# Meowuu7/equi-articulated-pose

Measured on AMD Instinct MI355X. Metric: point-clouds/sec (4096 pts, 60 anchors) fwd+bwd, higher is better.
Workload: dtype f32; 1 GPU; 8 x 4096-pt synthetic laptop clouds per GPU, 3-block inter backbone 1->64->128->512 (NN=64,K=24,A=60), forward+backward+Adam; clouds_per_gpu=8, points=4096, anchors=60

## Files before the change

equi-articulated-pose_amd/csrc/gemm_bf16x3.hip:

```cpp
#include "common.h"
#include "device_prims.h"
#include <algorithm>
#include <type_traits>

namespace {

constexpr int BK = 16, BN = 256;
constexpr unsigned PLANE_BYTES = 256 * BK * 2;
constexpr unsigned oper_bytes(int pl) { return (unsigned)pl * PLANE_BYTES; }
constexpr unsigned stage_bytes(int pl) { return 2 * oper_bytes(pl); }
constexpr size_t shmem_bytes(int pl) { return 3 * (size_t)stage_bytes(pl); }
constexpr int WAVES_N = 4;

struct Args {
    int M, N, K;
    const float *A; long long lda;
    const float *B; long long ldb, sB;
    float *C; long long ldc, sC;
    int tiles_m, tiles_n;
    const int *tbl; int na;
    int nr;
    const unsigned *Apre;
    long long sA; int slabs, kslab;
    const float *ep_scale, *ep_shift, *ep_res; float ep_slope; long long sRes;
    const unsigned *absA, *absB; float multB; int grpB; long long sAbsB;
};
constexpr int TAPS = 12;
constexpr unsigned TBL_BYTES = 64 * TAPS * 4;

__device__ __forceinline__ unsigned pk_bf16(float a, float b) {
    unsigned r;
    asm("v_cvt_pk_bf16_f32 %0, %1, %2" : "=v"(r) : "v"(a), "v"(b));
    return r;
}

struct Row16 { f32x4 q0, q1; u32x2 p0, p1; };

__device__ __forceinline__ void split_pair(float x0, float x1, unsigned &h, unsigned &m, unsigned &l) {
    h = pk_bf16(x0, x1);
    const float r0 = x0 - __uint_as_float(h << 16), r1 = x1 - __uint_as_float(h & 0xffff0000u);
    m = pk_bf16(r0, r1);
    const float s0 = r0 - __uint_as_float(m << 16), s1 = r1 - __uint_as_float(m & 0xffff0000u);
    l = pk_bf16(s0, s1);
}

__device__ __forceinline__ void split_pair_h(float x0, float x1, unsigned &h, unsigned &l) {
    const f16x2 hh = __builtin_convertvector((f32x2){x0, x1}, f16x2);
    const f16x2 ll = __builtin_convertvector((f32x2){x0 - (float)hh.x, x1 - (float)hh.y}, f16x2);
    h = __builtin_bit_cast(unsigned, hh);
    l = __builtin_bit_cast(unsigned, ll);
}

__device__ __forceinline__ void split_quad(const f32x4 &a, const f32x4 &b, u32x4 &h, u32x4 &m, u32x4 &l) {
    unsigned h0, h1, h2, h3, m0, m1, m2, m3, l0, l1, l2, l3;
    split_pair(a.x, a.y, h0, m0, l0);
    split_pair(a.z, a.w, h1, m1, l1);
    split_pair(b.x, b.y, h2, m2, l2);
    split_pair(b.z, b.w, h3, m3, l3);
    h = (u32x4){h0, h1, h2, h3};
    m = (u32x4){m0, m1, m2, m3};
    l = (u32x4){l0, l1, l2, l3};
}

template <int MI, int WN, int BMODE, bool APRE, int PL>
__device__ __forceinline__ void split_gemm_body(const Args &g) {
    constexpr unsigned OPER_BYTES = oper_bytes(PL), STAGE_BYTES = stage_bytes(PL);
    constexpr int NT = 128 * WN, NI = 8 / WN, WM = 8 / WN, BM = 32 * MI * WM, RG = NT / 4;
    constexpr int NPA = BM / RG, NPO = 256 / RG;
    static_assert(WN == 4 && NPO == 2 && (NPA == 1 || NPA == 2), "8 waves, 128-row staging groups");
    extern __shared__ __attribute__((aligned(16))) unsigned char smem[];

    int id = blockIdx.x, tm, tn;
    {
        const int groups = g.tiles_n / 8 * 8;
        const int xcd = id & 7, slot = id >> 3;
        const int panel = (slot / g.tiles_m) * 8 + xcd;
        if (panel < groups && id < groups * g.tiles_m) { tn = panel; tm = slot % g.tiles_m; }
        else { const int r = id - groups * g.tiles_m; tn = groups + r / g.tiles_m; tm = r % g.tiles_m; }
    }
    const int z = blockIdx.y;
    const int m0 = tm * BM, n0 = tn * BN;
    const int item = g.slabs > 1 ? z / g.slabs : z;
    const long long item_of_z = item;
    const long long kbeg = g.slabs > 1 ? (long long)(z - item * g.slabs) * g.kslab : 0;
    const float *A = g.A + item * g.sA + kbeg;
    const float *B = g.B + item * g.sB + (BMODE == 0 ? kbeg : BMODE == 1 ? kbeg * g.ldb : 0);
    long long zc = z;
    if constexpr (BMODE == 1) {
        if (g.slabs > 1) zc = (long long)(z - item * g.slabs) * (gridDim.y / g.slabs) + item;
    }
    float *C = g.C + zc * g.sC;

    const int t = threadIdx.x, lane = t & 63;
    const int wave = __builtin_amdgcn_readfirstlane(t >> 6);
    const int wm = wave / WN, wn = wave % WN;
    const int li = lane & 31, lh = lane >> 5;

    const int c4 = t & 3, rq = t >> 2;
    const int c4b = BMODE ? __builtin_amdgcn_readfirstlane(t >> 7) : c4, rqb = BMODE ? (t & 127) : rq;
    const float *baseA[NPA], *baseB[NPO];
#pragma unroll
    for (int u = 0; u < NPA; ++u) baseA[u] = A + (long long)min(m0 + RG * u, g.M - RG) * g.lda;
#pragma unroll
    for (int u = 0; u < NPO; ++u) baseB[u] = B + (long long)min(n0 + RG * u, g.N - RG) * g.ldb;
    const unsigned char *preA[NPA];
    constexpr int PRE_PIECE = PL == 3 ? 32 : 16;
    const long long pre_pitch = (long long)(g.K / 4) * PRE_PIECE;
#pragma unroll
    for (int u = 0; u < NPA; ++u)
        preA[u] = reinterpret_cast<const unsigned char *>(g.Apre) + (long long)min(m0 + RG * u, g.M - RG) * pre_pitch + (kbeg / 4) * PRE_PIECE;
    const unsigned offP = (unsigned)((long long)rq * pre_pitch + PRE_PIECE * c4);
    float sclA[2] = {1.0f, 1.0f}, sclB[2] = {1.0f, 1.0f};
    const unsigned *absBz = g.absB + item_of_z * g.sAbsB;
    if constexpr (PL == 2) {
#pragma unroll
        for (int u = 0; u < NPA; ++u) sclA[u] = pow2_scale(__uint_as_float(g.absA[min(m0 + RG * u, g.M - RG) + rq]));
#pragma unroll
        for (int u = 0; u < NPO; ++u) sclB[u] = pow2_scale(__uint_as_float(absBz[(min(n0 + RG * u, g.N - RG) + rqb) / g.grpB]) * g.multB);
    }
    const unsigned offA = (unsigned)((long long)rq * g.lda + 4 * c4) * 4u, offB = (unsigned)((long long)rq * g.ldb + 4 * c4) * 4u;
    unsigned colB[NPO], tapB[NPO];
#pragma unroll
    for (int u = 0; u < NPO; ++u) {
        const int n = min(n0 + RG * u, g.N - RG) + rqb;
        if constexpr (BMODE == 2) {
            const int per = g.na * g.nr, pt = n / per, an = (n - pt * per) / g.nr;
            colB[u] = (unsigned)(n - an * g.nr) * 4u;
            tapB[u] = (unsigned)an * (TAPS * 4u);
        } else {
            colB[u] = (unsigned)n * 4u; tapB[u] = 0;
        }
    }
    auto wr_of = [](int r, int c) { return (unsigned)r * 32u + ((16u * (unsigned)(c >> 1)) ^ ((((unsigned)r >> 2) ^ ((unsigned)r >> 3)) & 1u) * 16u) + 8u * (unsigned)(c & 1); };
    const unsigned wr_off = wr_of(rq, c4), wr_offB = wr_of(rqb, c4b);
    const unsigned char *tbl = smem + 3 * STAGE_BYTES;
    if constexpr (BMODE == 2) {
        for (int i = t; i < g.na * TAPS; i += NT) reinterpret_cast<int *>(smem + 3 * STAGE_BYTES)[i] = g.tbl[i] * 4 * g.nr;
        __syncthreads();
    }
    const int nk = (g.slabs > 1 ? g.kslab : g.K) / BK;

    Row16 ra0, rb0, ra1, rb1;
    auto ld = [&](const float *ubase, unsigned voff) __attribute__((always_inline)) {
        return *reinterpret_cast<const f32x4 *>(reinterpret_cast<const char *>(ubase) + voff);
    };
    auto ldw = [&](const float *ubase, unsigned voff) __attribute__((always_inline)) {
        return *reinterpret_cast<const float *>(reinterpret_cast<const char *>(ubase) + voff);
    };
    auto load_tile = [&](int kt, Row16 &a, Row16 &b) __attribute__((always_inline)) {
        const int ko = kt * BK;
        if constexpr (APRE) {
            const unsigned char *p0 = preA[0] + kt * (4 * PRE_PIECE) + offP;
            a.q0 = *reinterpret_cast<const f32x4 *>(p0);
            if constexpr (PL == 3) a.p0 = *reinterpret_cast<const u32x2 *>(p0 + 16);
            if constexpr (NPA == 2) {
                const unsigned char *p1 = preA[1] + kt * (4 * PRE_PIECE) + offP;
                a.q1 = *reinterpret_cast<const f32x4 *>(p1);
                if constexpr (PL == 3) a.p1 = *reinterpret_cast<const u32x2 *>(p1 + 16);
            }
        } else {
            a.q0 = ld(baseA[0] + ko, offA);
            if constexpr (NPA == 2) a.q1 = ld(baseA[1] + ko, offA);
        }
        if constexpr (BMODE == 0) {
            b.q0 = ld(baseB[0] + ko, offB); b.q1 = ld(baseB[1] + ko, offB);
        } else if constexpr (BMODE == 1) {
            const float *r0 = B + (long long)(ko + 4 * c4b) * g.ldb, *r1 = r0 + g.ldb, *r2 = r1 + g.ldb, *r3 = r2 + g.ldb;
            b.q0 = (f32x4){ldw(r0, colB[0]), ldw(r1, colB[0]), ldw(r2, colB[0]), ldw(r3, colB[0])};
            b.q1 = (f32x4){ldw(r0, colB[1]), ldw(r1, colB[1]), ldw(r2, colB[1]), ldw(r3, colB[1])};
        } else {
            const int k0 = ko + 4 * c4b, ch = k0 / TAPS, t0 = k0 - ch * TAPS;
            const float *r = B + (long long)ch * g.ldb;
            const u32x4 o0 = *reinterpret_cast<const u32x4 *>(tbl + tapB[0] + 4 * t0);
            const u32x4 o1 = *reinterpret_cast<const u32x4 *>(tbl + tapB[1] + 4 * t0);
            b.q0 = (f32x4){ldw(r, colB[0] + o0.x), ldw(r, colB[0] + o0.y), ldw(r, colB[0] + o0.z), ldw(r, colB[0] + o0.w)};
            b.q1 = (f32x4){ldw(r, colB[1] + o1.x), ldw(r, colB[1] + o1.y), ldw(r, colB[1] + o1.z), ldw(r, colB[1] + o1.w)};
        }
    };
    auto park_piece = [&](unsigned char *oper, int u, const f32x4 &q, unsigned wr, float scl) __attribute__((always_inline)) {
        unsigned h0, m0_, l0, h1, m1, l1;
        if constexpr (PL == 2) {
            split_pair_h(q.x * scl, q.y * scl, h0, l0);
            split_pair_h(q.z * scl, q.w * scl, h1, l1);
            unsigned char *row = oper + (unsigned)u * ((unsigned)RG * 32u) + wr;
            *reinterpret_cast<u32x2 *>(row) = (u32x2){h0, h1};
            *reinterpret_cast<u32x2 *>(row + PLANE_BYTES) = (u32x2){l0, l1};
            return;
        }
        split_pair(q.x, q.y, h0, m0_, l0);
        split_pair(q.z, q.w, h1, m1, l1);
        unsigned char *row = oper + (unsigned)u * ((unsigned)RG * 32u) + wr;
        *reinterpret_cast<u32x2 *>(row) = (u32x2){h0, h1};
        *reinterpret_cast<u32x2 *>(row + PLANE_BYTES) = (u32x2){m0_, m1};
        *reinterpret_cast<u32x2 *>(row + 2 * PLANE_BYTES) = (u32x2){l0, l1};
    };
    auto park_half = [&](unsigned char *oper, const Row16 &r, int half, int pieces, unsigned wr, float scl) __attribute__((always_inline)) {
        if (half < pieces) park_piece(oper, half, half ? r.q1 : r.q0, wr, scl);
    };
    auto park_half_a = [&](unsigned char *oper, const Row16 &r, int half, unsigned wr) __attribute__((always_inline)) {
// ... 68 lines not shown
            SB();
            product(al, bh);
            park_half(s2 + OPER_BYTES, sb, 1, NPO, wr_offB, sclB[1]);
            load_tile(min(kt + 4, nk - 1), sa, sb);
            SB();
            __syncthreads();
            return;
        }
        u32x4 bm[NI], am[MI], bh[NI], al[MI];
        frag(st, rdB, 1, bm);
        SB();
        if constexpr (decltype(first)::value) product0(ah, bl); else product(ah, bl);
        park_half_a(s2, sa, 0, wr_off);
        SB();
        frag(st, rdA, 1, am);
        SB();
        product(ah, bm);
        park_half_a(s2, sa, 1, wr_off);
        SB();
        frag(st, rdB, 0, bh);
        SB();
        product(am, bm);
        park_half(s2 + OPER_BYTES, sb, 0, NPO, wr_offB, sclB[0]);
        SB();
        frag(st, rdA, 2, al);
        SB();
        product(am, bh);
        park_half(s2 + OPER_BYTES, sb, 1, NPO, wr_offB, sclB[1]);
        SB();
        u32x4 ah2[MI];
        frag(s1, rdA, 0, ah2);
        SB();
        product(al, bh);
        load_tile(min(kt + 4, nk - 1), sa, sb);
        SB();
        frag(s1, rdB, 2, bl);
        SB();
        product(ah, bh);
        SB();
#undef SB
#pragma unroll
        for (int i = 0; i < MI; ++i) ah[i] = ah2[i];
        __syncthreads();
    };

    load_tile(0, ra0, rb0);
    load_tile(min(1, nk - 1), ra1, rb1);
    park_a(smem, ra0, wr_off);
    park(smem + OPER_BYTES, rb0, NPO, wr_offB);
    load_tile(min(2, nk - 1), ra0, rb0);
    park_a(smem + STAGE_BYTES, ra1, wr_off);
    park(smem + STAGE_BYTES + OPER_BYTES, rb1, NPO, wr_offB);
    load_tile(min(3, nk - 1), ra1, rb1);
    __syncthreads();
    frag(smem, rdA, 0, ah);
    frag(smem, rdB, PL - 1, bl);

    unsigned s0 = 0, s1 = STAGE_BYTES, s2 = 2 * STAGE_BYTES;
    tile(std::true_type{}, 0, smem + s0, smem + s1, smem + s2, ra0, rb0);
    int kt = 1;
    for (; kt + 1 < nk; kt += 2) {
        { const unsigned r = s0; s0 = s1; s1 = s2; s2 = r; }
        tile(std::false_type{}, kt, smem + s0, smem + s1, smem + s2, ra1, rb1);
        { const unsigned r = s0; s0 = s1; s1 = s2; s2 = r; }
        tile(std::false_type{}, kt + 1, smem + s0, smem + s1, smem + s2, ra0, rb0);
    }
    if (kt < nk) {
        { const unsigned r = s0; s0 = s1; s1 = s2; s2 = r; }
        tile(std::false_type{}, kt, smem + s0, smem + s1, smem + s2, ra1, rb1);
    }

#pragma unroll
    for (int i = 0; i < MI; ++i)
#pragma unroll
        for (int j = 0; j < NI; ++j) {
            const int col = n0 + 32 * NI * wn + 32 * j + li;
            float unsB = 1.0f;
            if constexpr (PL == 2) unsB = 1.0f / pow2_scale(__uint_as_float(absBz[min(col, g.N - 1) / g.grpB]) * g.multB);
#pragma unroll
            for (int r = 0; r < 16; ++r) {
                const int row = m0 + 32 * MI * wm + 32 * i + (r & 3) + 8 * (r >> 2) + 4 * lh;
                if (row < g.M && col < g.N) {
                    float v = acc[i][j][r];
                    if constexpr (PL == 2) v = (v * (1.0f / pow2_scale(__uint_as_float(g.absA[row])))) * unsB;
                    if (g.ep_scale != nullptr) {
                        v = fmaf(v, g.ep_scale[row], g.ep_shift[row]);
                        v = v >= 0.f ? v : v * g.ep_slope;
                        if (g.ep_res != nullptr) v += g.ep_res[(long long)z * g.sRes + (long long)row * g.ldc + col];
                    }
                    C[(long long)row * g.ldc + col] = v;
                }
            }
        }
}

template <int MI, int WN, int BMODE, bool APRE>
__global__ __launch_bounds__(128 * WN, WN / 2) void gemm_bf16x3_kernel(Args g) { split_gemm_body<MI, WN, BMODE, APRE, 3>(g); }

template <int MI, int WN, int BMODE, bool APRE>
__global__ __launch_bounds__(128 * WN, WN / 2) void gemm_f16x2_kernel(Args g) { split_gemm_body<MI, WN, BMODE, APRE, 2>(g); }

}

namespace {

__global__ __launch_bounds__(256) void presplit_kernel(int M, int K4, const float *__restrict__ A, long long lda, u32x4 *__restrict__ out) {
    const long long i = (long long)blockIdx.x * 256 + threadIdx.x;
    if (i >= (long long)M * K4) return;
    const int row = (int)(i / K4), c = (int)(i - (long long)row * K4);
    const f32x4 q = *reinterpret_cast<const f32x4 *>(A + row * lda + 4 * c);
    unsigned h0, m0, l0, h1, m1, l1;
    split_pair(q.x, q.y, h0, m0, l0);
    split_pair(q.z, q.w, h1, m1, l1);
    out[2 * i] = (u32x4){h0, h1, m0, m1};
    out[2 * i + 1] = (u32x4){l0, l1, 0u, 0u};
}

__global__ __launch_bounds__(256) void presplit_h_kernel(int M, int K4, const float *__restrict__ A, long long lda, const unsigned *__restrict__ absA,
                                                         u32x4 *__restrict__ out) {
    const long long i = (long long)blockIdx.x * 256 + threadIdx.x;
    if (i >= (long long)M * K4) return;
    const int row = (int)(i / K4), c = (int)(i - (long long)row * K4);
    const float scl = pow2_scale(__uint_as_float(absA[row]));
    const f32x4 q = *reinterpret_cast<const f32x4 *>(A + row * lda + 4 * c);
    unsigned h0, l0, h1, l1;
    split_pair_h(q.x * scl, q.y * scl, h0, l0);
    split_pair_h(q.z * scl, q.w * scl, h1, l1);
    out[i] = (u32x4){h0, h1, l0, l1};
}

__device__ __forceinline__ unsigned absbits4(const f32x4 &q) {
    return max(max(__float_as_uint(q.x) & 0x7fffffffu, __float_as_uint(q.y) & 0x7fffffffu), max(__float_as_uint(q.z) & 0x7fffffffu, __float_as_uint(q.w) & 0x7fffffffu));
}
__global__ __launch_bounds__(256) void absmax_rows_kernel(long long rows_total, int rows, int cols4, const float *__restrict__ x, long long ld,
                                                          long long stride, unsigned *__restrict__ out) {
    const long long r = (long long)blockIdx.x * 4 + (threadIdx.x >> 6);
    if (r >= rows_total) return;
    const long long item = r / rows;
    const f32x4 *row = reinterpret_cast<const f32x4 *>(x + item * stride + (r - item * rows) * ld);
    unsigned m = 0u;
    for (int c = threadIdx.x & 63; c < cols4; c += 64) m = max(m, absbits4(row[c]));
#pragma unroll
    for (int o = 32; o > 0; o >>= 1) m = max(m, (unsigned)__shfl_xor((int)m, o));
    if ((threadIdx.x & 63) == 0) out[r] = m;
}
__global__ __launch_bounds__(256) void absmax_colgroups_kernel(int rows, int cols4, int grp4, int row_slices, const float *__restrict__ x, long long ld,
                                                               long long stride, unsigned *__restrict__ out) {
    const int c = blockIdx.x * 256 + threadIdx.x;
    if (c >= cols4) return;
    const int item = blockIdx.z, sl = blockIdx.y;
    const int r0 = (int)((long long)rows * sl / row_slices), r1 = (int)((long long)rows * (sl + 1) / row_slices);
    const float *p = x + item * stride + 4 * (long long)c;
    unsigned m = 0u;
    for (int r = r0; r < r1; ++r) m = max(m, absbits4(*reinterpret_cast<const f32x4 *>(p + r * ld)));
    if (m != 0u) atomicMax(out + (long long)item * (cols4 / grp4) + c / grp4, m);
}
__global__ __launch_bounds__(256) void grouped_bound_kernel(long long total, int p, int nn, int n_sup, const unsigned *__restrict__ point_max,
                                                            const int32_t *__restrict__ idx, unsigned *__restrict__ out) {
    const long long i = (long long)blockIdx.x * 256 + threadIdx.x;
    if (i >= total) return;
    const unsigned *pm = point_max + (i / p) * n_sup;
    const int32_t *id = idx + i * nn;
    float s = 0.f;
    for (int n = 0; n < nn; ++n) {
        const int q = id[n];
        if ((unsigned)q < (unsigned)n_sup) s += __uint_as_float(pm[q]);
    }
// ... 247 lines not shown

void intra2d_args(Args &g, int o, int c, int p, int na, int nr, int nt, const float *W, const float *feats, const int32_t *intra_idx, float *out) {
    const long long pa = (long long)p * na * nr;
    g.M = o; g.N = (int)pa; g.K = c * nt;
    g.A = W; g.lda = (long long)c * nt;
    g.B = feats; g.ldb = pa; g.sB = (long long)c * pa;
    g.C = out; g.ldc = pa; g.sC = (long long)o * pa;
    g.tbl = intra_idx; g.na = na; g.nr = nr;
}

}

extern "C" int eap_so3_intra_conv2d_bf16x3_f32(int b, int o, int c, int p, int na, int nr, int nt, const float *W, const float *feats,
                                               const int32_t *intra_idx, float *out, eap_stream_t stream) {
    if (b <= 0 || o <= 0 || p <= 0 || na <= 0) return 0;
    if (int e = intra2d_refusal(b, o, c, p, na, nr, nt, W, "so3_intra_conv2d_bf16x3_f32")) return e;
    Args g{};
    intra2d_args(g, o, c, p, na, nr, nt, W, feats, intra_idx, out);
    return launch_split<2>(g, b, eap::S(stream), "so3_intra_conv2d_bf16x3_f32");
}

extern "C" int eap_so3_intra_conv2d_f16x2_f32(int b, int o, int c, int p, int na, int nr, int nt, const float *W, const float *feats,
                                              const int32_t *intra_idx, float *out, const int32_t *abs_w, const int32_t *abs_f, eap_stream_t stream) {
    if (b <= 0 || o <= 0 || p <= 0 || na <= 0) return 0;
    if (int e = intra2d_refusal(b, o, c, p, na, nr, nt, W, "so3_intra_conv2d_f16x2_f32")) return e;
    if (!abs_w || !abs_f) return eap::bad_arg("so3_intra_conv2d_f16x2_f32: the operand magnitudes are required (eap_absmax_rows_f32 / _colgroups_f32)");
    Args g{};
    intra2d_args(g, o, c, p, na, nr, nt, W, feats, intra_idx, out);
    g.absA = reinterpret_cast<const unsigned *>(abs_w); g.absB = reinterpret_cast<const unsigned *>(abs_f); g.multB = 1.0f;
    g.grpB = na * nr; g.sAbsB = p;
    return launch_split<2, 2>(g, b, eap::S(stream), "so3_intra_conv2d_f16x2_f32");
}

namespace {

__global__ __launch_bounds__(256) void split_reduce_kernel(long long mn4, int parts, const f32x4 *__restrict__ ws, float *__restrict__ C, int N, long long ldc) {
    const long long i = (long long)blockIdx.x * 256 + threadIdx.x;
    if (i >= mn4) return;
    f32x4 acc = ws[i];
    for (int z = 1; z < parts; ++z) acc += ws[(long long)z * mn4 + i];
    const long long e = i * 4, row = e / N, col = e - row * N;
    *reinterpret_cast<f32x4 *>(C + row * ldc + col) = acc;
}

inline int reduce_slabs(int M, int N, int K, int batch) {
    const int tiles = ((M % 256) == 0 ? M / 256 : M / 128) * ((N + BN - 1) / BN);
    int s = 1;
    while (s < 64 && (long long)tiles * batch * s < 512 && (K / BK) % (2 * s) == 0 && K / (2 * s) >= 64 * BK) s *= 2;
    return s;
}

}

extern "C" int eap_gemm_bf16x3_reduce_f32_supported(int M, int N, int K, const float *A, int64_t lda, int64_t strideA, const float *B,
                                                    int64_t ldb, int64_t strideB, int64_t ldc) {
    if (!tile_dims_ok(M, N, K)) return 0;
    if ((long long)32 * WAVES_N * lda * 4 >= (1ll << 32) || (long long)32 * WAVES_N * ldb * 4 >= (1ll << 32)) return 0;
    if ((lda & 3) || (ldb & 3) || (strideA & 3) || (strideB & 3) || (ldc & 3)) return 0;
    if ((reinterpret_cast<uintptr_t>(A) & 15) || (reinterpret_cast<uintptr_t>(B) & 15)) return 0;
    return 1;
}

extern "C" int64_t eap_gemm_bf16x3_reduce_workspace(int M, int N, int K, int batch) {
    if (M <= 0 || N <= 0 || K <= 0 || batch <= 0) return 0;
    return (int64_t)M * N * batch * reduce_slabs(M, N, K, batch);
}

extern "C" int eap_gemm_bf16x3_reduce_f32(int M, int N, int K, const float *A, int64_t lda, int64_t strideA, const float *B, int64_t ldb,
                                          int64_t strideB, float *C, int64_t ldc, int batch, float *workspace, eap_stream_t stream) {
    if (M <= 0 || N <= 0 || batch <= 0) return 0;
    if (!eap_gemm_bf16x3_reduce_f32_supported(M, N, K, A, lda, strideA, B, ldb, strideB, ldc) || (reinterpret_cast<uintptr_t>(C) & 15) ||
        (reinterpret_cast<uintptr_t>(workspace) & 15))
        return eap::bad_arg("gemm_bf16x3_reduce_f32: unsupported operands (ask eap_gemm_bf16x3_reduce_f32_supported)");
    const int slabs = reduce_slabs(M, N, K, batch);
    Args g{};
    g.M = M; g.N = N; g.K = K;
    g.A = A; g.lda = lda; g.sA = strideA;
    g.B = B; g.ldb = ldb; g.sB = strideB;
    g.C = workspace; g.ldc = N; g.sC = (long long)M * N;
    g.slabs = slabs; g.kslab = K / slabs;
    if (int e = launch_split<0>(g, (long long)batch * slabs, eap::S(stream), "gemm_bf16x3_reduce_f32")) return e;
    const long long mn4 = (long long)M * N / 4;
    return eap::run_kernel("gemm_bf16x3_reduce_f32 (sum of the partials)", split_reduce_kernel, eap::cdiv(mn4, 256), 1, 1, dim3(256), 0, eap::S(stream), mn4,
                           batch * slabs, reinterpret_cast<const f32x4 *>(workspace), C, N, (long long)ldc);
}

namespace {

int device_cus() {
    static std::atomic<int> seen[64] = {};
    int dev = 0;
    if (hipGetDevice(&dev) != hipSuccess) { (void)hipGetLastError(); return 256; }
    const bool slot = dev >= 0 && dev < 64;
    int n = slot ? seen[dev].load(std::memory_order_relaxed) : 0;
    if (n > 0) return n;
    if (hipDeviceGetAttribute(&n, hipDeviceAttributeMultiprocessorCount, dev) != hipSuccess || n <= 0) { (void)hipGetLastError(); n = 256; }
    if (slot) seen[dev].store(n, std::memory_order_relaxed);
    return n;
}

constexpr int SPLITK_MIN_TILES = 16;
constexpr int SPLITK_MAX_SLABS = 64;

inline bool splitk_slabs_ok(int K, int slabs) {
    return slabs >= 1 && slabs <= SPLITK_MAX_SLABS && (K / BK) % slabs == 0 && (slabs == 1 || K / BK / slabs >= SPLITK_MIN_TILES);
}

}

extern "C" int eap_gemm_f16x2_splitk_slabs(int M, int N, int K, int batch, int cus) {
    if (M != 128 || N <= 0 || batch <= 0 || K < 64 * BK || (K % BK) != 0) return 1;
    if (cus <= 0) cus = device_cus();
    const long long tiles = (long long)((N + BN - 1) / BN) * batch;
    const long long want = (4ll * cus + tiles - 1) / tiles;
    int best = 1;
    for (int s = 1; s <= SPLITK_MAX_SLABS; ++s) {
        if (!splitk_slabs_ok(K, s)) continue;
        best = s;
        if (s >= want) break;
    }
    const long long kt = K / BK;
    const long long one = ((tiles + cus - 1) / cus) * kt, cut = ((tiles * best + cus - 1) / cus) * (kt / best);
    return 4 * cut <= 3 * one ? best : 1;
}

extern "C" int64_t eap_gemm_f16x2_splitk_workspace(int M, int N, int batch, int slabs) {
    if (M <= 0 || N <= 0 || batch <= 0 || slabs <= 1) return 0;
    return (int64_t)M * N * batch * slabs;
}

extern "C" int eap_gemm_f16x2_splitk_f32(int M, int N, int K, const float *A, int64_t lda, const float *B, int64_t ldb, int64_t strideB,
                                         float *C, int64_t ldc, int64_t strideC, int batch, const int32_t *abs_a, const int32_t *abs_b, int grp_b,
                                         float mult_b, int slabs, float *workspace, int64_t workspace_floats, eap_stream_t stream) {
    if (M <= 0 || N <= 0 || batch <= 0) return eap::bad_arg("gemm_f16x2_splitk_f32: M, N and batch must be positive");
    if (!A || !B || !C) return eap::bad_arg("gemm_f16x2_splitk_f32: A, B and C are required");
    if (!abs_a || !abs_b || !(mult_b > 0.f) || grp_b <= 0 || (N % grp_b) != 0)
        return eap::bad_arg("gemm_f16x2_splitk_f32: the operand magnitudes are required (eap_absmax_rows_f32 / _colgroups_f32), column groups dividing N");
    if (M != 128 || !eap_gemm_bf16x3_nn_f32_supported(M, N, K, A, lda, B, ldb, strideB))
        return eap::bad_arg("gemm_f16x2_splitk_f32: one 128-row tile of operands eap_gemm_bf16x3_nn_f32_supported takes");
    if (slabs == 0) slabs = eap_gemm_f16x2_splitk_slabs(M, N, K, batch, 0);
    if (!splitk_slabs_ok(K, slabs))
        return eap::bad_arg("gemm_f16x2_splitk_f32: the slab count must divide the K / 16 k-tiles into slabs of at least 16 (at most 64 slabs)");
    if ((long long)batch * slabs > 65535) return eap::bad_arg("gemm_f16x2_splitk_f32: batch x slabs exceeds 65535");
    Args g{};
    g.M = M; g.N = N; g.K = K;
    g.A = A; g.lda = lda;
    g.B = B; g.ldb = ldb; g.sB = strideB;
    g.C = C; g.ldc = ldc; g.sC = strideC;
    g.absA = reinterpret_cast<const unsigned *>(abs_a); g.absB = reinterpret_cast<const unsigned *>(abs_b); g.multB = mult_b;
    g.grpB = grp_b; g.sAbsB = N / grp_b;
    if (slabs == 1) return launch_split<1, 2>(g, batch, eap::S(stream), "gemm_f16x2_splitk_f32");
    if (strideC != (int64_t)M * ldc || (ldc & 3) || ldc < N || !eap::aligned16(C, workspace))
        return eap::bad_arg("gemm_f16x2_splitk_f32: more than one slab needs strideC = M ldc, ldc a multiple of 4, C and the workspace 16-byte aligned");
    if (!workspace || workspace_floats < eap_gemm_f16x2_splitk_workspace(M, N, batch, slabs))
        return eap::bad_arg("gemm_f16x2_splitk_f32: the workspace is too small (ask eap_gemm_f16x2_splitk_workspace)");
    g.C = workspace; g.ldc = N; g.sC = (long long)M * N;
    g.slabs = slabs; g.kslab = K / slabs;
    if (int e = launch_split<1, 2>(g, (long long)batch * slabs, eap::S(stream), "gemm_f16x2_splitk_f32")) return e;
    const long long mn4 = (long long)batch * M * N / 4;
    return eap::run_kernel("gemm_f16x2_splitk_f32 (sum of the slabs)", split_reduce_kernel, eap::cdiv(mn4, 256), 1, 1, dim3(256), 0, eap::S(stream), mn4, slabs,
                           reinterpret_cast<const f32x4 *>(workspace), C, N, (long long)ldc);
}
```

equi-articulated-pose_amd/csrc/narrow_conv.hip:

```cpp
#include "common.h"
#include "device_prims.h"
#include <type_traits>

namespace {

constexpr int NT = 256, WAVES = 4;
constexpr int TILE = 128;
constexpr int SEGC = 2048;

__device__ __forceinline__ int drow(int r, int h) { return (r & 3) + 8 * (r >> 2) + 4 * h; }

template <int KS2>
__device__ __forceinline__ void load_x(f32x4 (&xa)[KS2], const float *__restrict__ xb, long n, long col0, unsigned voff, bool ok, int ck, int h) {
#pragma unroll
    for (int s = 0; s < KS2; ++s)
        xa[s] = (ok && 2 * s + h < ck) ? ld_off<f32x4>(xb + (size_t)(2 * s) * n + col0, voff) : (f32x4){0.f, 0.f, 0.f, 0.f};
}

template <int KS2>
__device__ __forceinline__ void load_w(float (&wf)[KS2], const float *__restrict__ W, int orow, int ck, int h) {
#pragma unroll
    for (int s = 0; s < KS2; ++s) wf[s] = (2 * s + h < ck) ? W[(size_t)orow * ck + 2 * s + h] : 0.f;
}

// ... 57 lines not shown
                                                                 const float *__restrict__ x, float *__restrict__ pivot,
                                                                 float *__restrict__ psum, float *__restrict__ psq) {
    __shared__ __attribute__((aligned(16))) float s_piv[64];
    __shared__ float s_red[WAVES][2][32];
    const Pos w(ct, n);
    const int t = threadIdx.x, o0 = blockIdx.y * ct * 32, h = w.h;
    if (t < 32 * ct) {
        float p = 0.f;
        for (int k = 0; k < ck; ++k) p = fmaf(W[(size_t)(o0 + t) * ck + k], x[(size_t)k * n], p);
        s_piv[t] = p;
        if (w.seg == 0 && w.bi == 0) pivot[o0 + t] = p;
    }
    __syncthreads();
    float wf[KS2];
    load_w<KS2>(wf, W, w.ch0 + w.li, ck, h);
    f32x4 pv[4];
#pragma unroll
    for (int g = 0; g < 4; ++g) pv[g] = *reinterpret_cast<const f32x4 *>(&s_piv[w.ch0 - o0 + 8 * g + 4 * h]);
    float sa[16], qa[16];
#pragma unroll
    for (int r = 0; r < 16; ++r) sa[r] = qa[r] = 0.f;
    const float *xb = x + (size_t)w.bi * ck * n;
#pragma unroll 1
    for (long col0 = w.beg + (long)w.cw * TILE; col0 < w.end; col0 += (long)w.ncw * TILE) {
        const long col = col0 + 4 * w.li;
        const bool ok = col < n;
        f32x4 xa[KS2];
        load_x<KS2>(xa, xb, n, col0, w.xoff, ok, ck, h);
        f32x16 d[4];
        conv_tile<KS2, false>(d, xa, wf);
        if (ok) {
#pragma unroll
            for (int r = 0; r < 16; ++r)
#pragma unroll
                for (int c = 0; c < 4; ++c) {
                    const float dd = d[c][r] - pv[r >> 2][r & 3];
                    sa[r] += dd;
                    qa[r] = fmaf(dd, dd, qa[r]);
                }
        }
    }
    block_sums(sa, qa, s_red, ct, o0, w.bi, gridDim.z, nseg, w.seg, psum, psq);
}

template <int KS2>
__global__ __launch_bounds__(NT) void narrow_conv_bnact_fwd_kernel(int ct, int o, int ck, long n, float slope, const float *__restrict__ W,
                                                                     const float *__restrict__ x, const float *__restrict__ scale,
                                                                     const float *__restrict__ shift, float *__restrict__ y) {
    const Pos w(ct, n);
    const int h = w.h;
    float wf[KS2];
    load_w<KS2>(wf, W, w.ch0 + w.li, ck, h);
    f32x4 sc[4], sh[4];
#pragma unroll
    for (int g = 0; g < 4; ++g) {
        sc[g] = *reinterpret_cast<const f32x4 *>(scale + w.ch0 + 8 * g + 4 * h);
        sh[g] = *reinterpret_cast<const f32x4 *>(shift + w.ch0 + 8 * g + 4 * h);
    }
    const float *xb = x + (size_t)w.bi * ck * n;
    float *yb = y + ((size_t)w.bi * o + w.ch0) * n;
    const unsigned roff = 4u * (4u * h * (unsigned)n + 4u * w.li);
#pragma unroll 1
    for (long col0 = w.beg + (long)w.cw * TILE; col0 < w.end; col0 += (long)w.ncw * TILE) {
        const long col = col0 + 4 * w.li;
        const bool ok = col < n;
        f32x4 xa[KS2];
        load_x<KS2>(xa, xb, n, col0, w.xoff, ok, ck, h);
        f32x16 d[4];
        conv_tile<KS2, false>(d, xa, wf);
        if (ok) {
#pragma unroll
            for (int r = 0; r < 16; ++r) {
                const float a = sc[r >> 2][r & 3], b = sh[r >> 2][r & 3];
                f32x4 v;
                v.x = fmaf(d[0][r], a, b); v.y = fmaf(d[1][r], a, b); v.z = fmaf(d[2][r], a, b); v.w = fmaf(d[3][r], a, b);
                v.x = v.x > 0.f ? v.x : v.x * slope; v.y = v.y > 0.f ? v.y : v.y * slope;
                v.z = v.z > 0.f ? v.z : v.z * slope; v.w = v.w > 0.f ? v.w : v.w * slope;
                st_off<f32x4>(yb + (size_t)(8 * (r >> 2)) * n + col0, roff + 4u * (unsigned)(r & 3) * (unsigned)n, v);
            }
        }
    }
}

template <int KS2>
__global__ __launch_bounds__(NT) void narrow_conv_bwd_reduce_kernel(int ct, int o, int ck, long n, int nseg, float slope,
                                                                      const float *__restrict__ gy, const float *__restrict__ x,
                                                                      const float *__restrict__ W, const float *__restrict__ scale,
                                                                      const float *__restrict__ shift, const float *__restrict__ mean,
                                                                      const float *__restrict__ invstd, float *__restrict__ pg,
                                                                      float *__restrict__ pgx) {
    __shared__ __attribute__((aligned(16))) float s_sc[64], s_sh[64], s_mu[64], s_is[64];
    __shared__ float s_red[WAVES][2][32];
    const Pos w(ct, n);
    const int t = threadIdx.x, o0 = blockIdx.y * ct * 32, h = w.h;
    if (t < 32 * ct) { s_sc[t] = scale[o0 + t]; s_sh[t] = shift[o0 + t]; s_mu[t] = mean[o0 + t]; s_is[t] = invstd[o0 + t]; }
    __syncthreads();
    float wf[KS2];
    load_w<KS2>(wf, W, w.ch0 + w.li, ck, h);
    float sa[16], qa[16];
#pragma unroll
    for (int r = 0; r < 16; ++r) sa[r] = qa[r] = 0.f;
    const float *xb = x + (size_t)w.bi * ck * n;
    const float *gb = gy + ((size_t)w.bi * o + w.ch0) * n;
    const unsigned roff = 4u * (4u * h * (unsigned)n + 4u * w.li);
    const int lc = w.ch0 - o0;
#pragma unroll 1
    for (long col0 = w.beg + (long)w.cw * TILE; col0 < w.end; col0 += (long)w.ncw * TILE) {
        const long col = col0 + 4 * w.li;
        const bool ok = col < n;
        f32x4 xa[KS2];
        load_x<KS2>(xa, xb, n, col0, w.xoff, ok, ck, h);
        f32x16 d[4];
        conv_tile<KS2, false>(d, xa, wf);
        if (ok) {
#pragma unroll
            for (int g = 0; g < 4; ++g) {
                f32x4 gv[4];
#pragma unroll
                for (int q = 0; q < 4; ++q) gv[q] = ld_off<f32x4>(gb + (size_t)(8 * g) * n + col0, roff + 4u * q * (unsigned)n);
                const f32x4 sc = *reinterpret_cast<const f32x4 *>(&s_sc[lc + 8 * g + 4 * h]), sh = *reinterpret_cast<const f32x4 *>(&s_sh[lc + 8 * g + 4 * h]);
                const f32x4 mu = *reinterpret_cast<const f32x4 *>(&s_mu[lc + 8 * g + 4 * h]), is = *reinterpret_cast<const f32x4 *>(&s_is[lc + 8 * g + 4 * h]);
#pragma unroll
                for (int q = 0; q < 4; ++q)
#pragma unroll
                    for (int c = 0; c < 4; ++c) {
                        const float yv = d[c][4 * g + q];
                        const float pre = fmaf(yv, sc[q], sh[q]);
                        const float gg = pre > 0.f ? gv[q][c] : gv[q][c] * slope;
                        sa[4 * g + q] += gg;
                        qa[4 * g + q] = fmaf(gg, (yv - mu[q]) * is[q], qa[4 * g + q]);
                    }
            }
        }
    }
    block_sums(sa, qa, s_red, ct, o0, w.bi, gridDim.z, nseg, w.seg, pg, pgx);
}

template <int KS2>
__global__ __launch_bounds__(NT) void narrow_conv_bwd_dw_kernel(int ct, int o, int ck, long n, int nseg, float slope,
                                                                  const float *__restrict__ gy, const float *__restrict__ x,
                                                                  const float *__restrict__ W, const float *__restrict__ scale,
                                                                  const float *__restrict__ shift, const float *__restrict__ mean,
                                                                  const float *__restrict__ invstd, const float *__restrict__ k2,
                                                                  const float *__restrict__ k3, float *__restrict__ partial) {
    __shared__ float s_part[WAVES][16][64];
    const Pos w(ct, n);
    const int h = w.h, li = w.li, wave = threadIdx.x >> 6;
    const int ch = w.ch0 + li;
    float wf[KS2];
    load_w<KS2>(wf, W, ch, ck, h);
    const float sc = scale[ch], sh = shift[ch], mu = mean[ch], is = invstd[ch], c2 = k2[ch], c3 = k3[ch];
    const float *gb = gy + ((size_t)w.bi * o + w.ch0) * n;
    const unsigned goff = 4u * ((unsigned)li * (unsigned)n + 16u * h), koff = 4u * ((unsigned)min(li, ck - 1) * (unsigned)n + 16u * h);
    f32x16 dw;
#pragma unroll
    for (int r = 0; r < 16; ++r) dw[r] = 0.f;
    const float *xb = x + (size_t)w.bi * ck * n;
    const f32x4 zero4 = {0.f, 0.f, 0.f, 0.f};
#pragma unroll 1
    for (long col0 = w.beg + (long)w.cw * TILE; col0 < w.end; col0 += (long)w.ncw * TILE) {
        const long col = col0 + 4 * li;
        f32x4 xa[KS2];
        load_x<KS2>(xa, xb, n, col0, w.xoff, col < n, ck, h);
        f32x16 d[4];
        conv_tile<KS2, true>(d, xa, wf);
#pragma unroll
        for (int g = 0; g < 4; ++g) {
            f32x4 gv[4], xv[4];
#pragma unroll
            for (int q = 0; q < 4; ++q) {
                const long cq = col0 + 4 * (8 * g + 4 * h + q);
                const bool in = cq < n;
                gv[q] = in ? ld_off<f32x4>(gb + col0 + 4 * (8 * g + q), goff) : zero4;
                xv[q] = (in && li < ck) ? ld_off<f32x4>(xb + col0 + 4 * (8 * g + q), koff) : zero4;
            }
#pragma unroll
            for (int q = 0; q < 4; ++q)
#pragma unroll
                for (int c = 0; c < 4; ++c) {
                    const float yv = d[c][4 * g + q];
                    const float pre = fmaf(yv, sc, sh);
                    const float gg = pre > 0.f ? gv[q][c] : gv[q][c] * slope;
                    const float gx = fmaf(gg, sc, -c2) - ((yv - mu) * is) * c3;
                    dw = __builtin_amdgcn_mfma_f32_32x32x2f32(gx, xv[q][c], dw, 0, 0, 0);
                }
        }
    }
#pragma unroll
    for (int r = 0; r < 16; ++r) s_part[wave][r][w.lane] = dw[r];
    __syncthreads();
    if (wave < ct) {
        float *slab = partial + ((size_t)w.bi * nseg + w.seg) * o * ck;
#pragma unroll
        for (int r = 0; r < 16; ++r) {
            float v = 0.f;
            for (int u = wave; u < WAVES; u += ct) v += s_part[u][r][w.lane];
            if (li < ck) slab[(size_t)(w.ch0 + drow(r, h)) * ck + li] = v;
        }
    }
}

__global__ __launch_bounds__(256) void narrow_conv_dw_sum_kernel(int mn, int slabs, const float *__restrict__ partial, float *__restrict__ dW) {
    const int e = blockIdx.x * 4 + (threadIdx.x >> 6), lane = threadIdx.x & 63;
    if (e >= mn) return;
    float s = 0.f;
    for (int z = lane; z < slabs; z += 64) s += partial[(size_t)z * mn + e];
#pragma unroll
    for (int d = 32; d > 0; d >>= 1) s += __shfl_xor(s, d);
    if (lane == 0) dW[e] = s;
}

inline int nseg_of(long n) { return (int)((n + SEGC - 1) / SEGC); }

inline bool misaligned(const void *p) { return (reinterpret_cast<uintptr_t>(p) & 15) != 0; }

inline int refuse(const char *who, int o, int ck, long n, const void *p0, const void *p1, const void *p2 = nullptr) {
    char buf[200];
    const char *why = nullptr;
    if (ck < 1 || ck > 32) why = "1 to 32 contraction indices (C*K)";
    else if (o < 32 || o % 32 != 0) why = "a multiple of 32 output channels";
    else if (n < 0 || (n & 3) != 0 || n >= (1l << 25)) why = "a row length (P*A) that is a multiple of 4 below 2^25";
    else if (misaligned(p0) || misaligned(p1) || misaligned(p2)) why = "16-byte aligned tensors";
    if (!why) return 0;
    snprintf(buf, sizeof(buf), "%s: takes %s", who, why);
    return eap::bad_arg(buf);
}

inline int tiles_per_block(int o) { return o % 64 == 0 ? 2 : 1; }

template <typename F>
int by_depth(int ck, F &&f) {
    return ck <= 24 ? f(std::integral_constant<int, 12>{}) : f(std::integral_constant<int, 16>{});
}

}

extern "C" int eap_narrow_conv_segments(int64_t n) { return n > 0 ? nseg_of((long)n) : 0; }

extern "C" int eap_narrow_conv_stats_f32(int b, int o, int ck, int64_t n, const float *W, const float *x, float *pivot, float *psum,
                                         float *psq, eap_stream_t stream) {
    if (int e = refuse("narrow_conv_stats", o, ck, (long)n, x, nullptr)) return e;
    if (b <= 0 || n <= 0) return 0;
    const int nseg = nseg_of((long)n), ct = tiles_per_block(o);
    return by_depth(ck, [&](auto ks2) {
        return eap::run_kernel("narrow_conv_stats", narrow_conv_stats_kernel<decltype(ks2)::value>, nseg, o / (32 * ct), b, dim3(NT), 0, eap::S(stream), ct,
                               ck, (long)n, nseg, W, x, pivot, psum, psq);
    });
}

extern "C" int eap_narrow_conv_bnact_fwd_f32(int b, int o, int ck, int64_t n, float slope, const float *W, const float *x, const float *scale,
                                             const float *shift, float *y, eap_stream_t stream) {
    if (int e = refuse("narrow_conv_bnact_fwd", o, ck, (long)n, x, y, scale)) return e;
    if (misaligned(shift)) return eap::bad_arg("narrow_conv_bnact_fwd: takes 16-byte aligned tensors");
    if (b <= 0 || n <= 0) return 0;
    const int ct = tiles_per_block(o);
    return by_depth(ck, [&](auto ks2) {
        return eap::run_kernel("narrow_conv_bnact_fwd", narrow_conv_bnact_fwd_kernel<decltype(ks2)::value>, nseg_of((long)n), o / (32 * ct), b, dim3(NT), 0,
                               eap::S(stream), ct, o, ck, (long)n, slope, W, x, scale, shift, y);
    });
}

extern "C" int eap_narrow_conv_bwd_reduce_f32(int b, int o, int ck, int64_t n, float slope, const float *gy, const float *x, const float *W,
                                              const float *scale, const float *shift, const float *mean, const float *invstd, float *pg,
                                              float *pgx, eap_stream_t stream) {
    if (int e = refuse("narrow_conv_bwd_reduce", o, ck, (long)n, x, gy)) return e;
    if (b <= 0 || n <= 0) return 0;
    const int nseg = nseg_of((long)n), ct = tiles_per_block(o);
    return by_depth(ck, [&](auto ks2) {
        return eap::run_kernel("narrow_conv_bwd_reduce", narrow_conv_bwd_reduce_kernel<decltype(ks2)::value>, nseg, o / (32 * ct), b, dim3(NT), 0, eap::S(stream),
                               ct, o, ck, (long)n, nseg, slope, gy, x, W, scale, shift, mean, invstd, pg, pgx);
    });
}

extern "C" int eap_narrow_conv_bwd_dw_f32(int b, int o, int ck, int64_t n, float slope, const float *gy, const float *x, const float *W,
                                          const float *scale, const float *shift, const float *mean, const float *invstd, const float *k2,
                                          const float *k3, float *partial, float *dW, eap_stream_t stream) {
    if (int e = refuse("narrow_conv_bwd_dw", o, ck, (long)n, x, gy)) return e;
    if (b <= 0 || n <= 0) return 0;
    const int nseg = nseg_of((long)n), ct = tiles_per_block(o);
    hipStream_t s = eap::S(stream);
    int e = by_depth(ck, [&](auto ks2) {
        return eap::run_kernel("narrow_conv_bwd_dw", narrow_conv_bwd_dw_kernel<decltype(ks2)::value>, nseg, o / (32 * ct), b, dim3(NT), 0, s, ct, o, ck, (long)n,
                               nseg, slope, gy, x, W, scale, shift, mean, invstd, k2, k3, partial);
    });
    if (e) return e;
    const int mn = o * ck;
    return eap::run_kernel("narrow_conv_bwd_dw (sum)", narrow_conv_dw_sum_kernel, eap::cdiv(mn, 4), 1, 1, dim3(256), 0, s, mn, b * nseg, partial, dW);
}
```

equi-articulated-pose_amd/csrc/norm_fold.hip:

```cpp
#include <math.h>
#include <string.h>

#include "common.h"

namespace {

constexpr int WAVE = 64;

__device__ __forceinline__ double wave_sum(double v) {
#pragma unroll
    for (int m = WAVE / 2; m >= 1; m >>= 1) v += __shfl_xor(v, m, WAVE);
    return v;
}

__device__ __forceinline__ void two_row_sums(const float *__restrict__ a, const float *__restrict__ q, int parts, int lane, double &sa, double &sq) {
    sa = 0.0, sq = 0.0;
    for (int i = lane; i < parts; i += WAVE) {
        sa += (double)a[i];
        sq += (double)q[i];
    }
    sa = wave_sum(sa);
    sq = wave_sum(sq);
}

// ... 15 lines not shown
    double var = s2 / count - m * m;
    var = var < 0.0 ? 0.0 : var;
    if (running_mean != nullptr) {
        const float keep = (float)(1.0 - momentum), alpha = (float)momentum;
        running_mean[ch] = fmaf(alpha, (float)mu, running_mean[ch] * keep);
        running_var[ch] = fmaf(alpha, (float)(var * (count / (count - 1.0))), running_var[ch] * keep);
    }
    const double g = (double)gamma[ch];
    const double is = rsqrt(var + eps);
    const double scale64 = g * is;
    scale[ch] = (float)scale64;
    shift[ch] = (float)((double)beta[ch] - mu * scale64);
    mean[ch] = mu;
    invstd[ch] = is;
    beta_copy[ch] = beta[ch];
    inv_gamma[ch] = g == 0.0 ? 0.f : (float)(1.0 / g);
}

__global__ __launch_bounds__(WAVE) void norm_fold_bwd_kernel(int o, int parts, int b, int na, double count, const float *__restrict__ pg,
                                                             const float *__restrict__ pgx, const float *__restrict__ k1v,
                                                             const float *__restrict__ beta, const float *__restrict__ inv_gamma,
                                                             const float *__restrict__ gmax, const float *__restrict__ xmax,
                                                             float *__restrict__ dgamma, float *__restrict__ dbeta, float *__restrict__ k2v,
                                                             float *__restrict__ k3v, float *__restrict__ coef, float *__restrict__ bound) {
    const int ch = blockIdx.x, lane = threadIdx.x;
    double tg, tgx;
    two_row_sums(pg + (long)ch * parts, pgx + (long)ch * parts, parts, lane, tg, tgx);
    const float k1 = k1v[ch];
    const float k2 = (float)((double)k1 * tg / count), k3 = (float)((double)k1 * tgx / count);
    if (lane == 0) {
        dgamma[ch] = (float)tgx;
        dbeta[ch] = (float)tg;
        k2v[ch] = k2;
        k3v[ch] = k3;
        if (coef != nullptr) {
            coef[ch] = k1, coef[o + ch] = k2, coef[2 * o + ch] = k3;
            coef[3 * o + ch] = beta[ch], coef[4 * o + ch] = inv_gamma[ch];
        }
    }
    if (bound == nullptr) return;
    const float a1 = fabsf(k1), a2 = fabsf(k2), a3 = fabsf(k3);
    for (int cloud = 0; cloud < b; ++cloud) {
        const long row = ((long)cloud * o + ch) * na;
        for (int a = lane; a < na; a += WAVE) bound[row + a] = (a1 * gmax[row + a] + a2) + a3 * xmax[row + a];
    }
}

__global__ __launch_bounds__(256) void norm_fold_colmax_kernel(int o, int na, const float *__restrict__ bound, float *__restrict__ colmax) {
    __shared__ float red[256];
    const int t = threadIdx.x, a = blockIdx.x * 16 + (t & 15), grp = t >> 4, cloud = blockIdx.y;
    float m = 0.f;
    if (a < na) {
        const float *src = bound + (long)cloud * o * na + a;
        for (int ch = grp; ch < o; ch += 16) m = nan_max(m, src[(long)ch * na]);
    }
    red[t] = m;
    __syncthreads();
    if (grp == 0 && a < na) {
        for (int g = 1; g < 16; ++g) m = nan_max(m, red[g * 16 + t]);
        colmax[(long)cloud * na + a] = m;
    }
}

__global__ __launch_bounds__(256) void dense_zbound_kernel(int b, int na, int rp, int p, int ldw, long cnt_stride, const float *__restrict__ colmax,
                                                           const int32_t *__restrict__ cnt, const int32_t *__restrict__ n_rows,
                                                           float *__restrict__ words) {
    const int w = blockIdx.x * blockDim.x + threadIdx.x, cloud = blockIdx.y;
    if (w >= ldw) return;
    float v = 0.f;
    if (w < na * rp / 4) {
        const int a = 4 * w / rp, r0 = 4 * w - a * rp, live = n_rows[cloud];
        const float m = colmax[(long)cloud * na + a];
#pragma unroll
        for (int j = 0; j < 4; ++j) {
            int c = r0 + j < live ? cnt[cloud * cnt_stride + r0 + j] : 0;
            c = c < 0 ? 0 : (c > p ? p : c);
            const float t = m * (float)c;
            v = j == 0 ? t : nan_max(v, t);
        }
    }
    words[(long)cloud * ldw + w] = v;
}

__global__ __launch_bounds__(256) void dense_gbound_parts_kernel(int bc, int c, int rp, int na, int ks, const float *__restrict__ W3,
                                                                 const float *__restrict__ fc4, float *__restrict__ fpart, float *__restrict__ wsum) {
    __shared__ float red[256];
    const int t = threadIdx.x, nt = blockDim.x;
    if ((int)blockIdx.x < bc) {
        const float *src = fc4 + (long)blockIdx.x * rp * na;
        const int len = rp * na;
        float m = 0.f, m1 = 0.f, m2 = 0.f, m3 = 0.f;
        int e = t;
        for (; e + 3 * nt < len; e += 4 * nt) {
            const float v0 = src[e], v1 = src[e + nt], v2 = src[e + 2 * nt], v3 = src[e + 3 * nt];
            m = nan_max(m, fabsf(v0)), m1 = nan_max(m1, fabsf(v1)), m2 = nan_max(m2, fabsf(v2)), m3 = nan_max(m3, fabsf(v3));
        }
        for (; e < len; e += nt) m = nan_max(m, fabsf(src[e]));
        m = nan_max(nan_max(m, m1), nan_max(m2, m3));
        red[t] = m;
        __syncthreads();
        if (t < na) {
            for (int g = 1; g < nt / na; ++g) m = nan_max(m, red[t + g * na]);
            fpart[(long)blockIdx.x * na + t] = m;
        }
        return;
    }
    const int oc = blockIdx.x - bc, lane = t & (WAVE - 1), wave = t / WAVE, waves = nt / WAVE;
    float m = 0.f;
    if (wave < waves)
        for (int k = wave; k < ks; k += waves) {
            const float *row = W3 + ((long)oc * ks + k) * c;
            double s = 0.0;
            for (int i = lane; i < c; i += WAVE) s += (double)fabsf(row[i]);
            m = nan_max(m, (float)wave_sum(s));
        }
    if (lane == 0 && wave < waves) red[wave] = m;
    __syncthreads();
    if (t == 0) {
        for (int g = 1; g < waves; ++g) m = nan_max(m, red[g]);
        wsum[oc] = m * 1.0001f;
    }
}

__global__ __launch_bounds__(256) void dense_gbound_kernel(int c, int na, int o, const float *__restrict__ fpart, const float *__restrict__ wsum,
                                                           float *__restrict__ bound) {
    __shared__ float red[256];
    const int t = threadIdx.x, cloud = blockIdx.x / na, a = blockIdx.x - cloud * na;
    float m = 0.f;
    for (int ch = t; ch < c; ch += 256) m = nan_max(m, fpart[((long)cloud * c + ch) * na + a]);
    red[t] = m;
    __syncthreads();
    for (int s = 128; s >= 1; s >>= 1) {
        if (t < s) red[t] = nan_max(red[t], red[t + s]);
        __syncthreads();
    }
    m = red[0];
    for (int oc = t; oc < o; oc += 256) bound[(long)blockIdx.x * o + oc] = m * wsum[oc];
}

__global__ __launch_bounds__(256) void dense_point_order_kernel(int p, int quads, const int64_t *__restrict__ order, const int4 *__restrict__ memb,
                                                                const float *__restrict__ q_xyz, int32_t *__restrict__ order32,
                                                                int4 *__restrict__ memb_out, float *__restrict__ xyz_out,
                                                                int32_t *__restrict__ pivot_pos) {
    const long i = (long)blockIdx.x * blockDim.x + threadIdx.x;
    const int cloud = blockIdx.y;
    if (i >= (long)p * quads) return;
    const int j = (int)(i / quads), q = (int)(i - (long)j * quads);
    const int64_t src = order[(long)cloud * p + j];
    if (src < 0 || src >= p) return;
    memb_out[((long)cloud * p + j) * quads + q] = memb[((long)cloud * p + src) * quads + q];
    if (q != 0) return;
    order32[(long)cloud * p + j] = (int32_t)src;
#pragma unroll
    for (int k = 0; k < 3; ++k) xyz_out[((long)cloud * 3 + k) * p + j] = q_xyz[((long)cloud * 3 + k) * p + src];
    if (cloud == 0 && src == 0) pivot_pos[0] = j;
}

inline double from_bits(int64_t bits) {
    double v;
    memcpy(&v, &bits, sizeof v);
    return v;
}

inline bool aligned16(const void *p) { return (reinterpret_cast<uintptr_t>(p) & 15) == 0; }

}

extern "C" int eap_norm_fold_train_f32(int o, int parts, int64_t pivot_stride, int64_t count, int64_t eps_bits, int64_t momentum_bits,
                                       const float *ps, const float *pq, const float *pivot, const float *gamma, const float *beta,
                                       float *running_mean, float *running_var, float *scale, float *shift, double *mean, double *invstd,
                                       float *beta_copy, float *inv_gamma, eap_stream_t stream) {
    if (!ps || !pq || !pivot || !gamma || !beta || !scale || !shift || !mean || !invstd || !beta_copy || !inv_gamma)
        return eap::bad_arg("norm_fold_train: null pointer (only running_mean / running_var may be null, and only together)");
    if ((running_mean == nullptr) != (running_var == nullptr))
        return eap::bad_arg("norm_fold_train: null pointer (only running_mean / running_var may be null, and only together)");
    if (o <= 0 || parts <= 0 || count <= 0 || pivot_stride <= 0) return eap::bad_arg("norm_fold_train: o, parts, count and the pivot stride must be positive");
    return eap::run_kernel("norm_fold_train", norm_fold_train_kernel, o, 1, 1, dim3(WAVE), 0, eap::S(stream), parts, (long)pivot_stride, (double)count,
                           from_bits(eps_bits), from_bits(momentum_bits), ps, pq, pivot, gamma, beta, running_mean, running_var, scale, shift, mean,
                           invstd, beta_copy, inv_gamma);
}

extern "C" int eap_norm_fold_bwd_f32(int o, int parts, int b, int na, int64_t count, const float *pg, const float *pgx, const float *k1,
                                     const float *beta, const float *inv_gamma, const float *gmax, const float *xmax, float *dgamma, float *dbeta,
                                     float *k2, float *k3, float *coef, float *bound, float *colmax, eap_stream_t stream) {
    if (!pg || !pgx || !k1 || !dgamma || !dbeta || !k2 || !k3) return eap::bad_arg("norm_fold_bwd: null pointer");
    const bool dense = beta || inv_gamma || gmax || xmax || coef || bound || colmax;
    if (dense && !(beta && inv_gamma && gmax && xmax && coef && bound && colmax))
        return eap::bad_arg("norm_fold_bwd: null pointer (beta, inv_gamma, gmax, xmax, coef, bound and colmax come together or not at all)");
    if (o <= 0 || parts <= 0 || count <= 0) return eap::bad_arg("norm_fold_bwd: o, parts and count must be positive");
    if (dense && (b <= 0 || na <= 0 || b > 65535)) return eap::bad_arg("norm_fold_bwd: b and na must be positive, b at most 65535 (grid.y)");
    if (int e = eap::run_kernel("norm_fold_bwd", norm_fold_bwd_kernel, o, 1, 1, dim3(WAVE), 0, eap::S(stream), o, parts, b, na, (double)count, pg, pgx, k1,
                                beta, inv_gamma, gmax, xmax, dgamma, dbeta, k2, k3, coef, bound))
        return e;
    if (!dense) return 0;
    return eap::run_kernel("norm_fold_bwd (colmax)", norm_fold_colmax_kernel, eap::cdiv(na, 16), b, 1, dim3(256), 0, eap::S(stream), o, na, (const float *)bound,
                           colmax);
}

extern "C" int eap_so3_dense_zbound_f32(int b, int na, int rp, int p, int ldz, int64_t cnt_stride, const float *colmax, const int32_t *cnt,
                                        const int32_t *n_rows, float *words, eap_stream_t stream) {
    if (!colmax || !cnt || !n_rows || !words) return eap::bad_arg("so3_dense_zbound: null pointer");
    if (b <= 0 || na <= 0 || rp <= 0 || p <= 0 || ldz <= 0) return eap::bad_arg("so3_dense_zbound: b, na, rp, p and ldz must be positive");
    if (rp % 4 != 0 || ldz % 4 != 0 || (long long)na * rp > ldz || cnt_stride < rp)
        return eap::bad_arg("so3_dense_zbound: rp and ldz multiples of 4, ldz >= na * rp, the row stride of cnt >= rp");
    return eap::run_kernel("so3_dense_zbound", dense_zbound_kernel, eap::cdiv(ldz / 4, 256), b, 1, dim3(256), 0, eap::S(stream), b, na, rp, p, ldz / 4,
                           (long)cnt_stride, colmax, cnt, n_rows, words);
}

extern "C" int eap_so3_dense_gplanes_bound_f32(int b, int o, int c, int na, int ks, int rp, const float *W3, const float *fc4, float *fpart,
                                               float *wsum, float *bound, eap_stream_t stream) {
    if (!W3 || !fc4 || !fpart || !wsum || !bound) return eap::bad_arg("so3_dense_gplanes_bound: null pointer");
    if (b <= 0 || o <= 0 || c <= 0 || na <= 0 || ks <= 0 || rp <= 0) return eap::bad_arg("so3_dense_gplanes_bound: every size must be positive");
    if (na > 128 || (long long)rp * na > 0x7fffffffLL || (long long)b * c > 0x7fffffffLL - o || (long long)b * na > 0x7fffffffLL)
        return eap::bad_arg("so3_dense_gplanes_bound: na <= 128, rp * na, b * c + o and b * na below 2^31");
    const int nt = 256 / na * na;
    if (int e = eap::run_kernel("so3_dense_gplanes_bound (parts)", dense_gbound_parts_kernel, (long long)b * c + o, 1, 1, dim3(nt), 0, eap::S(stream), b * c, c,
                                rp, na, ks, W3, fc4, fpart, wsum))
        return e;
    return eap::run_kernel("so3_dense_gplanes_bound", dense_gbound_kernel, (long long)b * na, 1, 1, dim3(256), 0, eap::S(stream), c, na, o, (const float *)fpart,
                           (const float *)wsum, bound);
}

extern "C" int eap_so3_dense_point_order(int b, int p, int words, const int64_t *order, const uint32_t *memb, const float *q_xyz, int32_t *order32,
                                         uint32_t *memb_out, float *xyz_out, int32_t *pivot_pos, eap_stream_t stream) {
    if (!order || !memb || !q_xyz || !order32 || !memb_out || !xyz_out || !pivot_pos) return eap::bad_arg("so3_dense_point_order: null pointer");
    if (b <= 0 || p <= 0) return eap::bad_arg("so3_dense_point_order: b and p must be positive");
    if (words != 16 && words != 32) return eap::bad_arg("so3_dense_point_order: 16 or 32 membership words per point");
    if (!aligned16(memb) || !aligned16(memb_out)) return eap::bad_arg("so3_dense_point_order: takes 16-byte aligned membership tables");
    const int quads = words / 4;
    return eap::run_kernel("so3_dense_point_order", dense_point_order_kernel, eap::cdiv((long long)p * quads, 256), b, 1, dim3(256), 0, eap::S(stream), p, quads,
                           order, reinterpret_cast<const int4 *>(memb), q_xyz, order32, reinterpret_cast<int4 *>(memb_out), xyz_out, pivot_pos);
}
```

equi-articulated-pose_amd/vgtk/_hip.py:

```python
import ctypes
import os
import re
import struct
import types
import weakref

import torch

_PKG_ROOT = os.path.abspath(os.path.join(os.path.dirname(__file__), '..'))
LIB_PATH = os.path.join(_PKG_ROOT, 'libeap_hip.so')

if not os.path.exists(LIB_PATH):
    raise ImportError(
        f'{LIB_PATH} not found: build the HIP extension first '
        '(python -c "import __graft_entry__ as g; g.build()" or make -C equi-articulated-pose_amd/csrc). '
        'This package has no CPU fallback.')

lib = ctypes.CDLL(LIB_PATH)


_HEADERS = (os.path.join(_PKG_ROOT, 'include', 'eap_hip.h'), os.path.join(os.path.dirname(_PKG_ROOT), 'include', 'eap_hip.h'))
HEADER_PATH = next((p for p in _HEADERS if os.path.exists(p)), _HEADERS[-1])

_I64 = ctypes.c_int64
# ... 133 lines not shown

SPLIT_PLANES_SCAN_ROWS = 384


def _pieces_ok(t, *dims):
    return not any(int(d) & 3 for d in dims) and t.data_ptr() % 16 == 0


def absmax_rows(t, batch, rows, cols, ld, stride):
    if not _pieces_ok(t, cols, ld, stride):
        return None
    out = torch.empty(batch, rows, dtype=torch.int32, device=t.device)
    call('eap_absmax_rows_f32', t, t, batch, rows, cols, ld, stride, out)
    return out


def absmax_colgroups(t, batch, rows, cols, ld, stride, grp):
    if not _pieces_ok(t, cols, ld, stride, grp) or cols % grp:
        return None
    out = torch.empty(batch, cols // grp, dtype=torch.int32, device=t.device)
    call('eap_absmax_colgroups_f32', t, t, batch, rows, cols, ld, stride, grp, out)
    return out


def so3_grouped_bound(feats, idx):
    b, c, n, na = feats.shape
    pm = absmax_colgroups(feats, b, c, n * na, n * na, c * n * na, na) if na % 4 == 0 else None
    if pm is None:
        return None
    out = torch.empty(b, idx.shape[1], dtype=torch.int32, device=feats.device)
    call('eap_so3_grouped_bound_f32', feats, b, idx.shape[1], idx.shape[2], n, pm, idx, out)
    return out


def _planes2(transB, M, N, K, A, lda, batch, B, ldb, strideB, b_bound):
    if SPLIT_PLANES != 2:
        return None
    if b_bound is None and M < SPLIT_PLANES_SCAN_ROWS:
        return None
    abs_a = absmax_rows(A, 1, M, K, lda, 0)
    if abs_a is None:
        return None
    if b_bound is not None:
        return abs_a, b_bound[0], int(b_bound[1]), float(b_bound[2])
    abs_b = absmax_rows(B, batch, N, K, ldb, strideB) if transB else absmax_colgroups(B, batch, K, N, ldb, strideB, 4)
    return None if abs_b is None else (abs_a, abs_b, 1 if transB else 4, 1.0)


def _gemm_split(transB, M, N, K, A, lda, B, ldb, strideB, C, ldc, strideC, batch, b_bound, tag, epilogue=None):
    tb = int(bool(transB))
    split = 'eap_gemm_bf16x3_f32' if tb else 'eap_gemm_bf16x3_nn_f32'
    if not getattr(abi, split + '_supported')(M, N, K, A, lda, B, ldb, strideB):
        return False
    ops = (M, N, K, A, lda, B, ldb, strideB, C, ldc, strideC, batch)
    ep = (None, None, 0.0, None, 0) if epilogue is None else (*epilogue, strideC)
    two = _planes2(tb, M, N, K, A, lda, batch, B, ldb, strideB, b_bound)
    if two is not None:
        call('eap_gemm_f16x2_f32', C, tb, *ops, two[0], two[1], two[2], two[3], *ep, tag=tag)
    elif epilogue is None:
        call(split, C, *ops, tag=tag)
    else:
        call('eap_gemm_bf16x3_ep_f32', C, tb, *ops, *ep, tag=tag)
    return True


def gemm(transA, transB, M, N, K, A, lda, strideA, B, ldb, strideB, C, ldc, strideC, batch, b_blocked=False, b_bound=None):
    tag = {'flops': 2.0 * M * N * K * batch, 'shape': ('gemm', int(transA), int(transB), M, N, K, batch)}
    if SPLIT_BF16_CONTRACTION and not b_blocked and not transA and (strideA == 0 or batch == 1) and \
            _gemm_split(transB, M, N, K, A, lda, B, ldb, strideB, C, ldc, strideC, batch, b_bound, tag):
        return
    if not b_blocked and _dma_ok(transA, transB, M, N, K, A, lda, strideA, B, ldb, strideB):
        call('eap_gemm_dma_f32', C, int(transA), int(transB), M, N, K, A, lda, strideA, B, ldb, strideB, C, ldc, strideC, batch, tag=tag)
        return
    call('eap_gemm_f32_xb' if b_blocked else 'eap_gemm_f32', C, int(transA), int(transB), M, N, K, A, lda, strideA, B,
         (N if transB else K) if b_blocked else ldb, strideB, C, ldc, strideC, batch, tag=tag)


def gemm_epilogue(transB, M, N, K, A, lda, B, ldb, strideB, C, ldc, strideC, batch, scale, shift, slope, residual=None, b_bound=None):
    tag = {'flops': 2.0 * M * N * K * batch, 'shape': ('gemm_epilogue', 0, int(transB), M, N, K, batch)}
    return bool(SPLIT_BF16_CONTRACTION and _gemm_split(transB, M, N, K, A, lda, B, ldb, strideB, C, ldc, strideC, batch, b_bound, tag,
                                                       (scale, shift, slope, residual)))


def gemm_reduce(transA, transB, M, N, K, A, lda, strideA, B, ldb, strideB, C, ldc, batch, b_blocked=False):
    tag = {'flops': 2.0 * M * N * K * batch, 'shape': ('gemm_reduce', int(transA), int(transB), M, N, K, batch)}
    ops = (M, N, K, A, lda, strideA, B, ldb, strideB)
    nt = not b_blocked and not transA and transB
    lead = (int(transA), int(transB))
    if SPLIT_BF16_CONTRACTION and nt and C.data_ptr() % 16 == 0 and abi.eap_gemm_bf16x3_reduce_f32_supported(*ops, ldc):
        name, ws_words, lead = 'eap_gemm_bf16x3_reduce_f32', abi.eap_gemm_bf16x3_reduce_workspace, ()
    elif nt and abi.eap_gemm_skinny_reduce_f32_supported(*ops):
        name, ws_words, lead = 'eap_gemm_skinny_reduce_f32', abi.eap_gemm_skinny_reduce_workspace, ()
    elif not b_blocked and _dma_ok(transA, transB, M, N, K, A, lda, strideA, B, ldb, strideB):
        name, ws_words = 'eap_gemm_dma_f32_reduce', abi.eap_gemm_dma_f32_reduce_workspace
    else:
        name, ws_words = 'eap_gemm_f32_reduce_xb' if b_blocked else 'eap_gemm_f32_reduce', abi.eap_gemm_f32_reduce_workspace
        if b_blocked:
            ops = ops[:7] + (N if transB else K,) + ops[8:]
    ws = torch.empty(max(int(ws_words(M, N, K, batch)), 1), dtype=torch.float32, device=C.device)
    call(name, C, *lead, *ops, C, ldc, batch, ws, tag=tag)



def operand(t, name='operand'):
    shape, strides = t.shape, t.stride()
    if t.dtype != torch.float32 or len(shape) not in (2, 3):
        raise RuntimeError(f'{name}: a float32 view [rows, cols] or [batch, rows, cols], not {t.dtype} {tuple(shape)}')
    rows, cols = shape[-2], shape[-1]
    if strides[-1] == 1:
        trans, ld, outer, inner = 0, strides[-2], rows, cols
    elif strides[-2] == 1:
        trans, ld, outer, inner = 1, strides[-1], cols, rows
    else:
        raise RuntimeError(f'{name}: neither the rows nor the columns are contiguous (strides {strides})')
    batch, stride = (shape[0], strides[0]) if len(shape) == 3 else (1, 0)
    extent = (batch - 1) * stride + (outer - 1) * ld + inner
    if 4 * (t.storage_offset() + extent) > t.untyped_storage().nbytes():
        raise RuntimeError(f'{name}: {tuple(shape)} with strides {strides} at offset {t.storage_offset()} addresses {extent} elements, '
                           f'its storage holds {t.untyped_storage().nbytes() // 4}')
    return trans, ld, stride, batch, rows, cols


def _product(A, B, out, reduce=False):
    ta, lda, sa, ba, M, K = operand(A, 'A')
    tb, ldb, sb, batch, Kb, N = operand(B, 'B')
    tc, ldc, sc, bc, Mc, Nc = operand(out, 'out')
    if B.dim() != 3 or out.dim() != 3 - reduce:
        raise RuntimeError(f'B is a stack of matrices, out {"one matrix" if reduce else "a stack"}: got B {tuple(B.shape)}, out {tuple(out.shape)}')
    if K != Kb or (M, N) != (Mc, Nc) or (A.dim() == 3 and ba != batch) or bc != (1 if reduce else batch):
        raise RuntimeError(f'A {tuple(A.shape)} x B {tuple(B.shape)} -> out {tuple(out.shape)}: the sizes do not agree')
    if tc:
        raise RuntimeError(f'out must be row-major (strides {tuple(out.stride())})')
    if (M > 1 and ldc < N) or (bc > 1 and sc < (M - 1) * ldc + N):
        raise RuntimeError(f'out {tuple(out.shape)} with strides {tuple(out.stride())} overlaps itself')
    return ta, tb, M, N, K, lda, sa, ldb, sb, ldc, sc, batch


SPLIT_K_ONE_ROW_TILE = True


def _matmul_split_k(M, N, K, A, lda, B, ldb, sb, out, ldc, sc, batch, b_bound):
    if not (SPLIT_K_ONE_ROW_TILE and SPLIT_BF16_CONTRACTION and M == 128 and K >= 16 * 64 and out.is_cuda and sc == M * ldc and ldc % 4 == 0
            and out.data_ptr() % 16 == 0 and abi.eap_gemm_bf16x3_nn_f32_supported(M, N, K, A, lda, B, ldb, sb)):
        return False
    slabs = abi.eap_gemm_f16x2_splitk_slabs(M, N, K, batch, 0)
    if slabs <= 1:
        return False
    two = _planes2(0, M, N, K, A, lda, batch, B, ldb, sb, b_bound)
    if two is None:
        return False
    floats = int(abi.eap_gemm_f16x2_splitk_workspace(M, N, batch, slabs))
    work = torch.empty(floats, dtype=torch.float32, device=out.device)
    tag = {'flops': 2.0 * M * N * K * batch, 'shape': ('gemm', 0, 0, M, N, K, batch)}
    call('eap_gemm_f16x2_splitk_f32', out, M, N, K, A, lda, B, ldb, sb, out, ldc, sc, batch, two[0], two[1], two[2], two[3], slabs, work, floats, tag=tag)
    return True


def matmul(A, B, out, b_bound=None):
    ta, tb, M, N, K, lda, sa, ldb, sb, ldc, sc, batch = _product(A, B, out)
    if not ta and not tb and (sa == 0 or batch == 1) and _matmul_split_k(M, N, K, A, lda, B, ldb, sb, out, ldc, sc, batch, b_bound):
        return
    gemm(ta, tb, M, N, K, A, lda, sa, B, ldb, sb, out, ldc, sc, batch, b_bound=b_bound)


def matmul_reduce(A, B, out):
    ta, tb, M, N, K, lda, sa, ldb, sb, ldc, _, batch = _product(A, B, out, reduce=True)
    gemm_reduce(ta, tb, M, N, K, A, lda, sa, B, ldb, sb, out, ldc, batch)


def matmul_reduce_takes_split(A, B, out):
    ta, tb, M, N, K, lda, sa, ldb, sb, ldc, _, _ = _product(A, B, out, reduce=True)
    return bool(SPLIT_BF16_CONTRACTION and not ta and tb and out.data_ptr() % 16 == 0 and
                abi.eap_gemm_bf16x3_reduce_f32_supported(M, N, K, A, lda, sa, B, ldb, sb, ldc))


def matmul_epilogue(A, B, out, scale, shift, slope, residual=None, b_bound=None):
    ta, tb, M, N, K, lda, sa, ldb, sb, ldc, sc, batch = _product(A, B, out)
    if ta or (sa != 0 and batch != 1):
        raise RuntimeError(f'A must be one row-major matrix shared by the batch, not {tuple(A.shape)} with strides {tuple(A.stride())}')
    if residual is not None:
        tight = residual.is_contiguous() and residual.numel() == batch * M * N and (ldc, sc) == (N, M * N)
        if residual.dtype != torch.float32 or not (tight or (residual.shape == out.shape and residual.stride() == out.stride())):
            raise RuntimeError(f'residual: float32 laid out like out {tuple(out.shape)} with strides {out.stride()}, not {residual.dtype} '
                               f'{tuple(residual.shape)} with strides {residual.stride()}')
        operand(residual.view(batch, M, N) if tight else residual, 'residual')
    return gemm_epilogue(tb, M, N, K, A, lda, B, ldb, sb, out, ldc, sc, batch, scale, shift, slope, residual, b_bound)


def so3_prep(q_xyz, s_xyz, idx, q_pose, s_pose, anchors, identity_anchor):
    b, _, p = q_xyz.shape
    n = s_xyz.shape[2]
    nn = idx.shape[2]
    gx = torch.empty(b, p, nn, 4, dtype=torch.float32, device=q_xyz.device)
    nonident = torch.empty(b, dtype=torch.int32, device=q_xyz.device)
    call('eap_so3_prep_f32', gx, b, p, n, nn, anchors.shape[0], q_xyz, s_xyz, idx, q_pose, s_pose, anchors, int(identity_anchor), gx, nonident)
    return gx, nonident


def so3_inter_weights(gx, rk, sigma):
    b, p, nn, _ = gx.shape
    na, ks, _ = rk.shape
    w = torch.empty(b, p, na, ks, nn, dtype=torch.float32, device=gx.device)
    call('eap_so3_inter_weights_f32', w, b, p, nn, na, ks, sigma, gx, rk, w)
    return w


def so3_anchor_perm(gx, mult):
    b, p, nn, _ = gx.shape
    na = mult.shape[0]
    perm = torch.empty(b, p, nn, na, dtype=torch.int64, device=gx.device)
    call('eap_so3_anchor_perm', gx, b, p, nn, na, gx, mult, perm)
    return perm




def so3_anchor_map(idx, q_pose, s_pose, anchors):
    check_input(idx, q_pose, s_pose, anchors)
    b, p, nn = idx.shape
    na = anchors.shape[0]
    if tuple(q_pose.shape) != (b, p, 4, 4) or s_pose.shape[0] != b or tuple(s_pose.shape[2:]) != (4, 4):
        raise RuntimeError('so3_anchor_map: poses must be [b,p,4,4] (query) and [b,n,4,4] (support)')
    amap = torch.empty(b, p, nn, na, dtype=torch.uint8, device=idx.device)
    nontrivial = torch.empty(b, dtype=torch.int32, device=idx.device)
    call('eap_so3_anchor_map_f32', amap, b, p, s_pose.shape[1], nn, na, idx, q_pose, s_pose, anchors, amap, nontrivial)
    return amap, nontrivial


def _check_map(amap, idx, na):
    if amap.dtype != torch.uint8 or tuple(amap.shape) != tuple(idx.shape) + (na,) or not amap.is_contiguous():
        raise RuntimeError('anchor map: contiguous uint8 [b,p,nn,na] expected')


def so3_inter_group_fwd_map(feats, idx, gx, rk, amap, sigma):
    b, c, n, na = feats.shape
    p, nn = idx.shape[1], idx.shape[2]
    ks = rk.shape[1]
    _check_map(amap, idx, na)
    out = torch.empty(b, c, ks, p, na, dtype=torch.float32, device=feats.device)
    call('eap_so3_inter_group_fwd_map_f32', out, b, c, p, n, nn, na, ks, sigma, feats, idx, gx, rk, amap, out,
         tag={'flops': 2.0 * b * c * ks * p * nn * na, 'shape': ('group_fwd_map', b, c, p, nn, na, ks)})
    return out


def so3_inter_group_bwd_map(gout, idx, gx, rk, amap, sigma, n):
    b, c, ks, p, na = gout.shape
    nn = idx.shape[2]
    _check_map(amap, idx, na)
    gfeats = torch.empty(b, c, n, na, dtype=torch.float32, device=gout.device)
# ... 421 lines not shown
         geo.mask(direction), geo.steps(direction), out, tag={'flops': flops, 'executed_f16_flops': _dense_executed_flops(geo, o, p, direction),
         'shape': ('so3_dense', direction, b, o, p, geo.na, geo.ks, geo.rp)})
    return out


def so3_dense_bwd(gy, geo, ldz=None, colmap=None, rowmax=False):
    b, o, p, na = gy.shape
    ldz = na * geo.rp if ldz is None else int(ldz)
    colmap = geo.columns(colmap)
    scale, planes = so3_dense_split(gy, rowmax=take_rowmax_hint(gy) if rowmax is False else rowmax, colmap=colmap)
    if colmap is not None:
        p = colmap.shape[1]
    z = torch.empty(b, o, geo.ks, ldz, dtype=torch.float32, device=gy.device)
    return _dense_product(0, geo, b, o, p, ldz, scale, planes, z, 2.0 * b * o * p * na * geo.ks * geo.nn)


def so3_dense_gplanes(fc4, W3, geo):
    b, c, rp, na = fc4.shape
    o = W3.shape[0] // geo.ks
    if not GPLANES or not abi.eap_so3_dense_gplanes_supported(o, c, na, geo.ks, rp):
        return None
    ft = fc4.permute(0, 3, 2, 1).contiguous()
    if NATIVE_NORM_GLUE:
        bound = so3_dense_gplanes_bound(W3, fc4, geo.ks)
    else:
        wsum = W3.abs().sum(1).view(o, geo.ks).amax(1)
        fm = fc4.abs().amax((1, 2))
        bound = (fm[:, :, None] * (wsum * 1.0001)[None, None, :]).contiguous()
    scale = torch.empty(2, b, na, o, dtype=torch.float32, device=fc4.device)
    planes = torch.empty(b * na * o * ((geo.ks * rp + 31) // 32 * 32), dtype=torch.int32, device=fc4.device)
    call('eap_so3_dense_gplanes_f32', fc4, b, o, c, na, geo.ks, rp, W3, ft, geo.n_rows, bound, scale, planes,
         tag={'flops': 0.0, 'shape': ('so3_dense_gplanes', b, o, c, na, geo.ks, rp)})
    return scale, planes


GPLANES = True


NATIVE_NORM_GLUE = True


def _f64_bits(x):
    return struct.unpack('<q', struct.pack('<d', float(x)))[0]


def norm_fold_train(ps, pq, pivot, count, gamma, beta, eps, momentum, running_mean, running_var):
    check_input(ps, pq, gamma, beta, running_mean, running_var)
    o, parts = ps.shape
    if pivot.dim() != 1 or pivot.shape[0] != o or pivot.dtype != torch.float32 or not pivot.is_cuda:
        raise RuntimeError('norm_fold_train: pivot must be a float32 device vector (any stride) of one element per channel')
    dev = ps.device
    scale, shift, beta_copy, inv_gamma = (torch.empty(o, dtype=torch.float32, device=dev) for _ in range(4))
    mean, invstd = (torch.empty(o, dtype=torch.float64, device=dev) for _ in range(2))
    call('eap_norm_fold_train_f32', ps, o, parts, max(int(pivot.stride(0)), 1), int(count), _f64_bits(eps), _f64_bits(momentum), ps, pq, pivot, gamma,
         beta, running_mean, running_var, scale, shift, mean, invstd, beta_copy, inv_gamma)
    return scale, shift, mean, invstd, beta_copy, inv_gamma


def norm_fold_bwd(pg, pgx, k1, count, beta=None, inv_gamma=None, gmax=None, xmax=None):
    check_input(pg, pgx, k1, beta, inv_gamma, gmax, xmax)
    o, parts = pg.shape
    dev = pg.device
    dgamma, dbeta, k2, k3 = (torch.empty(o, dtype=torch.float32, device=dev) for _ in range(4))
    if gmax is None:
        call('eap_norm_fold_bwd_f32', pg, o, parts, 0, 0, int(count), pg, pgx, k1, None, None, None, None, dgamma, dbeta, k2, k3, None, None, None)
        return dgamma, dbeta, k2, k3
    b, _, na = gmax.shape
    coef = torch.empty(5, o, dtype=torch.float32, device=dev)
    bound = torch.empty(b, o, na, dtype=torch.float32, device=dev)
    colmax = torch.empty(b, na, dtype=torch.float32, device=dev)
    call('eap_norm_fold_bwd_f32', pg, o, parts, b, na, int(count), pg, pgx, k1, beta, inv_gamma, gmax, xmax, dgamma, dbeta, k2, k3, coef, bound, colmax)
    return dgamma, dbeta, k2, k3, coef, bound, colmax


def so3_dense_zbound(colmax, cnt, n_rows, rp, p, ldz):
    b, na = colmax.shape
    if cnt.dtype != torch.int32 or n_rows.dtype != torch.int32 or cnt.stride(1) != 1 or not n_rows.is_contiguous():
        raise RuntimeError('so3_dense_zbound: cnt and n_rows must be int32, the rows of cnt contiguous')
    words = torch.empty(b, ldz // 4, dtype=torch.float32, device=colmax.device)
    call('eap_so3_dense_zbound_f32', colmax, b, na, int(rp), int(p), int(ldz), cnt.stride(0), colmax, cnt, n_rows, words)
    return words


def so3_dense_gplanes_bound(W3, fc4, ks):
    check_input(W3, fc4)
    b, c, rp, na = fc4.shape
    o = W3.shape[0] // ks
    dev = fc4.device
    fpart = torch.empty(b, c, na, dtype=torch.float32, device=dev)
    wsum = torch.empty(o, dtype=torch.float32, device=dev)
    bound = torch.empty(b, na, o, dtype=torch.float32, device=dev)
    call('eap_so3_dense_gplanes_bound_f32', fc4, b, o, c, na, int(ks), rp, W3, fc4, fpart, wsum, bound)
    return bound


def so3_dense_point_order(order, memb, q_xyz):
    check_input(order, memb, q_xyz)
    b, p = order.shape
    order32 = torch.empty(b, p, dtype=torch.int32, device=order.device)
    memb_out, xyz_out = torch.empty_like(memb), torch.empty_like(q_xyz)
    pivot_pos = torch.empty(1, dtype=torch.int32, device=order.device)
    call('eap_so3_dense_point_order', order, b, p, memb.shape[2], order, memb, q_xyz, order32, memb_out, xyz_out, pivot_pos)
    return order32, memb_out, xyz_out, pivot_pos


def so3_dense_fwd(g, geo, p, c=0, ldg=None, out=None, col_map=None, operand=None, o=None):
    yt = _dense_fwd_yt(g, geo, p, c, ldg, operand, o)
    b, na, o = yt.shape[0], geo.na, yt.shape[2]
    if col_map is not None:
        if out is None or col_map.dtype != torch.int32 or tuple(col_map.shape) != (b, p) or not col_map.is_contiguous() or not out.is_contiguous():
            raise RuntimeError('so3_dense_fwd: col_map must be a contiguous int32 [b,p] and come with a contiguous out')
        call('eap_so3_dense_untranspose_map_f32', yt, b, o, p, na, out.shape[2], geo.columns(col_map), yt, out)
        return out
    y = torch.empty(b, o, p, na, dtype=torch.float32, device=yt.device)
    chunks = (p + 63) // 64
    ps = torch.empty(o, b * chunks, dtype=torch.float32, device=yt.device)
    pq = torch.empty_like(ps)
    if geo.order is not None:
        call('eap_so3_dense_untranspose_map_stats_f32', yt, b, o, p, na, p, geo.order, geo.pivot_pos, yt, y, ps, pq)
    else:
        call('eap_so3_dense_untranspose_f32', yt, b, o, p, na, yt, y, ps, pq)
    leave_stats_hint(y, (ps, pq))
    return y


def _dense_fwd_yt(g, geo, p, c, ldg, operand, o):
    na = geo.na
    if operand is None:
        b, o = g.shape[:2]
        ldg = geo.rp * na if ldg is None else int(ldg)
        scale, planes = so3_dense_split(g, seg=geo.rp, seg_pitch=ldg, shape=(b, o, geo.ks * geo.rp, na), mapped=True, n_rows=geo.n_rows)
    else:
        scale, planes = operand
        b = geo.b
    yt = torch.empty(b, na, o, p, dtype=torch.float32, device=planes.device)
    return _dense_product(1, geo, b, o, p, 0, scale, planes, yt, 2.0 * b * c * geo.ks * na * (p * geo.nn + o * p - o * geo.rp))


def so3_dense_fwd_bnact(g, geo, p, c, ldg, norm_moments, operand=None, o=None, affine=None, partials=False):
    yt = _dense_fwd_yt(g, geo, p, c, ldg, operand, o)
    b, na, o = yt.shape[0], geo.na, yt.shape[2]
    if affine is not None:
        bn_scale, bn_shift, slope = affine[0].contiguous(), affine[1].contiguous(), float(affine[2])
    else:
        ps, pq = _partials(yt, b * na, o, p)
        call('eap_bn_stats_f32', yt, b * na, o, p, yt, ps, pq)
        if partials:
            bn_scale, bn_shift, slope = norm_moments(ps, pq, yt[0, 0, :, 0], b * na * p)
        else:
            bn_scale, bn_shift, slope = norm_moments(ps.sum(1, dtype=torch.float64), pq.sum(1, dtype=torch.float64), yt[0, 0, :, 0].double(), b * na * p)
    y = torch.empty(b, o, p, na, dtype=torch.float32, device=yt.device)
    call('eap_so3_dense_untranspose_bnact_f32', yt, b, o, p, na, p, geo.order, yt, bn_scale, bn_shift, slope, y)
    return y


def bn_act_bwd_reduce_fromy(gy, y, beta, inv_gamma, slope, partials=False):
    b, c, p, na = y.shape
    n = p * na
    nblk = int(abi.eap_bn_act_fromy_blocks(n, na))
    pg = torch.empty(c, b * nblk, dtype=torch.float32, device=y.device)
    pgx = torch.empty_like(pg)
    gmax = torch.empty(b, c, na, dtype=torch.int32, device=y.device)
    xmax = torch.empty_like(gmax)
    call('eap_bn_act_bwd_reduce_fromy_f32', y, b, c, n, na, slope, gy, y, beta, inv_gamma, pg, pgx, gmax, xmax)
    if partials:
        return pg, pgx, gmax.view(torch.float32), xmax.view(torch.float32)
# ... 4 lines not shown
    b, o, p, na = gy.shape
    ldz = na * geo.rp if ldz is None else int(ldz)
    colmap = geo.columns(None)
    l = p if colmap is None else colmap.shape[1]
    scale = torch.empty(2, b, na, o, dtype=torch.float32, device=gy.device)
    planes = torch.empty(b * na * o * ((l + 31) // 32 * 32), dtype=torch.int32, device=gy.device)
    call('eap_so3_dense_split_bn_f32', gy, b, o, l, p, na, rowbound.view(torch.int32), colmap, gy, yact, coef, slope, scale, planes)
    z = torch.empty(b, o, geo.ks, ldz, dtype=torch.float32, device=gy.device)
    return _dense_product(0, geo, b, o, l, ldz, scale, planes, z, 2.0 * b * o * l * na * geo.ks * geo.nn)


def _partials(x, b, c, n):
    nseg = int(abi.eap_bn_act_segments(n))
    return (torch.empty(c, b * nseg, dtype=torch.float32, device=x.device),
            torch.empty(c, b * nseg, dtype=torch.float32, device=x.device))


_STATS_HINT = [None]
STATS_HINTS_TAKEN = 0


def _leave_hint(slot, t, payload):
    slot[0] = (weakref.ref(t), t._version, tuple(t.shape), payload)


def _take_hint(slot, t):
    h, slot[0] = slot[0], None
    if not USE_ROWMAX_HINT or h is None or h[0]() is not t or h[1] != t._version or h[2] != tuple(t.shape):
        return None
    return h[3]


def leave_stats_hint(t, partials):
    _leave_hint(_STATS_HINT, t, partials)


def take_stats_hint(t):
    global STATS_HINTS_TAKEN
    partials = _take_hint(_STATS_HINT, t)
    STATS_HINTS_TAKEN += partials is not None
    return partials


def bn_stats(x, b, c, n):
    hint = take_stats_hint(x)
    if hint is not None and hint[0].shape[0] == c:
        return hint[0].sum(1, dtype=torch.float64), hint[1].sum(1, dtype=torch.float64)
    ps, pq = _partials(x, b, c, n)
    call('eap_bn_stats_f32', x, b, c, n, x, ps, pq)
    return ps.sum(1, dtype=torch.float64), pq.sum(1, dtype=torch.float64)


def bn_act_fwd(x, b, c, n, scale, shift, slope, residual=None):
    y = torch.empty_like(x)
    if residual is None:
        call('eap_bn_act_fwd_f32', x, b, c, n, slope, x, scale, shift, y)
    else:
        call('eap_bn_act_add_fwd_f32', x, b, c, n, slope, x, scale, shift, residual, y)
    return y


def bn_act_bwd_reduce(gy, x, b, c, n, scale, shift, mean, invstd, slope):
    pg, pgx = _partials(x, b, c, n)
    call('eap_bn_act_bwd_reduce_f32', x, b, c, n, slope, gy, x, scale, shift, mean, invstd, pg, pgx)
    return pg.sum(1, dtype=torch.float64), pgx.sum(1, dtype=torch.float64)


_ROWMAX_HINT = [None]
USE_ROWMAX_HINT = True
ROWMAX_HINTS_TAKEN = 0


def leave_rowmax_hint(t, rowmax):
    _leave_hint(_ROWMAX_HINT, t, rowmax)


def take_rowmax_hint(t):
    global ROWMAX_HINTS_TAKEN
    rowmax = _take_hint(_ROWMAX_HINT, t)
    ROWMAX_HINTS_TAKEN += rowmax is not None
    return rowmax


def bn_act_bwd_apply(gy, x, b, c, n, scale, shift, mean, invstd, k2, k3, slope):
    gx = torch.empty_like(x)
    if x.dim() == 4 and x.shape[3] % 4 == 0 and x.shape[3] <= 64 and n == x.shape[2] * x.shape[3] and c % 128 == 0 and gx.data_ptr() % 16 == 0 \
            and gy.data_ptr() % 16 == 0 and x.data_ptr() % 16 == 0:
        rowmax = torch.empty(b, c, x.shape[3], dtype=torch.int32, device=x.device)
        call('eap_bn_act_bwd_apply_rowmax_f32', x, b, c, n, int(x.shape[3]), slope, gy, x, scale, shift, mean, invstd, k2, k3, gx, rowmax)
        leave_rowmax_hint(gx, rowmax)
        return gx
    call('eap_bn_act_bwd_apply_f32', x, b, c, n, slope, gy, x, scale, shift, mean, invstd, k2, k3, gx)
    return gx



NARROW_CONV_MAX_CK = 32


def narrow_conv_takes(o, ck, n):
    return 1 <= ck <= NARROW_CONV_MAX_CK and o >= 32 and o % 32 == 0 and n % 4 == 0 and n < (1 << 25)


def _narrow_partials(x, b, o, n):
    nseg = int(abi.eap_narrow_conv_segments(n))
    return (torch.empty(o, b * nseg, dtype=torch.float32, device=x.device),
            torch.empty(o, b * nseg, dtype=torch.float32, device=x.device))


def narrow_conv_stats(W, x, partials=False):
    check_input(W, x)
    b, ck, n = x.shape
    o = W.shape[0]
    ps, pq = _narrow_partials(x, b, o, n)
    pivot = torch.empty(o, dtype=torch.float32, device=x.device)
    call('eap_narrow_conv_stats_f32', x, b, o, ck, n, W, x, pivot, ps, pq)
    if partials:
        return ps, pq, pivot
    return ps.sum(1, dtype=torch.float64), pq.sum(1, dtype=torch.float64), pivot.double()


def narrow_conv_bnact_fwd(W, x, scale, shift, slope):
    check_input(W, x, scale, shift)
    b, ck, n = x.shape
    o = W.shape[0]
    y = torch.empty(b, o, n, dtype=torch.float32, device=x.device)
    call('eap_narrow_conv_bnact_fwd_f32', x, b, o, ck, n, slope, W, x, scale, shift, y)
    return y


def narrow_conv_bwd_reduce(gy, x, W, scale, shift, mean, invstd, slope, partials=False):
    check_input(gy, x, W, scale, shift, mean, invstd)
    b, ck, n = x.shape
    o = W.shape[0]
    pg, pgx = _narrow_partials(x, b, o, n)
    call('eap_narrow_conv_bwd_reduce_f32', x, b, o, ck, n, slope, gy, x, W, scale, shift, mean, invstd, pg, pgx)
    if partials:
        return pg, pgx
    return pg.sum(1, dtype=torch.float64), pgx.sum(1, dtype=torch.float64)


def narrow_conv_bwd_dw(gy, x, W, scale, shift, mean, invstd, k2, k3, slope):
    check_input(gy, x, W, scale, shift, mean, invstd, k2, k3)
    b, ck, n = x.shape
    o = W.shape[0]
    nseg = int(abi.eap_narrow_conv_segments(n))
    partial = torch.empty(b * nseg, o, ck, dtype=torch.float32, device=x.device)
    dW = torch.empty(o, ck, dtype=torch.float32, device=x.device)
    call('eap_narrow_conv_bwd_dw_f32', x, b, o, ck, n, slope, gy, x, W, scale, shift, mean, invstd, k2, k3, partial, dW)
    return dW



def bn_stats_masked(x, b, c, n, na, mask):
    ps, pq = _partials(x, b, c, n)
    call('eap_bn_stats_masked_f32', x, b, c, n, na, x, mask, ps, pq)
    return ps.view(c, b, -1).sum(2, dtype=torch.float64).t(), pq.view(c, b, -1).sum(2, dtype=torch.float64).t()


def bn_act_cloud_fwd(x, b, c, n, scale, shift, slope):
    y = torch.empty_like(x)
    call('eap_bn_act_cloud_fwd_f32', x, b, c, n, slope, x, scale, shift, y)
    return y


def bn_act_cloud_bwd_reduce(gy, x, b, c, n, scale, shift, mean, invstd, slope):
    pg, pgx = _partials(x, b, c, n)
    call('eap_bn_act_cloud_bwd_reduce_f32', x, b, c, n, slope, gy, x, scale, shift, mean, invstd, pg, pgx)
    return pg.view(c, b, -1).sum(2, dtype=torch.float64).t(), pgx.view(c, b, -1).sum(2, dtype=torch.float64).t()


def bn_act_cloud_bwd_apply(gy, x, b, c, n, na, scale, shift, mean, invstd, k2, k3, mask, slope):
    gx = torch.empty_like(x)
    call('eap_bn_act_cloud_bwd_apply_f32', x, b, c, n, na, slope, gy, x, scale, shift, mean, invstd, k2, k3, mask, gx)
    return gx



def bn_act_cloud_mean_fwd(x, scale, shift, w, inv_den, slope):
    b, c, p, na = x.shape
    out = torch.empty(b, c, na, dtype=torch.float32, device=x.device)
    call('eap_bn_act_cloud_mean_fwd_f32', x, b, c, p, na, slope, x, scale, shift, w, inv_den, out)
    return out


def bn_act_cloud_mean_bwd_reduce(g, x, scale, shift, mean, invstd, w, inv_den, slope):
    b, c, p, na = x.shape
    parts = int(abi.eap_bn_act_cloud_mean_parts(p))
    pg = torch.empty(b, c, parts, dtype=torch.float32, device=x.device)
    pgx = torch.empty_like(pg)
    call('eap_bn_act_cloud_mean_bwd_reduce_f32', x, b, c, p, na, slope, g, x, scale, shift, mean, invstd, w, inv_den, pg, pgx)
    return pg.sum(2, dtype=torch.float64), pgx.sum(2, dtype=torch.float64)


def bn_act_cloud_mean_bwd_apply(g, x, scale, shift, mean, invstd, k2, k3, w, inv_den, stat_mask, slope):
    b, c, p, na = x.shape
    gx = torch.empty_like(x)
    call('eap_bn_act_cloud_mean_bwd_apply_f32', x, b, c, p, na, slope, g, x, scale, shift, mean, invstd, k2, k3, w, inv_den, stat_mask, gx)
    return gx



def bn_act_cloud_mean_wide_fwd(x, scale, shift, w, inv_den, slope):
    b, c, p, na = x.shape
    out = torch.empty(b, c, na, dtype=torch.float32, device=x.device)
    call('eap_bn_act_cloud_mean_wide_fwd_f32', x, b, c, p, na, slope, x, scale, shift, w, inv_den, out)
    return out


def bn_act_cloud_mean_wide_bwd_reduce(g, x, scale, shift, mean, invstd, w, inv_den, slope):
    b, c, p, na = x.shape
    parts = int(abi.eap_bn_act_cloud_mean_wide_parts(p))
    pg = torch.empty(b, c, parts, dtype=torch.float32, device=x.device)
    pgx = torch.empty_like(pg)
    call('eap_bn_act_cloud_mean_wide_bwd_reduce_f32', x, b, c, p, na, slope, g, x, scale, shift, mean, invstd, w, inv_den, pg, pgx)
    return pg.sum(2, dtype=torch.float64), pgx.sum(2, dtype=torch.float64)


def bn_act_cloud_mean_wide_bwd_apply(g, x, scale, shift, mean, invstd, k2, k3, w, inv_den, stat_mask, slope):
    b, c, p, na = x.shape
    gx = torch.empty_like(x)
    call('eap_bn_act_cloud_mean_wide_bwd_apply_f32', x, b, c, p, na, slope, g, x, scale, shift, mean, invstd, k2, k3, w, inv_den, stat_mask, gx)
    return gx



def _slot_f32(*tensors):
    check_input(*tensors)
    for t in tensors:
        if t is not None and t.dtype != torch.float32:
            raise RuntimeError(f'slot attention kernels take float32 tensors, not {t.dtype}')


# ... 75 lines not shown
```

equi-articulated-pose_amd/vgtk/so3conv/functional.py:

```python
import math
import os
import weakref

import numpy as np
import torch

import vgtk
import vgtk.functional as fr
import vgtk.pc as pctk
import vgtk.spconv as zpconv
import vgtk.cuda.grouping as cuda_nn

from .. import _hip
from . import norm_fold

inter_so3conv_feat_grouping = zpconv.inter_zpconv_grouping_naive
batched_index_select = zpconv.batched_index_select
batched_index_select_other = zpconv.batched_index_select_other

MATERIALIZE_INTER_W = False

GAMMA_SIZE = 3
ROOT = vgtk.__path__[0]
Rs, R_idx, canonical_relative = fr.icosahedron_so3(GAMMA_SIZE)
# ... 514 lines not shown
    def moments(self, s1, s2, pivot, count):
        norm = self.norm
        gamma = norm.weight.detach().double()
        scale, shift, mean, invstd, total = norm_fold.fold((s1, s2, pivot, count), gamma, norm.bias.detach(), norm.running_mean, norm.running_var,
                                                           True, norm.momentum, norm.eps, sync=norm.sync)
        self.stats = (mean, invstd)
        inv_gamma = torch.where(gamma == 0, torch.zeros_like(gamma), 1.0 / gamma).float()
        self.saved = (scale, norm.bias.detach().float().clone(), inv_gamma.contiguous(), total)
        return scale.contiguous(), shift.contiguous(), float(norm.negative_slope)

    def takes_partials(self, t):
        norm = self.norm
        return bool(_hip.NATIVE_NORM_GLUE and t.is_cuda and not norm_fold._syncing(norm.sync) and norm.weight.dtype == torch.float32
                    and norm.bias.dtype == torch.float32 and (norm.running_mean is None or norm.running_mean.dtype == torch.float32))

    def moments_from_partials(self, ps, pq, pivot, count):
        norm = self.norm
        running = (None, None) if norm.running_mean is None else (norm.running_mean, norm.running_var)
        scale, shift, mean, invstd, beta, inv_gamma = _hip.norm_fold_train(ps, pq, pivot, count, norm.weight.detach().contiguous(),
                                                                          norm.bias.detach().contiguous(), norm.eps, norm.momentum, *running)
        self.stats = (mean, invstd)
        self.saved = (scale, beta, inv_gamma, count)
        return scale, shift, float(norm.negative_slope)


def _contract_into(W, x, y, layout, epilogue=None, b0=0, x_bound=None):
    b, c, ks, p, na = x.shape
    o = W.shape[0]
    if layout == 2:
        xt = x.view(b, p * na, c * ks).transpose(1, 2)
    if epilogue is not None and layout == 2:
        res = None if epilogue.residual is None else epilogue.residual[b0:b0 + b]
        if _hip.matmul_epilogue(W, xt, y, epilogue.scale, epilogue.shift, epilogue.slope, res, b_bound=x_bound):
            epilogue.applied = True
            return
        if b0 > 0 and epilogue.applied:
            raise RuntimeError('folded epilogue: the slabs of one contraction took different kernels')
    if layout == 2:
        _hip.matmul(W, xt, y, b_bound=x_bound)
    elif layout == 1:
        _hip.gemm(0, 0, o, p * na, c * ks, W, c * ks, 0, x, p * na, c * ks * p * na, y, p * na, o * p * na, b, b_blocked=True)
    else:
        _hip.matmul(W, x.view(b, c * ks, p * na), y)


def _grouped_bound(feats, idx):
    if not (_hip.SPLIT_BF16_CONTRACTION and _hip.SPLIT_PLANES == 2):
        return None
    return _hip.so3_grouped_bound(feats, idx)


BACKWARD_LOG = None
FORWARD_LOG = None


DENSE_MODE = os.environ.get('EAP_DENSE', 'auto')
DENSE_ROW_FACTOR = 5.0
DENSE_MAX_GROUPS = 16.0
DENSE_MAX_GROUPS_WIDE = 16.0
DENSE_FWD_NARROW = True
FUSE_CONV_NORM = True
NORM_IN_NODE_MAX_RATIO = 128.0


def _dense_rows(rcap, n):
    return (rcap + 15) & ~15


def _dense_wanted(head, o, p, na, ks, nn, n):
    if DENSE_MODE == 'off' or head is None or head.memb is None:
        return 0, False
    rcap, _ = head.decide()
    rp = _dense_rows(rcap, n)
    if rp <= 0 or rp > n or not head.dense_possible() or not _hip.so3_dense_supported(p, na, ks, rp, o):
        return 0, False
    if DENSE_MODE == 'force':
        return rp, True
    if rp > DENSE_ROW_FACTOR * nn and not (rp <= _hip.DENSE_MAX_ROWS and
                                           head.groups_touched() <= (DENSE_MAX_GROUPS if rp <= _hip.DENSE_NARROW_ROWS else DENSE_MAX_GROUPS_WIDE)):
        return 0, False
    return rp, (o % 256 == 0) or DENSE_FWD_NARROW


def _weight_grad_from_z(z, fc, b, c, o, ks, ra, ldz=None):
    ldz = ra if ldz is None else ldz
    z = z.view(b, o * ks, ldz)[..., :ra]
    dt = torch.empty(c, o * ks, dtype=torch.float32, device=z.device)
    if _hip.matmul_reduce_takes_split(fc, z.transpose(1, 2), dt):
        _hip.matmul_reduce(fc, z.transpose(1, 2), dt)
        return dt.view(c, o, ks).permute(1, 0, 2).reshape(o, c * ks).contiguous()
    d = dt.view(o * ks, c)
    _hip.matmul_reduce(z, fc.transpose(1, 2), d)
    return d.view(o, ks, c).permute(0, 2, 1).reshape(o, c * ks).contiguous()


DENSE_MAX_PARTS = 6
_POSE_PARTS = {}


class _PoseParts:

    def __init__(self, labels, reps, sizes, p):
        dev = labels.device
        b = labels.shape[0]
        self.labels, self.reps, self.sizes, self.n = labels, reps, sizes, len(sizes[0])
        self.single = self.n == 1
        order = torch.argsort(labels, dim=1, stable=True)
        self.pts, self.col_map, self.width = [], [], []
        start = [0] * b
        for i in range(self.n):
            width = (max(sizes[bi][i] for bi in range(b)) + 31) // 32 * 32
            st = torch.tensor(start, dtype=torch.int64, device=dev)[:, None]
            sz = torch.tensor([sizes[bi][i] for bi in range(b)], dtype=torch.int64, device=dev)[:, None]
            t = torch.arange(width, dtype=torch.int64, device=dev)[None, :]
            valid = t < sz
            pts = order.gather(1, (st + torch.where(valid, t, torch.zeros_like(t))).clamp(max=p - 1))
            self.pts.append(pts.contiguous())
            self.col_map.append(torch.where(valid, pts, torch.full_like(pts, -1)).to(torch.int32).contiguous())
            self.width.append(width)
            start = [start[bi] + sizes[bi][i] for bi in range(b)]


def _pose_parts(rot):
    key = (rot.data_ptr(), rot._version, tuple(rot.shape))
    hit = _POSE_PARTS.get(key)
    if hit is not None and hit[0]() is rot:
        return hit[1]
    b, p = rot.shape[:2]
    dev = rot.device
    r9 = rot[:, :, :3, :3].reshape(b * p, 9).contiguous()
    bits = r9.view(torch.int32).to(torch.int64)
    mul = torch.tensor([0x9E3779B97F4A7C15 - (1 << 64), 0xC2B2AE3D27D4EB4F - (1 << 64), 0x165667B19E3779F9, 0x27D4EB2F165667C5, 0x85EBCA77C2B2AE63 - (1 << 64),
                        0x2545F4914F6CDD1D, 0x5851F42D4C957F2D, 0x14057B7EF767814F, 0x3C6EF372FE94F82B], dtype=torch.int64, device=dev)
    h = (bits * mul).sum(1)
    h = (h ^ (h >> 31)) & ((1 << 55) - 1)
    keys = h + (torch.arange(b, dtype=torch.int64, device=dev).repeat_interleave(p) << 55)
    uniq, inv, counts = torch.unique(keys, return_inverse=True, return_counts=True)
    result = None
    if uniq.numel() <= b * DENSE_MAX_PARTS:
        nu = uniq.numel()
        first = torch.full((nu,), b * p, dtype=torch.int64, device=dev).scatter_reduce(0, inv, torch.arange(b * p, dtype=torch.int64, device=dev), 'amin')
        rep = r9[first]
        same = (rep[inv] == r9).all().to(torch.int64)
        host = torch.cat([same[None], uniq >> 55, counts]).tolist()
        ok, cloud, cnt = host[0], host[1:1 + nu], host[1 + nu:]
        per = [[] for _ in range(b)]
        for u in range(nu):
            per[cloud[u]].append((cnt[u], u))
        n = max(len(x) for x in per)
        if ok and n <= DENSE_MAX_PARTS and min(len(x) for x in per) >= 1:
            slot = [0] * nu
            sizes = [[0] * n for _ in range(b)]
            rep_idx = [[per[bi][0][1]] * n for bi in range(b)]
            for bi in range(b):
                for i, (c_, u) in enumerate(sorted(per[bi], key=lambda x: (-x[0], x[1]))):
                    slot[u], sizes[bi][i], rep_idx[bi][i] = i, c_, u
            labels = torch.tensor(slot, dtype=torch.int64, device=dev)[inv].view(b, p)
            reps = rep[torch.tensor(rep_idx, dtype=torch.int64, device=dev)].view(b, n, 3, 3)
            result = _PoseParts(labels, reps, sizes, p)
    if len(_POSE_PARTS) > 16:
        _POSE_PARTS.clear()
    _POSE_PARTS[key] = (weakref.ref(rot), result)
    return result


class _PartsDense:

    def __init__(self, parts, xyz, memb, rows, rp, rk, sigma, nn, n_rows, mult, anchors):
        b, p = parts.labels.shape
        dev = xyz.device
        self.parts, self.rp, self.ks, self.na = parts, int(rp), rk.shape[1], rk.shape[0]
        ld = rows.stride(0)
# ... 143 lines not shown
    Wc = W.index_select(1, _hip.so3_group_fwd_tp_columns(c, ks, W.device)) if tp else W
    x = None
    for b0 in range(0, b, step):
        b1 = min(b, b0 + step)
        x = _hip.so3_inter_group_fwd(feats[b0:b1], idx[b0:b1], gx[b0:b1], rk, mult, sigma,
                                     None if nonident is None else nonident[b0:b1], blocked=layout, coset=coset, store_order=tp)
        _contract_into(Wc, x, y[b0:b1].view(b1 - b0, o, p * na), layout, folded, b0,
                       x_bound=None if x_bound is None else (x_bound[b0:b1], na, 1.0))
        x = x if keep else None
    return y, x


def _forward_map(feats, W, args, keep, folded):
    idx, gx, rk, amap = args.idx, args.gx, args.rk, args.amap
    b, na = feats.shape[0], feats.shape[3]
    p, o = idx.shape[1], W.shape[0]
    y = torch.empty(b, o, p, na, dtype=torch.float32, device=feats.device)
    step = max(1, b if keep else X_CHUNK_CLOUDS)
    x = None
    for b0 in range(0, b, step):
        b1 = min(b, b0 + step)
        x = _hip.so3_inter_group_fwd_map(feats[b0:b1], idx[b0:b1], gx[b0:b1], rk, amap[b0:b1], args.sigma)
        _contract_into(W, x, y[b0:b1].view(b1 - b0, o, p * na), 0, folded, b0)
        x = x if keep else None
    return y, x


def _forward_res(feats, W, args, keep, folded):
    idx, gx, rk, shift = args.idx, args.gx, args.rk, args.shift
    b, na4 = feats.shape[0], feats.shape[3]
    p, o = idx.shape[1], W.shape[0]
    y = torch.empty(b, o, p, na4, dtype=torch.float32, device=feats.device)
    step = max(1, b if keep else X_CHUNK_CLOUDS)
    x = None
    for b0 in range(0, b, step):
        b1 = min(b, b0 + step)
        x = _hip.so3_inter_group_fwd_res(feats[b0:b1], idx[b0:b1], gx[b0:b1], rk, shift[b0:b1], args.sigma)
        _contract_into(W, x, y[b0:b1].view(b1 - b0, o, p * na4), 0, folded, b0)
        x = x if keep else None
    return y, x


def _backward_res(gy, W, feats, x, args, need_f, need_w):
    b, c, n, na4 = feats.shape
    idx, gx, rk, shift = args.idx, args.gx, args.rk, args.shift
    p, ks = idx.shape[1], rk.shape[1]
    o, ck, pa = W.shape[0], c * ks, p * na4
    gF = gW = None
    if need_w:
        if x is None:
            x = _hip.so3_inter_group_fwd_res(feats, idx, gx, rk, shift, args.sigma)
        gW = torch.empty_like(W)
        _hip.matmul_reduce(gy.view(b, o, pa), x.view(b, ck, pa).transpose(1, 2), gW)
        x = None
    if need_f:
        gx_ = torch.empty(b, ck, pa, dtype=torch.float32, device=gy.device)
        Wt = W.t().contiguous()
        _hip.matmul(Wt, gy.view(b, o, pa), gx_)
        gF = _hip.so3_inter_group_bwd_res(gx_.view(b, c, ks, p, na4), idx, gx, rk, shift, args.sigma, n)
    return gF, gW



def _forward_narrow(feats, W, args, train_ep):
    idx, rk = args.idx, args.rk
    b, c, _, na = feats.shape
    p, ks, o = idx.shape[1], rk.shape[1], W.shape[0]
    x = _hip.so3_inter_group_fwd(feats, idx, args.gx, rk, args.mult, args.sigma, args.nonident).view(b, c * ks, p * na)
    if train_ep.takes_partials(x):
        scale, shift, slope = train_ep.moments_from_partials(*_hip.narrow_conv_stats(W, x, partials=True), b * p * na)
    else:
        s1, s2, pivot = _hip.narrow_conv_stats(W, x)
        scale, shift, slope = train_ep.moments(s1, s2, pivot, b * p * na)
    y = _hip.narrow_conv_bnact_fwd(W, x, scale, shift, slope).view(b, o, p, na)
    train_ep.applied = True
    mean, invstd = train_ep.stats
    return y, x, (scale, shift, mean.float(), invstd.float(), train_ep.saved[3], slope, bool(train_ep.norm.sync))


def _native_norm_bwd(gy, count, sync):
    return bool(_hip.NATIVE_NORM_GLUE and gy.is_cuda and isinstance(count, int) and not norm_fold._syncing(sync))


def _backward_narrow(gy, W, x, bn, need_w):
    scale, shift, mean, invstd, count, slope, sync = bn
    b, o = gy.shape[0], gy.shape[1]
    gy = gy.view(b, o, -1)
    if _native_norm_bwd(gy, count, sync):
        g_bn_w, g_bn_b, k2, k3 = _hip.norm_fold_bwd(*_hip.narrow_conv_bwd_reduce(gy, x, W, scale, shift, mean, invstd, slope, partials=True), scale, count)
        return (_hip.narrow_conv_bwd_dw(gy, x, W, scale, shift, mean, invstd, k2, k3, slope) if need_w else None), g_bn_w, g_bn_b
    sg, sgx = _hip.narrow_conv_bwd_reduce(gy, x, W, scale, shift, mean, invstd, slope)
    gW = None
    if need_w:
        k2, k3 = norm_fold.backward_coefficients(scale, sg, sgx, count, True, sync)
        gW = _hip.narrow_conv_bwd_dw(gy, x, W, scale, shift, mean, invstd, k2, k3, slope)
    return gW, sgx.float(), sg.float()



def _weight_operand(W, c, ks, pad_c=None):
    o = W.shape[0]
    W2 = W.view(o, c, ks).permute(1, 0, 2).reshape(c, o * ks).contiguous()
    if pad_c is not None and pad_c != c:
        W2 = torch.cat([W2, torch.zeros(pad_c - c, o * ks, dtype=torch.float32, device=W.device)])
    return W2


def _rows_grad_from_z(z, W2, c, rp, na, ldz, anchor_major, z_bound=None, reorder=None):
    b, (pad_c, oks) = z.shape[0], W2.shape
    gFc = torch.empty(b, pad_c, ldz, dtype=torch.float32, device=z.device)
    _hip.matmul(W2, z.view(b, oks, ldz), gFc, b_bound=z_bound)
    if anchor_major:
        return gFc[:, :c, :rp * na].reshape(b, c, na, rp).transpose(2, 3)
    gFc = gFc.view(b, c, rp, na)
    return gFc if reorder is None else _hip.anchor_reorder(gFc, reorder)


def _weight_grad_rows(z, fc4, o, ks, ldz, anchor_major, reorder=None):
    b, c, rp, na = fc4.shape
    if reorder is not None:
        fc4 = _hip.anchor_reorder(fc4, reorder)
    fc = fc4.transpose(2, 3).contiguous() if anchor_major else fc4
    return _weight_grad_from_z(z, fc.view(b, c, rp * na), b, c, o, ks, rp * na, ldz)



def _backward_dense(gy, W, feats, head, geo, bn, yact, need_f, need_w):
    b, c, n, na = feats.shape
    o, ks, p, rp = W.shape[0], geo.ks, gy.shape[2], geo.rp
    if BACKWARD_LOG is not None:
        BACKWARD_LOG.append({'channels': (c, o), 'support_rows': n, 'referenced_rows_max': int(rp), 'regime': 'dense rows',
                             **({'norm': 'in the node'} if bn is not None else {})})
    ra = na * rp
    pad_c = 128 if (c == 64 and bn is not None) else c
    ldz = _hip.dense_pitch(ra) if (pad_c % 128 == 0 and (o * ks) % 16 == 0 and need_f) else ra
    gF = gW = g_bn_w = g_bn_b = z_bound = None
    if bn is not None:
        k1, beta, inv_gamma, count, slope, sync = bn
        native = _native_norm_bwd(gy, count, sync)
        if native:
            pg, pgx, gmax, xmax = _hip.bn_act_bwd_reduce_fromy(gy, yact, beta, inv_gamma, slope, partials=True)
            g_bn_w, g_bn_b, _, _, coef, bound, colmax = _hip.norm_fold_bwd(pg, pgx, k1, count, beta, inv_gamma, gmax, xmax)
        else:
            sg, sgx, gmax, xmax = _hip.bn_act_bwd_reduce_fromy(gy, yact, beta, inv_gamma, slope)
            g_bn_w, g_bn_b = sgx.float(), sg.float()
            k2, k3 = norm_fold.backward_coefficients(k1, sg, sgx, count, True, sync)
            coef = torch.stack([k1, k2, k3, beta, inv_gamma]).contiguous()
            bound = (k1.abs()[None, :, None] * gmax + k2.abs()[None, :, None] + k3.abs()[None, :, None] * xmax).contiguous()
        z = _hip.so3_dense_bwd_bn(gy, yact, geo, ldz, coef, bound, slope)
        if ldz % 4 == 0 and rp % 4 == 0 and native:
            z_bound = (_hip.so3_dense_zbound(colmax, head.cnt, head.n_rows, rp, p, ldz).view(torch.int32), 4, 1.0)
        elif ldz % 4 == 0 and rp % 4 == 0:
            live = torch.arange(rp, device=gy.device)[None, :] < head.n_rows[:, None]
            cntf = torch.where(live, head.cnt[:, :rp], torch.zeros_like(head.cnt[:, :rp])).clamp(min=0, max=p).to(torch.float32)
            cols = bound.amax(1)[:, :, None] * cntf[:, None, :]
            words = torch.zeros(b, ldz // 4, dtype=torch.float32, device=gy.device)
            words[:, :ra // 4] = cols.view(b, na, rp // 4, 4).amax(3).view(b, ra // 4)
            z_bound = (words.view(torch.int32), 4, 1.0)
    else:
        z = _hip.so3_dense_bwd(gy, geo, ldz)
    if need_f:
        gFr = _rows_grad_from_z(z, _weight_operand(W, c, ks, pad_c), c, rp, na, ldz, True, z_bound)
        gF = _hip.rows_scatter(gFr.contiguous(), head.rows, n)
    if need_w:
        gW = _weight_grad_rows(z, _hip.rows_gather(feats, head.rows, rp), o, ks, ldz, True)
    return gF, gW, g_bn_w, g_bn_b


def _backward_dense_parts(gy, W, feats, head, pd, need_f, need_w):
    b, c, n, na = feats.shape
    o, ks, rp = W.shape[0], pd.ks, pd.rp
    ra = na * rp
    if BACKWARD_LOG is not None:
        BACKWARD_LOG.append({'channels': (c, o), 'support_rows': n, 'referenced_rows_max': int(rp), 'regime': 'dense rows', 'parts': pd.parts.n})
    ldz = _hip.dense_pitch(ra) if (c % 128 == 0 and (o * ks) % 16 == 0 and need_f) else ra
    W2 = _weight_operand(W, c, ks) if need_f else None
    fc0 = _hip.rows_gather(feats, head.rows, rp) if need_w else None
    gFr = gW = None
    rowmax = _hip.take_rowmax_hint(gy)
    for i, geo in enumerate(pd.geo):
        perm = pd.perm[i]
        z = _hip.so3_dense_bwd(gy, geo, ldz, colmap=pd.parts.col_map[i], rowmax=rowmax)
        pe = None if perm is None else perm[:, None].expand(b, c, rp, na)
        if need_f:
            t = _rows_grad_from_z(z, W2, c, rp, na, ldz, True)
            if gFr is None:
                gFr = torch.zeros(b, c, rp, na, dtype=torch.float32, device=gy.device)
            if pe is None:
                gFr += t
            else:
                gFr.scatter_add_(3, pe, t.contiguous())
        if need_w:
            gw = _weight_grad_rows(z, fc0 if pe is None else fc0.gather(3, pe), o, ks, ldz, True)
            gW = gw if gW is None else gW + gw
        del z
    gF = _hip.rows_scatter(gFr, head.rows, n) if need_f else None
    return gF, gW


def _backward_lists(gy, W, feats, idx, gx, rk, mult, args, head, rcap, any_nonident, need_f, need_w):
    b, c, n, na = feats.shape
    p, ks, o = idx.shape[1], rk.shape[1], W.shape[0]
    gF = gW = None
    rcap = min((rcap + 3) & ~3, n)
    head.wait()
    rows = head.rows[:, :rcap].contiguous()
    off, cnt = head.off[:, :rcap].contiguous(), head.cnt[:, :rcap].contiguous()
    ent_p, ent_gx = head.entries if head.entries is not None else _hip.inv_lists_fill(idx, gx, head.rows, head.off, rcap)
    multinv = _group_tables_inverse(mult) if (mult is not None and any_nonident) else None
    coset = _coset_tables(multinv, args.ident) if multinv is not None else None
    z_order = z_pos = None
    if coset is not None and _hip.so3_group_perm_lists2_takes(o, na, ks, p):
        z_order, z_pos = coset[0], coset[2]
        ent_pc, ent_gx2 = _hip.so3_perm_entries(ent_p, ent_gx, coset[1], args.anchors, args.ident, na, p)
        z = _hip.so3_inter_group_inv_perm2(_hip.anchor_reorder(gy, z_order), rows, off, cnt, ent_pc, ent_gx2, rk, z_order,
                                           args.sigma, idx.shape[2])
    else:
        z = _hip.so3_inter_group_inv(gy, rows, off, cnt, ent_p, ent_gx, rk, multinv, args.sigma, idx.shape[2],
                                     args.ident, args.anchors, coset)
    if need_f:
        gFr = _rows_grad_from_z(z, _weight_operand(W, c, ks), c, rcap, na, rcap * na, False, reorder=z_pos)
        gF = _hip.rows_scatter(gFr, rows, n)
    if need_w:
        gW = _weight_grad_rows(z, _hip.rows_gather(feats, rows, rcap), o, ks, rcap * na, False, reorder=z_order)
    return gF, gW


def _backward_textbook(gy, W, feats, x, idx, gx, rk, mult, nonident, args, layout, need_f, need_w):
    b, c, n, na = feats.shape
    p, ks = idx.shape[1], rk.shape[1]
    o, ck, pa = W.shape[0], c * ks, p * na
    gF = gW = None
    if x is None:
        x = _hip.so3_inter_group_fwd(feats, idx, gx, rk, mult, args.sigma, nonident, blocked=layout,
                                     coset=_coset_tables(mult, args.ident) if (mult is not None and layout == 2) else None)
    if need_w:
        gW = torch.empty_like(W)
        if layout == 2:
            _hip.matmul_reduce(gy.view(b, o, pa), x.view(b, pa, ck), gW)
        elif layout == 1:
            _hip.gemm_reduce(0, 1, o, ck, pa, gy, pa, o * pa, x, pa, ck * pa, gW, ck, b, b_blocked=True)
        else:
            _hip.matmul_reduce(gy.view(b, o, pa), x.view(b, ck, pa).transpose(1, 2), gW)
    if need_f:
        gx_ = torch.empty_like(x.view(b, ck, pa))
        Wt = W.t().contiguous()
        _hip.matmul(Wt, gy.view(b, o, pa), gx_)
        gF = _hip.so3_inter_group_bwd(gx_.view(b, c, ks, p, na), idx, gx, rk, mult, args.sigma, n, args.ident)
    return gF, gW


def _backward_map(gy, W, feats, x, args, need_f, need_w):
    b, c, n, na = feats.shape
    idx, gx, rk, amap = args.idx, args.gx, args.rk, args.amap
    p, ks = idx.shape[1], rk.shape[1]
    o, ck, pa = W.shape[0], c * ks, p * na
    gF = gW = None
    if need_w:
        if x is None:
            x = _hip.so3_inter_group_fwd_map(feats, idx, gx, rk, amap, args.sigma)
        gW = torch.empty_like(W)
        _hip.matmul_reduce(gy.view(b, o, pa), x.view(b, ck, pa).transpose(1, 2), gW)
    if need_f:
        gx_ = torch.empty(b, ck, pa, dtype=torch.float32, device=gy.device)
        Wt = W.t().contiguous()
        _hip.matmul(Wt, gy.view(b, o, pa), gx_)
        gF = _hip.so3_inter_group_bwd_map(gx_.view(b, c, ks, p, na), idx, gx, rk, amap, args.sigma, n)
    return gF, gW


class _InterConv(torch.autograd.Function):

    DIFFERENTIABLE = 4

    @staticmethod
    def forward(ctx, feats, W_param, bn_weight, bn_bias, args):
        feats = feats.contiguous()
        W = W_param.contiguous()
        idx, rk, mult, nonident = args.idx, args.rk, args.mult, args.nonident
        can = X_LAYOUT != 'reference' and _hip.so3_inter_group_fwd_can_block(
            feats.shape[1], feats.shape[2], feats.shape[3], rk.shape[1], mult is not None, nonident is not None)
        layout = 0 if not can else (2 if X_LAYOUT == 'transposed' else 1)
        _, c, n, na = feats.shape
        p, ks, o = idx.shape[1], rk.shape[1], W.shape[0]
        needs_grad = (ctx.needs_input_grad[0] or ctx.needs_input_grad[1]) and args.grad_mode
        train_ep = args.epilogue if isinstance(args.epilogue, TrainEpilogue) else None
        folded = None if train_ep is not None else args.epilogue
        if folded is not None and (needs_grad or not folded.inference):
            raise RuntimeError('a folded epilogue is an inference-time fusion: build and use it under torch.no_grad()')
        if args.amap is not None or args.shift is not None:
            regime, fwd = ('anchor map', _forward_map) if args.shift is None else ('residual map', _forward_res)
            if FORWARD_LOG is not None:
                FORWARD_LOG.append({'channels': (c, o), 'dense': False, 'parts': None, 'regime': regime})
            y, x = fwd(feats, W, args, needs_grad and ctx.needs_input_grad[1], folded)
            ctx.bn, ctx.conv_args, ctx.head, ctx.layout, ctx.plan = None, args, None, 0, None
            ctx.W_param = weakref.ref(W_param)
            ctx.save_for_backward(W, x, idx, args.gx, rk, None, nonident, feats, None)
            return y
        narrow = c * ks <= _hip.NARROW_CONV_MAX_CK and not ctx.needs_input_grad[0]
        if narrow and train_ep is not None and FUSE_CONV_NORM and _hip.narrow_conv_takes(o, c * ks, p * na):
            if FORWARD_LOG is not None:
                FORWARD_LOG.append({'channels': (c, o), 'dense': False, 'parts': None, 'regime': 'narrow input'})
            y, x, bn = _forward_narrow(feats, W, args, train_ep)
            wanted = args.grad_mode and any(ctx.needs_input_grad[1:_InterConv.DIFFERENTIABLE])
            ctx.bn, ctx.conv_args, ctx.head, ctx.layout, ctx.plan = (bn if wanted else None), args, None, 0, None
            ctx.narrow = True
            ctx.W_param = weakref.ref(W_param)
            ctx.save_for_backward(W, x if wanted else None, idx, None, rk, None, None, feats, None)
            return y
        lists_ok = BACKWARD_MODE != 'dx' and _inv_lists_supported(idx, n, na, ks) and not narrow
        keep = needs_grad and (not lists_ok or _keep_x_hint(W_param))
        plan = _DensePlan(args, n, o, lists_ok, needs_grad, keep, folded, train_ep.norm if (train_ep is not None and FUSE_CONV_NORM) else None)
        head = plan.head if needs_grad else None
        if FORWARD_LOG is not None:
            FORWARD_LOG.append({'channels': (c, o), 'dense': bool(plan.forward), 'parts': None if plan.parts is None else plan.parts.n})
        if plan.forward:
            bn_only = args.grad_mode and not needs_grad and (ctx.needs_input_grad[2] or ctx.needs_input_grad[3])
            join = FUSE_CONV_NORM and not bn_only and train_ep is not None and not plan.head.norm_ill()
            y, ctx.bn = _forward_dense(feats, W, plan, p, train_ep if join else None, folded)
            x, layout = None, 0
        else:
            fill = head is not None and plan.probed and not keep and plan.rp == 0
            y, x = _forward_lists(feats, W, args, layout, keep, folded, head, fill)
            ctx.bn = None
        ctx.conv_args, ctx.head, ctx.layout = args, head, layout
        ctx.plan = plan if (plan.rp > 0 and needs_grad) else None
        ctx.W_param = weakref.ref(W_param)
        ctx.save_for_backward(W, x, idx, args.gx, rk, mult, nonident, feats, y if (ctx.bn is not None and needs_grad) else None)
        return y

    @staticmethod
    def backward(ctx, gy):
        W, x, idx, gx, rk, mult, nonident, feats, yact = ctx.saved_tensors
        args, head, plan = ctx.conv_args, ctx.head, ctx.plan
        gy = gy.contiguous()
        n = feats.shape[2]
        need_f, need_w = ctx.needs_input_grad[0], ctx.needs_input_grad[1]
        g_bn_w = g_bn_b = None
        if getattr(ctx, 'narrow', False):
            if BACKWARD_LOG is not None:
                BACKWARD_LOG.append({'channels': (feats.shape[1], W.shape[0]), 'support_rows': n, 'referenced_rows_max': 0,
                                     'regime': 'narrow input', 'norm': 'in the node'})
            gF = None
            gW, g_bn_w, g_bn_b = _backward_narrow(gy, W, x, ctx.bn, need_w)
        elif args.amap is not None or args.shift is not None:
            regime, bwd = ('anchor map', _backward_map) if args.shift is None else ('residual map', _backward_res)
            if BACKWARD_LOG is not None:
                BACKWARD_LOG.append({'channels': (feats.shape[1], W.shape[0]), 'support_rows': n, 'referenced_rows_max': 0, 'regime': regime})
            gF, gW = bwd(gy, W, feats, x, args, need_f, need_w)
        elif plan is not None and plan.parts is not None:
            gF, gW = _backward_dense_parts(gy, W, feats, head, plan.geo(), need_f, need_w)
        elif plan is not None:
            gF, gW, g_bn_w, g_bn_b = _backward_dense(gy, W, feats, head, plan.geo(), ctx.bn, yact, need_f, need_w)
        else:
            rcap, any_nonident = 0, True
            if head is not None:
                rcap, any_nonident = head.decide()
                if BACKWARD_MODE == 'auto' and rcap * INV_ROW_FRACTION > n:
                    head.entries = None
                    head = None
            if BACKWARD_LOG is not None:
                BACKWARD_LOG.append({'channels': (feats.shape[1], W.shape[0]), 'support_rows': n, 'referenced_rows_max': int(rcap),
                                     'regime': 'inverse lists' if head is not None else 'textbook dX'})
            Wp = ctx.W_param()
            if Wp is not None:
                _set_keep_x_hint(Wp, head is None)
            if head is not None:
                gF, gW = _backward_lists(gy, W, feats, idx, gx, rk, mult, args, head, rcap, any_nonident, need_f, need_w)
            else:
                gF, gW = _backward_textbook(gy, W, feats, x, idx, gx, rk, mult, nonident, args, ctx.layout, need_f, need_w)
        return (gF, gW, g_bn_w, g_bn_b) + (None,) * (len(ctx.needs_input_grad) - _InterConv.DIFFERENTIABLE)


INTRA_DW_SLICE = 64


def _intra_inverse_table(idx32):
    na, nt = idx32.shape
    inv = torch.empty_like(idx32)
    inv.scatter_(0, idx32.long(), torch.arange(na, device=idx32.device, dtype=torch.int32)[:, None].expand(na, nt).contiguous())
    return inv.contiguous()


def _intra_kernels(feats, idx32):
    if feats.shape[3] == idx32.shape[0]:
        return _hip.so3_intra_conv, _hip.so3_intra_group_fwd
    return _hip.so3_intra_conv2d, _hip.so3_intra_group2d_fwd


class _IntraConv(torch.autograd.Function):

    @staticmethod
    def forward(ctx, feats, W, idx32):
        feats, W = feats.contiguous(), W.contiguous()
        ctx.save_for_backward(feats, W, idx32)
        return _intra_kernels(feats, idx32)[0](feats, W, idx32)

    @staticmethod
    def backward(ctx, gy):
        feats, W, idx32 = ctx.saved_tensors
        gy = gy.contiguous()
        b, c, p, tot = feats.shape
        o, (na, nt) = W.shape[0], idx32.shape
        conv, group = _intra_kernels(feats, idx32)
        gF = gW = None
        if ctx.needs_input_grad[0]:
            W2 = W.view(o, c, nt).permute(1, 0, 2).reshape(c, o * nt).contiguous()
            gF = conv(gy, W2, _intra_inverse_table(idx32))
        if ctx.needs_input_grad[1]:
            gW = torch.empty(o, c, nt, dtype=torch.float32, device=gy.device)
            pa = p * tot
            step = max(1, INTRA_DW_SLICE * na // tot)
            for c0 in range(0, c, step):
                c1 = min(c, c0 + step)
                g = group(feats[:, c0:c1].contiguous(), idx32)
                d = torch.empty(o, (c1 - c0) * nt, dtype=torch.float32, device=gy.device)
                _hip.matmul_reduce(gy.view(b, o, pa), g.view(b, (c1 - c0) * nt, pa).transpose(1, 2), d)
                gW[:, c0:c1] = d.view(o, c1 - c0, nt)
                del g, d
            gW = gW.view(o, c * nt)
        return gF, gW, None


def intra_so3conv(feats, W, intra_idx):
    if feats.dtype != torch.float32 or not feats.is_cuda:
        raise RuntimeError('intra_so3conv: float32 device tensors only')
    return _IntraConv.apply(feats, W, intra_idx.to(torch.int32).contiguous())
# ... 433 lines not shown
```

include/eap_hip.h:

```cpp
#ifndef EAP_HIP_H
#define EAP_HIP_H

#include <stdint.h>

#ifdef __cplusplus
extern "C" {
#endif

typedef void *eap_stream_t;

const char *eap_last_error(void);
int eap_launch_dims_ok(int64_t gx, int64_t gy, int64_t gz, int bx, int by, int bz);
const char *eap_last_kernel(void);
int eap_abi_version(void);


int eap_ball_query_f32(int b, int n, int m, float radius, int nsample, const float *new_xyz,
                       const float *xyz, int32_t *idx, eap_stream_t stream);
int eap_ball_query_f64(int b, int n, int m, float radius, int nsample, const double *new_xyz,
                       const double *xyz, int32_t *idx, eap_stream_t stream);

int eap_furthest_point_sampling_f32(int b, int n, int m, const float *xyz, float *temp,
                                    int32_t *idx, eap_stream_t stream);
int eap_furthest_point_sampling_f64(int b, int n, int m, const double *xyz, double *temp,
// ... 182 lines not shown
int eap_so3_dense_untranspose_f32(int b, int o, int p, int na, const float *yt, float *y, float *psum, float *psq, eap_stream_t stream);
int eap_so3_dense_untranspose_map_f32(int b, int o, int p, int na, int p_dst, const int32_t *map, const float *yt, float *y,
                                      eap_stream_t stream);
int eap_so3_dense_untranspose_map_stats_f32(int b, int o, int p, int na, int p_dst, const int32_t *map, const int32_t *pivot_pos, const float *yt,
                                            float *y, float *psum, float *psq, eap_stream_t stream);
int eap_so3_dense_split_bn_f32(int b, int m, int l, int l_src, int na, const uint32_t *rowbound, const int32_t *colmap, const float *grad,
                               const float *act, const float *coef, float slope, float *scale, void *planes, eap_stream_t stream);
int eap_so3_dense_untranspose_bnact_f32(int b, int o, int p, int na, int p_dst, const int32_t *map, const float *yt, const float *bn_scale,
                                        const float *bn_shift, float slope, float *y, eap_stream_t stream);
int eap_so3_dense_gplanes_supported(int o, int c, int na, int ks, int rp);
int eap_so3_dense_gplanes_f32(int b, int o, int c, int na, int ks, int rp, const float *W3, const float *Ft, const int32_t *n_rows,
                              const float *bound, float *scale, void *planes, eap_stream_t stream);
int eap_so3_dense_point_keys(int b, int p, const uint32_t *memb, int32_t *keys, eap_stream_t stream);
int64_t eap_so3_dense_steps_words(int b, int p, int ks, int rp, int dir);
int eap_so3_dense_steps(int b, int p, int ks, int rp, int dir, int skip, const int32_t *n_rows, const uint64_t *mask, int32_t *steps,
                        eap_stream_t stream);
int eap_so3_dense_product_steps_f32(int dir, int b, int o, int p, int na, int ks, int rp, int64_t ldz, float sigma, const int32_t *n_rows,
                                    const void *planes, const float *scale, const float *pt, const float *kr, const uint64_t *mask,
                                    const int32_t *steps, float *out, eap_stream_t stream);
int eap_so3_dense_max_rows(void);
int eap_so3_dense_member_wide(int b, int p, int n, int nn, int rp, int rows_ld, const int32_t *idx, const int32_t *rows,
                              const int32_t *n_rows, int32_t *slot_of, uint32_t *memb, int32_t *flags, eap_stream_t stream);
int eap_so3_dense_point_keys_wide(int b, int p, const uint32_t *memb, int64_t *keys, eap_stream_t stream);
int eap_so3_dense_masks_wide(int b, int p, int ks, int rp, int dir, const uint32_t *memb, uint64_t *mask, eap_stream_t stream);
int eap_so3_dense_steps_wide(int b, int p, int ks, int rp, int dir, int skip, const int32_t *n_rows, const uint64_t *mask, int32_t *steps,
                             eap_stream_t stream);
int64_t eap_so3_dense_probe_workspace(int b);
int eap_so3_dense_probe(int b, int p, int words, const int32_t *n_rows, const int32_t *nonident, const int32_t *dflags,
                        const uint32_t *memb, const float *rot_a, int64_t blocks_a, const float *rot_b, int64_t blocks_b,
                        const float *rot_cloud, const float *norm_w, const float *norm_b, int channels, float ratio,
                        int32_t *work, int32_t *out, eap_stream_t stream);


int eap_so3_intra_group_fwd_f32(int b, int c, int p, int na, int t, const float *feats,
                                const int32_t *intra_idx, float *out, eap_stream_t stream);
int eap_so3_intra_group_bwd_f32(int b, int c, int p, int na, int t, const float *gout,
                                const int32_t *intra_idx, float *gfeats, eap_stream_t stream);



int eap_gemm_f32(int transA, int transB, int M, int N, int K, const float *A, int64_t lda,
                 int64_t strideA, const float *B, int64_t ldb, int64_t strideB, float *C,
                 int64_t ldc, int64_t strideC, int batch, eap_stream_t stream);

int64_t eap_gemm_f32_reduce_workspace(int M, int N, int K, int batch);
int eap_gemm_f32_reduce(int transA, int transB, int M, int N, int K, const float *A, int64_t lda,
                        int64_t strideA, const float *B, int64_t ldb, int64_t strideB, float *C,
                        int64_t ldc, int batch, float *workspace, eap_stream_t stream);

int eap_gemm_bf16x3_f32_supported(int M, int N, int K, const float *A, int64_t lda, const float *B, int64_t ldb,
                                  int64_t strideB);
int eap_gemm_bf16x3_f32(int M, int N, int K, const float *A, int64_t lda, const float *B, int64_t ldb, int64_t strideB,
                        float *C, int64_t ldc, int64_t strideC, int batch, eap_stream_t stream);
int eap_gemm_bf16x3_presplit(int on);
int eap_gemm_bf16x3_nn_f32_supported(int M, int N, int K, const float *A, int64_t lda, const float *B, int64_t ldb,
                                     int64_t strideB);
int eap_gemm_bf16x3_nn_f32(int M, int N, int K, const float *A, int64_t lda, const float *B, int64_t ldb, int64_t strideB,
                           float *C, int64_t ldc, int64_t strideC, int batch, eap_stream_t stream);
int eap_gemm_bf16x3_ep_f32(int transB, int M, int N, int K, const float *A, int64_t lda, const float *B, int64_t ldb, int64_t strideB,
                           float *C, int64_t ldc, int64_t strideC, int batch, const float *scale, const float *shift, float slope,
                           const float *residual, int64_t strideRes, eap_stream_t stream);
int eap_gemm_bf16x3_reduce_f32_supported(int M, int N, int K, const float *A, int64_t lda, int64_t strideA, const float *B,
                                         int64_t ldb, int64_t strideB, int64_t ldc);
int64_t eap_gemm_bf16x3_reduce_workspace(int M, int N, int K, int batch);
int eap_gemm_bf16x3_reduce_f32(int M, int N, int K, const float *A, int64_t lda, int64_t strideA, const float *B, int64_t ldb,
                               int64_t strideB, float *C, int64_t ldc, int batch, float *workspace, eap_stream_t stream);
int eap_so3_intra_conv_bf16x3_f32_supported(int b, int o, int c, int p, int na, int nt);
int eap_so3_intra_conv_bf16x3_f32(int b, int o, int c, int p, int na, int nt, const float *W, const float *feats,
                                  const int32_t *intra_idx, float *out, eap_stream_t stream);
int eap_absmax_rows_f32(const float *x, int batch, int rows, int cols, int64_t ld, int64_t stride, int32_t *out_bits, eap_stream_t stream);
int eap_absmax_colgroups_f32(const float *x, int batch, int rows, int cols, int64_t ld, int64_t stride, int grp, int32_t *out_bits,
                             eap_stream_t stream);
int eap_so3_grouped_bound_f32(int b, int p, int nn, int n_sup, const int32_t *point_max_bits, const int32_t *idx, int32_t *out_bits,
                              eap_stream_t stream);
int eap_gemm_f16x2_f32(int trans_b, int M, int N, int K, const float *A, int64_t lda, const float *B, int64_t ldb, int64_t strideB,
                       float *C, int64_t ldc, int64_t strideC, int batch, const int32_t *abs_a, const int32_t *abs_b, int grp_b, float mult_b,
                       const float *scale, const float *shift, float slope, const float *residual, int64_t strideRes,
                       eap_stream_t stream);
int eap_gemm_f16x2_splitk_slabs(int M, int N, int K, int batch, int cus);
int64_t eap_gemm_f16x2_splitk_workspace(int M, int N, int batch, int slabs);
int eap_gemm_f16x2_splitk_f32(int M, int N, int K, const float *A, int64_t lda, const float *B, int64_t ldb, int64_t strideB,
                              float *C, int64_t ldc, int64_t strideC, int batch, const int32_t *abs_a, const int32_t *abs_b, int grp_b,
                              float mult_b, int slabs, float *workspace, int64_t workspace_floats, eap_stream_t stream);
int eap_so3_intra_conv_f16x2_f32(int b, int o, int c, int p, int na, int nt, const float *W, const float *feats,
                                 const int32_t *intra_idx, float *out, const int32_t *abs_w, const int32_t *abs_f, eap_stream_t stream);


int eap_gemm_dma_f32_supported(int transA, int transB, int M, int N, int K, const float *A, int64_t lda,
                               int64_t strideA, const float *B, int64_t ldb, int64_t strideB);
int eap_gemm_dma_f32(int transA, int transB, int M, int N, int K, const float *A, int64_t lda, int64_t strideA,
                     const float *B, int64_t ldb, int64_t strideB, float *C, int64_t ldc, int64_t strideC,
                     int batch, eap_stream_t stream);
int64_t eap_gemm_dma_f32_reduce_workspace(int M, int N, int K, int batch);
int eap_gemm_dma_f32_reduce(int transA, int transB, int M, int N, int K, const float *A, int64_t lda,
                            int64_t strideA, const float *B, int64_t ldb, int64_t strideB, float *C, int64_t ldc,
                            int batch, float *workspace, eap_stream_t stream);
int eap_gemm_skinny_reduce_f32_supported(int M, int N, int K, const float *A, int64_t lda, int64_t strideA, const float *B,
                                         int64_t ldb, int64_t strideB);
int64_t eap_gemm_skinny_reduce_workspace(int M, int N, int K, int batch);
int eap_gemm_skinny_reduce_f32(int M, int N, int K, const float *A, int64_t lda, int64_t strideA, const float *B, int64_t ldb,
                               int64_t strideB, float *C, int64_t ldc, int batch, float *workspace, eap_stream_t stream);

int eap_so3_inter_group_fwd_can_block(int c, int n, int na, int ks, int has_mult, int has_flag);
int eap_so3_inter_group_fwd_xb_f32(int b, int c, int p, int n, int nn, int na, int ks, float sigma,
                                   const float *feats, const int32_t *idx, const float *gx,
                                   const float *rk, const uint8_t *mult, const int32_t *nonident,
                                   float *out, eap_stream_t stream);
int eap_so3_inter_group_fwd_t_f32(int b, int c, int p, int n, int nn, int na, int ks, float sigma,
                                  const float *feats, const int32_t *idx, const float *gx,
                                  const float *rk, const uint8_t *mult, const int32_t *nonident,
                                  float *out, eap_stream_t stream);
int eap_gemm_f32_xb(int transA, int transB, int M, int N, int K, const float *A, int64_t lda,
                    int64_t strideA, const float *B, int64_t b_block_rows, int64_t strideB, float *C,
                    int64_t ldc, int64_t strideC, int batch, eap_stream_t stream);
int eap_gemm_f32_reduce_xb(int transA, int transB, int M, int N, int K, const float *A, int64_t lda,
                           int64_t strideA, const float *B, int64_t b_block_rows, int64_t strideB,
                           float *C, int64_t ldc, int batch, float *workspace, eap_stream_t stream);

int eap_so3_intra_conv_f32(int b, int o, int c, int p, int na, int nt, const float *W, const float *feats,
                           const int32_t *intra_idx, float *out, eap_stream_t stream);


int eap_so3_intra_group2d_fwd_f32(int b, int c, int p, int na, int nr, int t, const float *feats, const int32_t *intra_idx, float *out,
                                  eap_stream_t stream);
int eap_so3_intra_group2d_bwd_f32(int b, int c, int p, int na, int nr, int t, const float *gout, const int32_t *intra_idx, float *gfeats,
                                  eap_stream_t stream);
int eap_so3_intra_conv2d_f32(int b, int o, int c, int p, int na, int nr, int nt, const float *W, const float *feats,
                             const int32_t *intra_idx, float *out, eap_stream_t stream);
int eap_so3_intra_conv2d_split_supported(int b, int o, int c, int p, int na, int nr, int nt);
int eap_so3_intra_conv2d_bf16x3_f32(int b, int o, int c, int p, int na, int nr, int nt, const float *W, const float *feats,
                                    const int32_t *intra_idx, float *out, eap_stream_t stream);
int eap_so3_intra_conv2d_f16x2_f32(int b, int o, int c, int p, int na, int nr, int nt, const float *W, const float *feats,
                                   const int32_t *intra_idx, float *out, const int32_t *abs_w, const int32_t *abs_f, eap_stream_t stream);


int eap_chamfer_fwd_f32(int b, int n, int m, const float *xyz1, const float *xyz2, float *dist1,
                        float *dist2, int32_t *idx1, int32_t *idx2, eap_stream_t stream);
int eap_chamfer_fwd_f64(int b, int n, int m, const double *xyz1, const double *xyz2, double *dist1,
                        double *dist2, int32_t *idx1, int32_t *idx2, eap_stream_t stream);
int eap_chamfer_bwd_f32(int b, int n, int m, const float *xyz1, const float *xyz2,
                        const int32_t *idx1, const int32_t *idx2, const float *g1, const float *g2,
                        float *gxyz1, float *gxyz2, eap_stream_t stream);
int eap_chamfer_bwd_ordered_f32(int b, int n, int m, const float *xyz1, const float *xyz2,
                                const int32_t *idx1, const int32_t *idx2, const float *g1, const float *g2,
                                float *gxyz1, float *gxyz2, eap_stream_t stream);
int eap_chamfer_bwd_ordered_f64(int b, int n, int m, const double *xyz1, const double *xyz2,
                                const int32_t *idx1, const int32_t *idx2, const double *g1, const double *g2,
                                double *gxyz1, double *gxyz2, eap_stream_t stream);

int eap_orbit_chamfer_fwd_f32(int g, int s, int a, int m, int n, const float *recon, const float *ori, const uint8_t *member,
                              float *r2o_all, int32_t *r2o_all_idx, float *r2o_in, int32_t *r2o_in_idx, float *o2r_all,
                              int32_t *o2r_idx, float *o2r_in, eap_stream_t stream);
int eap_orbit_chamfer_fwd_f64(int g, int s, int a, int m, int n, const double *recon, const double *ori, const uint8_t *member,
                              double *r2o_all, int32_t *r2o_all_idx, double *r2o_in, int32_t *r2o_in_idx, double *o2r_all,
                              int32_t *o2r_idx, double *o2r_in, eap_stream_t stream);
int eap_orbit_chamfer_bwd_f32(int g, int s, int a, int m, int n, const float *recon, const float *ori, const uint8_t *member,
                              const int32_t *r2o_all_idx, const int32_t *r2o_in_idx, const int32_t *o2r_idx, const float *g_r2o_all,
                              const float *g_r2o_in, const float *g_o2r_all, const float *g_o2r_in, float *grecon, eap_stream_t stream);
int eap_orbit_chamfer_bwd_f64(int g, int s, int a, int m, int n, const double *recon, const double *ori, const uint8_t *member,
                              const int32_t *r2o_all_idx, const int32_t *r2o_in_idx, const int32_t *o2r_idx, const double *g_r2o_all,
                              const double *g_r2o_in, const double *g_o2r_all, const double *g_o2r_in, double *grecon, eap_stream_t stream);

int eap_bn_act_segments(int64_t n);
int eap_bn_stats_f32(int b, int c, int64_t n, const float *x, float *psum, float *psq, eap_stream_t stream);
int eap_bn_act_fwd_f32(int b, int c, int64_t n, float slope, const float *x, const float *scale,
                       const float *shift, float *y, eap_stream_t stream);
int eap_bn_act_add_fwd_f32(int b, int c, int64_t n, float slope, const float *x, const float *scale,
                           const float *shift, const float *res, float *y, eap_stream_t stream);
int eap_bn_act_bwd_reduce_f32(int b, int c, int64_t n, float slope, const float *gy, const float *x,
                              const float *scale, const float *shift, const float *mean,
                              const float *invstd, float *pg, float *pgx, eap_stream_t stream);
int eap_bn_act_bwd_apply_f32(int b, int c, int64_t n, float slope, const float *gy, const float *x,
                             const float *scale, const float *shift, const float *mean,
                             const float *invstd, const float *k2, const float *k3, float *gx,
                             eap_stream_t stream);
int eap_bn_act_bwd_apply_rowmax_f32(int b, int c, int64_t n, int na, float slope, const float *gy, const float *x,
                                    const float *scale, const float *shift, const float *mean, const float *invstd,
                                    const float *k2, const float *k3, float *gx, uint32_t *rowmax, eap_stream_t stream);
int eap_bn_act_fromy_blocks(int64_t n, int na);
int eap_bn_act_bwd_reduce_fromy_f32(int b, int c, int64_t n, int na, float slope, const float *gy, const float *y, const float *beta,
                                    const float *inv_gamma, float *pg, float *pgx, uint32_t *gmax, uint32_t *xmax, eap_stream_t stream);

int eap_bn_stats_masked_f32(int b, int c, int64_t n, int na, const float *x, const float *mask, float *psum, float *psq,
                            eap_stream_t stream);
int eap_bn_act_cloud_fwd_f32(int b, int c, int64_t n, float slope, const float *x, const float *scale, const float *shift,
                             float *y, eap_stream_t stream);
int eap_bn_act_cloud_bwd_reduce_f32(int b, int c, int64_t n, float slope, const float *gy, const float *x, const float *scale,
                                    const float *shift, const float *mean, const float *invstd, float *pg, float *pgx,
                                    eap_stream_t stream);
int eap_bn_act_cloud_bwd_apply_f32(int b, int c, int64_t n, int na, float slope, const float *gy, const float *x,
                                   const float *scale, const float *shift, const float *mean, const float *invstd,
                                   const float *k2, const float *k3, const float *mask, float *gx, eap_stream_t stream);

int eap_narrow_contract_supported(int b, int o, int c, int64_t n);
int eap_narrow_contract_fwd_f32(int b, int o, int c, int64_t n, const float *W, const float *x, float *y, eap_stream_t stream);
int eap_narrow_contract_dx_f32(int b, int o, int c, int64_t n, const float *W, const float *g, float *dx, eap_stream_t stream);
int eap_narrow_contract_dw_slabs(int64_t n);
int eap_narrow_contract_dw_f32(int b, int o, int c, int64_t n, const float *g, const float *x, float *partial, eap_stream_t stream);

int eap_narrow_conv_segments(int64_t n);
int eap_narrow_conv_stats_f32(int b, int o, int ck, int64_t n, const float *W, const float *x, float *pivot, float *psum, float *psq,
                              eap_stream_t stream);
int eap_narrow_conv_bnact_fwd_f32(int b, int o, int ck, int64_t n, float slope, const float *W, const float *x, const float *scale,
                                  const float *shift, float *y, eap_stream_t stream);
int eap_narrow_conv_bwd_reduce_f32(int b, int o, int ck, int64_t n, float slope, const float *gy, const float *x, const float *W,
                                   const float *scale, const float *shift, const float *mean, const float *invstd, float *pg, float *pgx,
                                   eap_stream_t stream);
int eap_narrow_conv_bwd_dw_f32(int b, int o, int ck, int64_t n, float slope, const float *gy, const float *x, const float *W,
                               const float *scale, const float *shift, const float *mean, const float *invstd, const float *k2,
                               const float *k3, float *partial, float *dW, eap_stream_t stream);

int eap_norm_fold_train_f32(int o, int parts, int64_t pivot_stride, int64_t count, int64_t eps_bits, int64_t momentum_bits, const float *ps,
                            const float *pq, const float *pivot, const float *gamma, const float *beta, float *running_mean, float *running_var,
                            float *scale, float *shift, double *mean, double *invstd, float *beta_copy, float *inv_gamma, eap_stream_t stream);
int eap_norm_fold_bwd_f32(int o, int parts, int b, int na, int64_t count, const float *pg, const float *pgx, const float *k1, const float *beta,
                          const float *inv_gamma, const float *gmax, const float *xmax, float *dgamma, float *dbeta, float *k2, float *k3, float *coef,
                          float *bound, float *colmax, eap_stream_t stream);
int eap_so3_dense_zbound_f32(int b, int na, int rp, int p, int ldz, int64_t cnt_stride, const float *colmax, const int32_t *cnt,
                             const int32_t *n_rows, float *words, eap_stream_t stream);
int eap_so3_dense_gplanes_bound_f32(int b, int o, int c, int na, int ks, int rp, const float *W3, const float *fc4, float *fpart, float *wsum,
                                    float *bound, eap_stream_t stream);
int eap_so3_dense_point_order(int b, int p, int words, const int64_t *order, const uint32_t *memb, const float *q_xyz, int32_t *order32,
                              uint32_t *memb_out, float *xyz_out, int32_t *pivot_pos, eap_stream_t stream);

int eap_anchor_attn_pool_fwd_f32(int b, int c, int n, int na, float temperature, const float *x, const float *logits,
                                 float *out, float *conf, eap_stream_t stream);
int eap_anchor_attn_pool_bwd_f32(int b, int c, int n, int na, float temperature, const float *x, const float *logits,
                                 const float *g, float *dx, float *dlogits, eap_stream_t stream);
int eap_slot_masked_mean_fwd_f32(int b, int ns, int c, int n, int na, const float *x, const float *mask,
                                 const float *inv_den, float *out, eap_stream_t stream);
int eap_slot_masked_mean_bwd_f32(int b, int ns, int c, int n, int na, const float *g, const float *mask,
                                 const float *inv_den, float *dx, eap_stream_t stream);
int eap_masked_max_fwd_f32(int b, int c, int n, int na, const float *x, const float *mask, float *out, int32_t *arg,
                           eap_stream_t stream);
int eap_masked_max_bwd_f32(int b, int c, int n, int na, const float *g, const int32_t *arg, const float *mask, float *dx,
                           eap_stream_t stream);
int eap_anchor_attn_pool_wide_fwd_f32(int b, int c, int n, int na, float temperature, const float *x, const float *logits,
                                      float *out, float *conf, eap_stream_t stream);
int eap_anchor_attn_pool_wide_bwd_f32(int b, int c, int n, int na, float temperature, const float *x, const float *logits,
                                      const float *g, float *dx, float *dlogits, eap_stream_t stream);
int eap_slot_masked_mean_wide_fwd_f32(int b, int ns, int c, int n, int na, const float *x, const float *mask,
                                      const float *inv_den, float *out, eap_stream_t stream);
int eap_slot_masked_mean_wide_bwd_f32(int b, int ns, int c, int n, int na, const float *g, const float *mask,
                                      const float *inv_den, float *dx, eap_stream_t stream);
int eap_masked_max_wide_fwd_f32(int b, int c, int n, int na, const float *x, const float *mask, float *out, int32_t *arg,
                                eap_stream_t stream);
int eap_masked_max_wide_bwd_f32(int b, int c, int n, int na, const float *g, const int32_t *arg, const float *mask, float *dx,
                                eap_stream_t stream);
int eap_bn_act_cloud_mean_fwd_f32(int b, int c, int n, int na, float slope, const float *x, const float *scale, const float *shift,
                                  const float *w, const float *inv_den, float *out, eap_stream_t stream);
int eap_bn_act_cloud_mean_parts(int n);
int eap_bn_act_cloud_mean_bwd_reduce_f32(int b, int c, int n, int na, float slope, const float *g, const float *x, const float *scale,
                                         const float *shift, const float *mean, const float *invstd, const float *w, const float *inv_den,
                                         float *pg, float *pgx, eap_stream_t stream);
int eap_bn_act_cloud_mean_bwd_apply_f32(int b, int c, int n, int na, float slope, const float *g, const float *x, const float *scale,
                                        const float *shift, const float *mean, const float *invstd, const float *k2, const float *k3,
                                        const float *w, const float *inv_den, const float *stat_mask, float *gx, eap_stream_t stream);
int eap_bn_act_cloud_mean_wide_fwd_f32(int b, int c, int n, int na, float slope, const float *x, const float *scale, const float *shift,
                                       const float *w, const float *inv_den, float *out, eap_stream_t stream);
int eap_bn_act_cloud_mean_wide_parts(int n);
int eap_bn_act_cloud_mean_wide_bwd_reduce_f32(int b, int c, int n, int na, float slope, const float *g, const float *x, const float *scale,
                                              const float *shift, const float *mean, const float *invstd, const float *w, const float *inv_den,
                                              float *pg, float *pgx, eap_stream_t stream);
int eap_bn_act_cloud_mean_wide_bwd_apply_f32(int b, int c, int n, int na, float slope, const float *g, const float *x, const float *scale,
                                             const float *shift, const float *mean, const float *invstd, const float *k2, const float *k3,
                                             const float *w, const float *inv_den, const float *stat_mask, float *gx, eap_stream_t stream);

int eap_slot_attn_stats_f32(int b, int d, int n, float ln_eps, const float *x, float *mean, float *rstd, eap_stream_t stream);
int eap_slot_attn_scores_fwd_f32(int b, int s, int d, int n, float eps, const float *x, const float *mean, const float *rstd, const float *u,
                                 const float *c0, float *attn, eap_stream_t stream);
int eap_slot_attn_pool_parts(int n);
int eap_slot_attn_pool_f32(int b, int s, int d, int n, const float *x, const float *mean, const float *rstd, const float *w, float *psum,
                           eap_stream_t stream);
int eap_slot_attn_scores_bwd_f32(int b, int s, int d, int n, float eps, const float *x, const float *mean, const float *rstd, const float *attn,
                                 const float *gmsum, const float *gwsum, const float *gattn, float *gdots, eap_stream_t stream);
int eap_slot_attn_input_grad_f32(int b, int j, int d, int n, const float *x, const float *mean, const float *rstd, const float *rows,
                                 const float *vecs, float *gx, eap_stream_t stream);

int eap_pointnet_max_parts(int n);
int eap_pointnet_max_fwd_f32(int b, int c, int o, int n, int na, const float *feats, const float *xyz, const float *centre, const float *member,
                             const float *wt, const float *v, const float *bias, float *pval, int32_t *parg, float *out, int32_t *arg,
                             eap_stream_t stream);
int eap_pointnet_max_bwd_data_f32(int b, int c, int o, int n, int na, const float *g, const int32_t *arg, const float *w, int ldw, float *dfeats,
                                  float *dcoords, eap_stream_t stream);
int eap_pointnet_max_bwd_weight_f32(int b, int c, int o, int n, int na, const float *g, const int32_t *arg, const float *feats, const float *xyz,
                                    const float *centre, const float *anchors, float *dwp, eap_stream_t stream);

#ifdef __cplusplus
}
#endif
#endif
```

Baseline: 174.5 point-clouds/sec.

## Add two-plane f16 reduce GEMM for weight grads and row-list narrow backward

Adds an f16x2 (two-plane) variant of the batched reduce GEMM, using per-batch row magnitude bounds for A and B, so the dense weight gradient can use two split planes instead of three. A new kernel computes per-row z bounds to feed it. It also adds a row-list variant of the narrow-conv backward reduction that visits only the rows referenced by the preceding scatter, passed along as a hint on the gradient tensor. This trades precision margin and extra bookkeeping kernels for less GEMM work and fewer columns scanned in the reduction.

After: 175.8 point-clouds/sec, median of 3. About the same (+0.8%).

```diff
diff --git a/equi-articulated-pose_amd/csrc/gemm_bf16x3.hip b/equi-articulated-pose_amd/csrc/gemm_bf16x3.hip
--- a/equi-articulated-pose_amd/csrc/gemm_bf16x3.hip
+++ b/equi-articulated-pose_amd/csrc/gemm_bf16x3.hip
@@ -24,6 +24,7 @@
     long long sA; int slabs, kslab;
     const float *ep_scale, *ep_shift, *ep_res; float ep_slope; long long sRes;
     const unsigned *absA, *absB; float multB; int grpB; long long sAbsB;
+    long long sAbsA;
 };
 constexpr int TAPS = 12;
 constexpr unsigned TBL_BYTES = 64 * TAPS * 4;
@@ -112,9 +113,11 @@
     const unsigned offP = (unsigned)((long long)rq * pre_pitch + PRE_PIECE * c4);
     float sclA[2] = {1.0f, 1.0f}, sclB[2] = {1.0f, 1.0f};
     const unsigned *absBz = g.absB + item_of_z * g.sAbsB;
+    const unsigned *absAz = g.absA;
+    if constexpr (PL == 2 && BMODE == 0) absAz += item_of_z * g.sAbsA;
     if constexpr (PL == 2) {
 #pragma unroll
-        for (int u = 0; u < NPA; ++u) sclA[u] = pow2_scale(__uint_as_float(g.absA[min(m0 + RG * u, g.M - RG) + rq]));
+        for (int u = 0; u < NPA; ++u) sclA[u] = pow2_scale(__uint_as_float(absAz[min(m0 + RG * u, g.M - RG) + rq]));
 #pragma unroll
         for (int u = 0; u < NPO; ++u) sclB[u] = pow2_scale(__uint_as_float(absBz[(min(n0 + RG * u, g.N - RG) + rqb) / g.grpB]) * g.multB);
     }
@@ -349,7 +352,7 @@
                 const int row = m0 + 32 * MI * wm + 32 * i + (r & 3) + 8 * (r >> 2) + 4 * lh;
                 if (row < g.M && col < g.N) {
                     float v = acc[i][j][r];
-                    if constexpr (PL == 2) v = (v * (1.0f / pow2_scale(__uint_as_float(g.absA[row])))) * unsB;
+                    if constexpr (PL == 2) v = (v * (1.0f / pow2_scale(__uint_as_float(absAz[row])))) * unsB;
                     if (g.ep_scale != nullptr) {
                         v = fmaf(v, g.ep_scale[row], g.ep_shift[row]);
                         v = v >= 0.f ? v : v * g.ep_slope;
@@ -763,6 +766,32 @@
     if (int e = launch_split<0>(g, (long long)batch * slabs, eap::S(stream), "gemm_bf16x3_reduce_f32")) return e;
     const long long mn4 = (long long)M * N / 4;
     return eap::run_kernel("gemm_bf16x3_reduce_f32 (sum of the partials)", split_reduce_kernel, eap::cdiv(mn4, 256), 1, 1, dim3(256), 0, eap::S(stream), mn4,
+                           batch * slabs, reinterpret_cast<const f32x4 *>(workspace), C, N, (long long)ldc);
+}
+
+extern "C" int eap_gemm_f16x2_reduce_f32(int M, int N, int K, const float *A, int64_t lda, int64_t strideA, const float *B, int64_t ldb,
+                                         int64_t strideB, float *C, int64_t ldc, int batch, const int32_t *abs_a, const int32_t *abs_b,
+                                         float *workspace, int64_t workspace_floats, eap_stream_t stream) {
+    if (M <= 0 || N <= 0 || batch <= 0) return eap::bad_arg("gemm_f16x2_reduce_f32: M, N and batch must be positive");
+    if (!A || !B || !C || !workspace) return eap::bad_arg("gemm_f16x2_reduce_f32: A, B, C and the workspace are required");
+    if (!abs_a || !abs_b) return eap::bad_arg("gemm_f16x2_reduce_f32: the row magnitudes of both operands are required (abs_a [batch][M], abs_b [batch][N])");
+    if (!eap_gemm_bf16x3_reduce_f32_supported(M, N, K, A, lda, strideA, B, ldb, strideB, ldc) || !eap::aligned16(C, workspace))
+        return eap::bad_arg("gemm_f16x2_reduce_f32: unsupported operands (ask eap_gemm_bf16x3_reduce_f32_supported; C and the workspace 16-byte aligned)");
+    if (workspace_floats < eap_gemm_bf16x3_reduce_workspace(M, N, K, batch))
+        return eap::bad_arg("gemm_f16x2_reduce_f32: the workspace is too small (ask eap_gemm_bf16x3_reduce_workspace)");
+    const int slabs = reduce_slabs(M, N, K, batch);
+    if ((long long)batch * slabs > 65535) return eap::bad_arg("gemm_f16x2_reduce_f32: batch x slabs exceeds 65535");
+    Args g{};
+    g.M = M; g.N = N; g.K = K;
+    g.A = A; g.lda = lda; g.sA = strideA;
+    g.B = B; g.ldb = ldb; g.sB = strideB;
+    g.C = workspace; g.ldc = N; g.sC = (long long)M * N;
+    g.slabs = slabs; g.kslab = K / slabs;
+    g.absA = reinterpret_cast<const unsigned *>(abs_a); g.sAbsA = M;
+    g.absB = reinterpret_cast<const unsigned *>(abs_b); g.multB = 1.0f; g.grpB = 1; g.sAbsB = N;
+    if (int e = launch_split<0, 2>(g, (long long)batch * slabs, eap::S(stream), "gemm_f16x2_reduce_f32")) return e;
+    const long long mn4 = (long long)M * N / 4;
+    return eap::run_kernel("gemm_f16x2_reduce_f32 (sum of the partials)", split_reduce_kernel, eap::cdiv(mn4, 256), 1, 1, dim3(256), 0, eap::S(stream), mn4,
                            batch * slabs, reinterpret_cast<const f32x4 *>(workspace), C, N, (long long)ldc);
 }
 
diff --git a/equi-articulated-pose_amd/csrc/narrow_conv.hip b/equi-articulated-pose_amd/csrc/narrow_conv.hip
--- a/equi-articulated-pose_amd/csrc/narrow_conv.hip
+++ b/equi-articulated-pose_amd/csrc/narrow_conv.hip
@@ -163,16 +163,17 @@
     }
 }
 
-template <int KS2>
-__global__ __launch_bounds__(NT) void narrow_conv_bwd_reduce_kernel(int ct, int o, int ck, long n, int nseg, float slope,
-                                                                      const float *__restrict__ gy, const float *__restrict__ x,
-                                                                      const float *__restrict__ W, const float *__restrict__ scale,
-                                                                      const float *__restrict__ shift, const float *__restrict__ mean,
-                                                                      const float *__restrict__ invstd, float *__restrict__ pg,
-                                                                      float *__restrict__ pgx) {
+struct RowList { const int32_t *rows; int rld, rcap, na, p; };
+
+template <int KS2, bool ROWS>
+__device__ __forceinline__ void bwd_reduce_body(int ct, int o, int ck, long n, int nseg, float slope, const float *__restrict__ gy,
+                                                const float *__restrict__ x, const float *__restrict__ W, const float *__restrict__ scale,
+                                                const float *__restrict__ shift, const float *__restrict__ mean, const float *__restrict__ invstd,
+                                                float *__restrict__ pg, float *__restrict__ pgx, const RowList rl) {
     __shared__ __attribute__((aligned(16))) float s_sc[64], s_sh[64], s_mu[64], s_is[64];
     __shared__ float s_red[WAVES][2][32];
-    const Pos w(ct, n);
+    const long nv = ROWS ? (long)rl.rcap * rl.na : n;
+    const Pos w(ct, nv);
     const int t = threadIdx.x, o0 = blockIdx.y * ct * 32, h = w.h;
     if (t < 32 * ct) { s_sc[t] = scale[o0 + t]; s_sh[t] = shift[o0 + t]; s_mu[t] = mean[o0 + t]; s_is[t] = invstd[o0 + t]; }
     __syncthreads();
@@ -183,14 +184,25 @@
     for (int r = 0; r < 16; ++r) sa[r] = qa[r] = 0.f;
     const float *xb = x + (size_t)w.bi * ck * n;
     const float *gb = gy + ((size_t)w.bi * o + w.ch0) * n;
-    const unsigned roff = 4u * (4u * h * (unsigned)n + 4u * w.li);
+    const unsigned roff0 = 4u * (4u * h * (unsigned)n + 4u * w.li);
     const int lc = w.ch0 - o0;
 #pragma unroll 1
     for (long col0 = w.beg + (long)w.cw * TILE; col0 < w.end; col0 += (long)w.ncw * TILE) {
         const long col = col0 + 4 * w.li;
-        const bool ok = col < n;
+        bool ok = col < nv;
+        long cb = col0;
+        unsigned xoff = ROWS ? 0u : w.xoff, roff = roff0;
+        if constexpr (ROWS) {
+            const int slot = (int)(col / rl.na);
+            const int r = ok ? rl.rows[(size_t)w.bi * rl.rld + slot] : -1;
+            ok = ok && (unsigned)r < (unsigned)rl.p;
+            const unsigned rc = ok ? (unsigned)r * (unsigned)rl.na + (unsigned)(col - (long)slot * rl.na) : 0u;
+            cb = 0;
+            xoff = 4u * ((unsigned)h * (unsigned)n + rc);
+            roff = 4u * (4u * h * (unsigned)n + rc);
+        }
         f32x4 xa[KS2];
-        load_x<KS2>(xa, xb, n, col0, w.xoff, ok, ck, h);
+        load_x<KS2>(xa, xb, n, cb, xoff, ok, ck, h);
         f32x16 d[4];
         conv_tile<KS2, false>(d, xa, wf);
         if (ok) {
@@ -198,7 +210,7 @@
             for (int g = 0; g < 4; ++g) {
                 f32x4 gv[4];
 #pragma unroll
-                for (int q = 0; q < 4; ++q) gv[q] = ld_off<f32x4>(gb + (size_t)(8 * g) * n + col0, roff + 4u * q * (unsigned)n);
+                for (int q = 0; q < 4; ++q) gv[q] = ld_off<f32x4>(gb + (size_t)(8 * g) * n + cb, roff + 4u * q * (unsigned)n);
                 const f32x4 sc = *reinterpret_cast<const f32x4 *>(&s_sc[lc + 8 * g + 4 * h]), sh = *reinterpret_cast<const f32x4 *>(&s_sh[lc + 8 * g + 4 * h]);
                 const f32x4 mu = *reinterpret_cast<const f32x4 *>(&s_mu[lc + 8 * g + 4 * h]), is = *reinterpret_cast<const f32x4 *>(&s_is[lc + 8 * g + 4 * h]);
 #pragma unroll
@@ -215,6 +227,26 @@
         }
     }
     block_sums(sa, qa, s_red, ct, o0, w.bi, gridDim.z, nseg, w.seg, pg, pgx);
+}
+
+template <int KS2>
+__global__ __launch_bounds__(NT) void narrow_conv_bwd_reduce_kernel(int ct, int o, int ck, long n, int nseg, float slope,
+                                                                      const float *__restrict__ gy, const float *__restrict__ x,
+                                                                      const float *__restrict__ W, const float *__restrict__ scale,
+                                                                      const float *__restrict__ shift, const float *__restrict__ mean,
+                                                                      const float *__restrict__ invstd, float *__restrict__ pg,
+                                                                      float *__restrict__ pgx) {
+    bwd_reduce_body<KS2, false>(ct, o, ck, n, nseg, slope, gy, x, W, scale, shift, mean, invstd, pg, pgx, RowList{});
+}
+
+template <int KS2>
+__global__ __launch_bounds__(NT) void narrow_conv_bwd_reduce_rows_kernel(int ct, int o, int ck, long n, int nseg, float slope,
+                                                                           const float *__restrict__ gy, const float *__restrict__ x,
+                                                                           const float *__restrict__ W, const float *__restrict__ scale,
+                                                                           const float *__restrict__ shift, const float *__restrict__ mean,
+                                                                           const float *__restrict__ invstd, float *__restrict__ pg,
+                                                                           float *__restrict__ pgx, RowList rl) {
+    bwd_reduce_body<KS2, true>(ct, o, ck, n, nseg, slope, gy, x, W, scale, shift, mean, invstd, pg, pgx, rl);
 }
 
 template <int KS2>
@@ -368,3 +400,34 @@
     const int mn = o * ck;
     return eap::run_kernel("narrow_conv_bwd_dw (sum)", narrow_conv_dw_sum_kernel, eap::cdiv(mn, 4), 1, 1, dim3(256), 0, s, mn, b * nseg, partial, dW);
 }
+
+namespace {
+
+inline int refuse_rows(const char *who, int64_t n, int na, int rcap, int rows_ld, const void *rows) {
+    char buf[200];
+    const char *why = nullptr;
+    if (na <= 0 || na % 4 != 0 || na > 64) why = "a multiple of 4 anchors, at most 64";
+    else if (n % na != 0) why = "a row length (P*A) that is a multiple of the anchors";
+    else if (rcap <= 0 || (long long)rcap * na >= (1ll << 25)) why = "1 to 2^25 / na row slots";
+    else if (!rows || rows_ld < rcap) why = "a row list with a pitch of at least rcap";
+    if (!why) return 0;
+    snprintf(buf, sizeof(buf), "%s: takes %s", who, why);
+    return eap::bad_arg(buf);
+}
+
+}
+
+extern "C" int eap_narrow_conv_bwd_reduce_rows_f32(int b, int o, int ck, int64_t n, int na, int rcap, int rows_ld, float slope, const float *gy,
+                                                   const float *x, const float *W, const float *scale, const float *shift, const float *mean,
+                                                   const float *invstd, const int32_t *rows, float *pg, float *pgx, eap_stream_t stream) {
+    if (int e = refuse("narrow_conv_bwd_reduce_rows", o, ck, (long)n, x, gy)) return e;
+    if (int e = refuse_rows("narrow_conv_bwd_reduce_rows", n, na, rcap, rows_ld, rows)) return e;
+    if (!gy || !x || !W || !scale || !shift || !mean || !invstd || !pg || !pgx) return eap::bad_arg("narrow_conv_bwd_reduce_rows: null pointer");
+    if (b <= 0 || n <= 0) return 0;
+    const int nseg = nseg_of((long)rcap * na), ct = tiles_per_block(o);
+    const RowList rl{rows, rows_ld, rcap, na, (int)(n / na)};
+    return by_depth(ck, [&](auto ks2) {
+        return eap::run_kernel("narrow_conv_bwd_reduce_rows", narrow_conv_bwd_reduce_rows_kernel<decltype(ks2)::value>, nseg, o / (32 * ct), b, dim3(NT), 0,
+                               eap::S(stream), ct, o, ck, (long)n, nseg, slope, gy, x, W, scale, shift, mean, invstd, pg, pgx, rl);
+    });
+}
diff --git a/equi-articulated-pose_amd/csrc/norm_fold.hip b/equi-articulated-pose_amd/csrc/norm_fold.hip
--- a/equi-articulated-pose_amd/csrc/norm_fold.hip
+++ b/equi-articulated-pose_amd/csrc/norm_fold.hip
@@ -121,6 +121,33 @@
     words[(long)cloud * ldw + w] = v;
 }
 
+__global__ __launch_bounds__(256) void dense_zrowbound_kernel(int o, int na, int ks, int rp, int p, long cnt_stride, const float *__restrict__ bound,
+                                                              const int32_t *__restrict__ cnt, const int32_t *__restrict__ n_rows,
+                                                              float *__restrict__ words) {
+    __shared__ int red[4];
+    const int cloud = blockIdx.y, t = threadIdx.x;
+    int live = n_rows[cloud];
+    live = live < 0 ? 0 : (live > rp ? rp : live);
+    int cm = 0;
+    for (int r = t; r < live; r += 256) {
+        int c = cnt[cloud * cnt_stride + r];
+        c = c < 0 ? 0 : (c > p ? p : c);
+        cm = c > cm ? c : cm;
+    }
+#pragma unroll
+    for (int m = WAVE / 2; m >= 1; m >>= 1) { const int v = __shfl_xor(cm, m, WAVE); cm = v > cm ? v : cm; }
+    if ((t & (WAVE - 1)) == 0) red[t / WAVE] = cm;
+    __syncthreads();
+    cm = max(max(red[0], red[1]), max(red[2], red[3]));
+    const int ch = blockIdx.x * 256 + t;
+    if (ch >= o) return;
+    const float *row = bound + ((long)cloud * o + ch) * na;
+    float m = row[0];
+    for (int a = 1; a < na; ++a) m = nan_max(m, row[a]);
+    const float v = m * (float)cm;
+    for (int k = 0; k < ks; ++k) words[((long)cloud * o + ch) * ks + k] = v;
+}
+
 __global__ __launch_bounds__(256) void dense_gbound_parts_kernel(int bc, int c, int rp, int na, int ks, const float *__restrict__ W3,
                                                                  const float *__restrict__ fc4, float *__restrict__ fpart, float *__restrict__ wsum) {
     __shared__ float red[256];
@@ -246,6 +273,16 @@
                            (long)cnt_stride, colmax, cnt, n_rows, words);
 }
 
+extern "C" int eap_so3_dense_zrowbound_f32(int b, int o, int na, int ks, int rp, int p, int64_t cnt_stride, const float *bound, const int32_t *cnt,
+                                           const int32_t *n_rows, float *words, eap_stream_t stream) {
+    if (!bound || !cnt || !n_rows || !words) return eap::bad_arg("so3_dense_zrowbound: null pointer");
+    if (b <= 0 || o <= 0 || na <= 0 || ks <= 0 || rp <= 0 || p <= 0) return eap::bad_arg("so3_dense_zrowbound: b, o, na, ks, rp and p must be positive");
+    if (b > 65535 || cnt_stride < rp || (long long)o * ks > 0x7fffffffLL)
+        return eap::bad_arg("so3_dense_zrowbound: b at most 65535 (grid.y), the row stride of cnt >= rp, o * ks below 2^31");
+    return eap::run_kernel("so3_dense_zrowbound", dense_zrowbound_kernel, eap::cdiv(o, 256), b, 1, dim3(256), 0, eap::S(stream), o, na, ks, rp, p,
+                           (long)cnt_stride, bound, cnt, n_rows, words);
+}
+
 extern "C" int eap_so3_dense_gplanes_bound_f32(int b, int o, int c, int na, int ks, int rp, const float *W3, const float *fc4, float *fpart,
                                                float *wsum, float *bound, eap_stream_t stream) {
     if (!W3 || !fc4 || !fpart || !wsum || !bound) return eap::bad_arg("so3_dense_gplanes_bound: null pointer");
diff --git a/equi-articulated-pose_amd/vgtk/_hip.py b/equi-articulated-pose_amd/vgtk/_hip.py
--- a/equi-articulated-pose_amd/vgtk/_hip.py
+++ b/equi-articulated-pose_amd/vgtk/_hip.py
@@ -239,6 +239,26 @@
                                                        (scale, shift, slope, residual)))
 
 
+REDUCE_TWO_PLANES = True
+
+
+def gemm_reduce_two_planes(M, N, K, A, lda, strideA, B, ldb, strideB, C, ldc, batch, b_bound):
+    if not REDUCE_TWO_PLANES or SPLIT_PLANES != 2 or b_bound is None or not SPLIT_BF16_CONTRACTION:
+        return False
+    if tuple(b_bound.shape) != (batch, N) or b_bound.element_size() != 4 or not b_bound.is_contiguous():
+        raise RuntimeError(f'gemm_reduce_two_planes: b_bound holds one 4-byte word per row of every B_z, [{batch}, {N}] contiguous, not {tuple(b_bound.shape)}')
+    if C.data_ptr() % 16 != 0 or not abi.eap_gemm_bf16x3_reduce_f32_supported(M, N, K, A, lda, strideA, B, ldb, strideB, ldc):
+        return False
+    abs_a = absmax_rows(A, batch, M, K, lda, strideA)
+    if abs_a is None:
+        return False
+    floats = max(int(abi.eap_gemm_bf16x3_reduce_workspace(M, N, K, batch)), 1)
+    ws = torch.empty(floats, dtype=torch.float32, device=C.device)
+    tag = {'flops': 2.0 * M * N * K * batch, 'shape': ('gemm_reduce', 0, 1, M, N, K, batch)}
+    call('eap_gemm_f16x2_reduce_f32', C, M, N, K, A, lda, strideA, B, ldb, strideB, C, ldc, batch, abs_a, b_bound, ws, floats, tag=tag)
+    return True
+
+
 def gemm_reduce(transA, transB, M, N, K, A, lda, strideA, B, ldb, strideB, C, ldc, batch, b_blocked=False):
     tag = {'flops': 2.0 * M * N * K * batch, 'shape': ('gemm_reduce', int(transA), int(transB), M, N, K, batch)}
     ops = (M, N, K, A, lda, strideA, B, ldb, strideB)
@@ -320,8 +340,10 @@
     gemm(ta, tb, M, N, K, A, lda, sa, B, ldb, sb, out, ldc, sc, batch, b_bound=b_bound)
 
 
-def matmul_reduce(A, B, out):
+def matmul_reduce(A, B, out, b_bound=None):
     ta, tb, M, N, K, lda, sa, ldb, sb, ldc, _, batch = _product(A, B, out, reduce=True)
+    if b_bound is not None and not ta and tb and gemm_reduce_two_planes(M, N, K, A, lda, sa, B, ldb, sb, out, ldc, batch, b_bound):
+        return
     gemm_reduce(ta, tb, M, N, K, A, lda, sa, B, ldb, sb, out, ldc, batch)
 
 
@@ -909,6 +931,16 @@
     return words
 
 
+def so3_dense_zrowbound(bound, cnt, n_rows, ks, rp, p):
+    check_input(bound)
+    b, o, na = bound.shape
+    if cnt.dtype != torch.int32 or n_rows.dtype != torch.int32 or cnt.stride(1) != 1 or not n_rows.is_contiguous() or cnt.shape[1] < rp:
+        raise RuntimeError('so3_dense_zrowbound: cnt and n_rows must be int32, the rows of cnt contiguous and at least rp long')
+    words = torch.empty(b, o * int(ks), dtype=torch.float32, device=bound.device)
+    call('eap_so3_dense_zrowbound_f32', bound, b, o, na, int(ks), int(rp), int(p), cnt.stride(0), bound, cnt, n_rows, words)
+    return words
+
+
 def so3_dense_gplanes_bound(W3, fc4, ks):
     check_input(W3, fc4)
     b, c, rp, na = fc4.shape
@@ -1079,6 +1111,30 @@
     return rowmax
 
 
+_ROWS_HINT = [None]
+USE_ROWS_HINT = True
+ROWS_HINTS_TAKEN = 0
+
+
+def leave_rows_hint(t, rows, n_rows, rcap=None):
+    rcap = int(rows.shape[1] if rcap is None else rcap)
+    _leave_hint(_ROWS_HINT, t, (rows, n_rows, rcap, rows._version, None if n_rows is None else n_rows._version))
+
+
+def take_rows_hint(t):
+    global ROWS_HINTS_TAKEN
+    h = _take_hint(_ROWS_HINT, t)
+    if h is None or not USE_ROWS_HINT:
+        return None
+    rows, n_rows, rcap, v_rows, v_n = h
+    if rows._version != v_rows or (n_rows is not None and n_rows._version != v_n) or not t.is_contiguous() or t.data_ptr() % 16 != 0:
+        return None
+    if rows.dtype != torch.int32 or rows.dim() != 2 or rows.stride(1) != 1 or rows.shape[0] != t.shape[0] or not 0 < rcap <= rows.shape[1]:
+        return None
+    ROWS_HINTS_TAKEN += 1
+    return rows, n_rows, rcap
+
+
 def bn_act_bwd_apply(gy, x, b, c, n, scale, shift, mean, invstd, k2, k3, slope):
     gx = torch.empty_like(x)
     if x.dim() == 4 and x.shape[3] % 4 == 0 and x.shape[3] <= 64 and n == x.shape[2] * x.shape[3] and c % 128 == 0 and gx.data_ptr() % 16 == 0 \
@@ -1146,6 +1202,21 @@
     dW = torch.empty(o, ck, dtype=torch.float32, device=x.device)
     call('eap_narrow_conv_bwd_dw_f32', x, b, o, ck, n, slope, gy, x, W, scale, shift, mean, invstd, k2, k3, partial, dW)
     return dW
+
+
+def narrow_conv_rows_takes(n, na, rcap):
+    return na % 4 == 0 and 0 < na <= 64 and n % na == 0 and 0 < rcap and rcap * na < (1 << 25)
+
+
+def narrow_conv_bwd_reduce_rows(gy, x, W, scale, shift, mean, invstd, slope, na, rows, rcap):
+    check_input(gy, x, W, scale, shift, mean, invstd)
+    b, ck, n = x.shape
+    o = W.shape[0]
+    parts = b * int(abi.eap_narrow_conv_segments(rcap * na))
+    pg = torch.empty(o, parts, dtype=torch.float32, device=x.device)
+    pgx = torch.empty(o, parts, dtype=torch.float32, device=x.device)
+    call('eap_narrow_conv_bwd_reduce_rows_f32', x, b, o, ck, n, int(na), int(rcap), rows.stride(0), slope, gy, x, W, scale, shift, mean, invstd, rows, pg, pgx)
+    return pg, pgx
 
 
 
diff --git a/equi-articulated-pose_amd/vgtk/so3conv/functional.py b/equi-articulated-pose_amd/vgtk/so3conv/functional.py
--- a/equi-articulated-pose_amd/vgtk/so3conv/functional.py
+++ b/equi-articulated-pose_amd/vgtk/so3conv/functional.py
@@ -620,12 +620,12 @@
     return rp, (o % 256 == 0) or DENSE_FWD_NARROW
 
 
-def _weight_grad_from_z(z, fc, b, c, o, ks, ra, ldz=None):
+def _weight_grad_from_z(z, fc, b, c, o, ks, ra, ldz=None, z_row_bound=None):
     ldz = ra if ldz is None else ldz
     z = z.view(b, o * ks, ldz)[..., :ra]
     dt = torch.empty(c, o * ks, dtype=torch.float32, device=z.device)
     if _hip.matmul_reduce_takes_split(fc, z.transpose(1, 2), dt):
-        _hip.matmul_reduce(fc, z.transpose(1, 2), dt)
+        _hip.matmul_reduce(fc, z.transpose(1, 2), dt, b_bound=z_row_bound)
         return dt.view(c, o, ks).permute(1, 0, 2).reshape(o, c * ks).contiguous()
     d = dt.view(o * ks, c)
     _hip.matmul_reduce(z, fc.transpose(1, 2), d)
@@ -935,10 +935,15 @@
     return bool(_hip.NATIVE_NORM_GLUE and gy.is_cuda and isinstance(count, int) and not norm_fold._syncing(sync))
 
 
-def _backward_narrow(gy, W, x, bn, need_w):
+def _backward_narrow(gy, W, x, bn, need_w, rows_hint=None):
     scale, shift, mean, invstd, count, slope, sync = bn
-    b, o = gy.shape[0], gy.shape[1]
+    b, o, na = gy.shape[0], gy.shape[1], gy.shape[3]
     gy = gy.view(b, o, -1)
+    if rows_hint is not None and _native_norm_bwd(gy, count, sync) and _hip.narrow_conv_rows_takes(gy.shape[2], na, rows_hint[2]):
+        rows, _, rcap = rows_hint
+        pg, pgx = _hip.narrow_conv_bwd_reduce_rows(gy, x, W, scale, shift, mean, invstd, slope, na, rows, rcap)
+        g_bn_w, g_bn_b, k2, k3 = _hip.norm_fold_bwd(pg, pgx, scale, count)
+        return (_hip.narrow_conv_bwd_dw(gy, x, W, scale, shift, mean, invstd, k2, k3, slope) if need_w else None), g_bn_w, g_bn_b
     if _native_norm_bwd(gy, count, sync):
         g_bn_w, g_bn_b, k2, k3 = _hip.norm_fold_bwd(*_hip.narrow_conv_bwd_reduce(gy, x, W, scale, shift, mean, invstd, slope, partials=True), scale, count)
         return (_hip.narrow_conv_bwd_dw(gy, x, W, scale, shift, mean, invstd, k2, k3, slope) if need_w else None), g_bn_w, g_bn_b
@@ -969,12 +974,12 @@
     return gFc if reorder is None else _hip.anchor_reorder(gFc, reorder)
 
 
-def _weight_grad_rows(z, fc4, o, ks, ldz, anchor_major, reorder=None):
+def _weight_grad_rows(z, fc4, o, ks, ldz, anchor_major, reorder=None, z_row_bound=None):
     b, c, rp, na = fc4.shape
     if reorder is not None:
         fc4 = _hip.anchor_reorder(fc4, reorder)
     fc = fc4.transpose(2, 3).contiguous() if anchor_major else fc4
-    return _weight_grad_from_z(z, fc.view(b, c, rp * na), b, c, o, ks, rp * na, ldz)
+    return _weight_grad_from_z(z, fc.view(b, c, rp * na), b, c, o, ks, rp * na, ldz, z_row_bound)
 
 
 
@@ -987,7 +992,7 @@
     ra = na * rp
     pad_c = 128 if (c == 64 and bn is not None) else c
     ldz = _hip.dense_pitch(ra) if (pad_c % 128 == 0 and (o * ks) % 16 == 0 and need_f) else ra
-    gF = gW = g_bn_w = g_bn_b = z_bound = None
+    gF = gW = g_bn_w = g_bn_b = z_bound = z_row_bound = None
     if bn is not None:
         k1, beta, inv_gamma, count, slope, sync = bn
         native = _native_norm_bwd(gy, count, sync)
@@ -1003,6 +1008,8 @@
         z = _hip.so3_dense_bwd_bn(gy, yact, geo, ldz, coef, bound, slope)
         if ldz % 4 == 0 and rp % 4 == 0 and native:
             z_bound = (_hip.so3_dense_zbound(colmax, head.cnt, head.n_rows, rp, p, ldz).view(torch.int32), 4, 1.0)
+            if need_w and c % 128 == 0 and _hip.SPLIT_PLANES == 2 and _hip.REDUCE_TWO_PLANES:
+                z_row_bound = _hip.so3_dense_zrowbound(bound, head.cnt, head.n_rows, ks, rp, p).view(torch.int32)
         elif ldz % 4 == 0 and rp % 4 == 0:
             live = torch.arange(rp, device=gy.device)[None, :] < head.n_rows[:, None]
             cntf = torch.where(live, head.cnt[:, :rp], torch.zeros_like(head.cnt[:, :rp])).clamp(min=0, max=p).to(torch.float32)
@@ -1015,8 +1022,9 @@
     if need_f:
         gFr = _rows_grad_from_z(z, _weight_operand(W, c, ks, pad_c), c, rp, na, ldz, True, z_bound)
         gF = _hip.rows_scatter(gFr.contiguous(), head.rows, n)
+        _hip.leave_rows_hint(gF, head.rows, head.n_rows, rp)
     if need_w:
-        gW = _weight_grad_rows(z, _hip.rows_gather(feats, head.rows, rp), o, ks, ldz, True)
+        gW = _weight_grad_rows(z, _hip.rows_gather(feats, head.rows, rp), o, ks, ldz, True, z_row_bound=z_row_bound)
     return gF, gW, g_bn_w, g_bn_b
 
 
@@ -1048,6 +1056,8 @@
             gW = gw if gW is None else gW + gw
         del z
     gF = _hip.rows_scatter(gFr, head.rows, n) if need_f else None
+    if gF is not None:
+        _hip.leave_rows_hint(gF, head.rows, head.n_rows, rp)
     return gF, gW
 
 
@@ -1074,6 +1084,7 @@
     if need_f:
         gFr = _rows_grad_from_z(z, _weight_operand(W, c, ks), c, rcap, na, rcap * na, False, reorder=z_pos)
         gF = _hip.rows_scatter(gFr, rows, n)
+        _hip.leave_rows_hint(gF, rows, getattr(head, 'n_rows', None), rcap)
     if need_w:
         gW = _weight_grad_rows(z, _hip.rows_gather(feats, rows, rcap), o, ks, rcap * na, False, reorder=z_order)
     return gF, gW
@@ -1186,6 +1197,7 @@
     def backward(ctx, gy):
         W, x, idx, gx, rk, mult, nonident, feats, yact = ctx.saved_tensors
         args, head, plan = ctx.conv_args, ctx.head, ctx.plan
+        rows_hint = _hip.take_rows_hint(gy) if getattr(ctx, 'narrow', False) else None
         gy = gy.contiguous()
         n = feats.shape[2]
         need_f, need_w = ctx.needs_input_grad[0], ctx.needs_input_grad[1]
@@ -1195,7 +1207,7 @@
                 BACKWARD_LOG.append({'channels': (feats.shape[1], W.shape[0]), 'support_rows': n, 'referenced_rows_max': 0,
                                      'regime': 'narrow input', 'norm': 'in the node'})
             gF = None
-            gW, g_bn_w, g_bn_b = _backward_narrow(gy, W, x, ctx.bn, need_w)
+            gW, g_bn_w, g_bn_b = _backward_narrow(gy, W, x, ctx.bn, need_w, rows_hint)
         elif args.amap is not None or args.shift is not None:
             regime, bwd = ('anchor map', _backward_map) if args.shift is None else ('residual map', _backward_res)
             if BACKWARD_LOG is not None:
diff --git a/include/eap_hip.h b/include/eap_hip.h
--- a/include/eap_hip.h
+++ b/include/eap_hip.h
@@ -288,6 +288,9 @@
 int eap_gemm_f16x2_splitk_f32(int M, int N, int K, const float *A, int64_t lda, const float *B, int64_t ldb, int64_t strideB,
                               float *C, int64_t ldc, int64_t strideC, int batch, const int32_t *abs_a, const int32_t *abs_b, int grp_b,
                               float mult_b, int slabs, float *workspace, int64_t workspace_floats, eap_stream_t stream);
+int eap_gemm_f16x2_reduce_f32(int M, int N, int K, const float *A, int64_t lda, int64_t strideA, const float *B, int64_t ldb,
+                              int64_t strideB, float *C, int64_t ldc, int batch, const int32_t *abs_a, const int32_t *abs_b,
+                              float *workspace, int64_t workspace_floats, eap_stream_t stream);
 int eap_so3_intra_conv_f16x2_f32(int b, int o, int c, int p, int na, int nt, const float *W, const float *feats,
                                  const int32_t *intra_idx, float *out, const int32_t *abs_w, const int32_t *abs_f, eap_stream_t stream);
 
@@ -415,6 +418,9 @@
 int eap_narrow_conv_bwd_dw_f32(int b, int o, int ck, int64_t n, float slope, const float *gy, const float *x, const float *W,
                                const float *scale, const float *shift, const float *mean, const float *invstd, const float *k2,
                                const float *k3, float *partial, float *dW, eap_stream_t stream);
+int eap_narrow_conv_bwd_reduce_rows_f32(int b, int o, int ck, int64_t n, int na, int rcap, int rows_ld, float slope, const float *gy,
+                                        const float *x, const float *W, const float *scale, const float *shift, const float *mean,
+                                        const float *invstd, const int32_t *rows, float *pg, float *pgx, eap_stream_t stream);
 
 int eap_norm_fold_train_f32(int o, int parts, int64_t pivot_stride, int64_t count, int64_t eps_bits, int64_t momentum_bits, const float *ps,
                             const float *pq, const float *pivot, const float *gamma, const float *beta, float *running_mean, float *running_var,
@@ -424,6 +430,8 @@
                           float *bound, float *colmax, eap_stream_t stream);
 int eap_so3_dense_zbound_f32(int b, int na, int rp, int p, int ldz, int64_t cnt_stride, const float *colmax, const int32_t *cnt,
                              const int32_t *n_rows, float *words, eap_stream_t stream);
+int eap_so3_dense_zrowbound_f32(int b, int o, int na, int ks, int rp, int p, int64_t cnt_stride, const float *bound, const int32_t *cnt,
+                                const int32_t *n_rows, float *words, eap_stream_t stream);
 int eap_so3_dense_gplanes_bound_f32(int b, int o, int c, int na, int ks, int rp, const float *W3, const float *fc4, float *fpart, float *wsum,
                                     float *bound, eap_stream_t stream);
 int eap_so3_dense_point_order(int b, int p, int words, const int64_t *order, const uint32_t *memb, const float *q_xyz, int32_t *order32,
```
